# jeun-990806/pim-jpeg-decoder

Measured on AMD Instinct MI355X. Metric: MPixels/sec JPEG->RGB (bit-exact BMP), higher is better.
Workload: dtype int16/int32 (integer IDCT), u8 out

## Files before the change

### include/pjd.h

```cpp
#ifndef PJD_H
#define PJD_H

#include <stddef.h>
#include <stdint.h>

#ifdef __cplusplus
extern "C" {
#endif

#define PJD_VERSION 6

#define PJD_OK              0
#define PJD_E_NODEVICE     -1
#define PJD_E_HIP          -2
#define PJD_E_ARG          -3
#define PJD_E_NOMEM        -4
#define PJD_E_STATE        -5

#define PJD_ST_OK        0
#define PJD_ST_DC_SYM    1
#define PJD_ST_DC_LEN    2
#define PJD_ST_DC_BITS   3
#define PJD_ST_AC_SYM    4
#define PJD_ST_AC_RUN    5
// ... 64 lines not shown
    uint32_t qt_slot48[4];
    const pjd_scan_desc *scans;
    uint32_t n_scans;
    uint32_t reserved_;
} pjd_image_desc;

typedef struct pjd_ctx pjd_ctx;
typedef struct pjd_batch pjd_batch;

#define PJD_MAX_KERNELS 16
typedef struct pjd_timings {
    int32_t n;
    float   ms[PJD_MAX_KERNELS];
    char    name[PJD_MAX_KERNELS][32];
    float   total_ms;
} pjd_timings;

typedef struct pjd_batch_info {
    int32_t  n_images;
    uint64_t pixels;
    uint64_t ecs_bytes;
    uint64_t out_bytes;
    uint64_t coef_bytes;
    uint64_t n_data_units;
    uint64_t n_subsequences;
    uint64_t device_bytes;
    int32_t  n_sequential;
    int32_t  n_fallback;
    uint64_t n_huff_workgroups;
    uint64_t sync_rounds;
    uint64_t sync_lane_passes;
    uint64_t fix_rounds, fix_lane_passes;
    uint32_t sub_bytes;
    uint32_t n_table_sets;
    uint64_t n_huff_waves;
    uint64_t n_entries;
    float    exact_fallback_ms;
    uint32_t n_entropy_errors;
    uint64_t flag_waves[8];
    uint32_t huff_lds_bytes;
    uint32_t plan_mode;
    uint64_t walks, walk_lanes;
    uint64_t n_steps;
    uint32_t lane_fill_x1024;
    uint32_t dc_plan;
} pjd_batch_info;

int  pjd_version(void);
int  pjd_open(int device_ordinal, pjd_ctx **out);
void pjd_close(pjd_ctx *ctx);
#define PJD_PLAN_LATENCY     0
#define PJD_PLAN_THROUGHPUT  1
int  pjd_set_plan_mode(pjd_ctx *ctx, int mode);
const char *pjd_last_error(pjd_ctx *ctx);
const char *pjd_status_string(int status);
void *pjd_stream(pjd_ctx *ctx);

int  pjd_batch_create(pjd_ctx *ctx, const pjd_image_desc *images, int n_images,
                      int out_format, pjd_batch **out);
int  pjd_batch_upload(pjd_batch *b);
int  pjd_batch_decode(pjd_batch *b);
int  pjd_batch_decode_timed(pjd_batch *b, pjd_timings *t);
int  pjd_batch_capture(pjd_batch *b);
int  pjd_batch_sync(pjd_batch *b);
int  pjd_batch_decode_chains(pjd_batch *b);
int  pjd_batch_download(pjd_batch *b, uint8_t *const *out, int32_t *status);
int  pjd_batch_download_packed(pjd_batch *b, uint8_t *host, uint64_t capacity, int32_t *status);
uint64_t pjd_batch_packed_size(pjd_batch *b);
uint64_t pjd_batch_output_offset(pjd_batch *b, int image);
int  pjd_batch_bind_output(pjd_batch *b, void *device_base, uint64_t capacity, const uint64_t *offsets);
int  pjd_batch_set_resize(pjd_batch *b, const uint32_t *out_w, const uint32_t *out_h);
int  pjd_resize_tap(uint32_t src_n, uint32_t dst_n, uint32_t i, uint32_t *i0, uint32_t *i1, uint32_t *w);
#define PJD_RESIZE_BILINEAR  0
#define PJD_RESIZE_ANTIALIAS 1
#define PJD_AA_MAX_TAPS      32
int  pjd_batch_set_resize_filter(pjd_batch *b, int filter);
int  pjd_resize_aa_taps(uint32_t src_n, uint32_t dst_n, uint32_t i, uint32_t *first, uint32_t *count, uint32_t *q);
#define PJD_RESIZE_BICUBIC      3
#define PJD_BICUBIC_MAX_TAPS    64
#define PJD_BICUBIC_MAX_GAIN    92681
int  pjd_resize_bicubic_taps(uint32_t src_n, uint32_t dst_n, uint32_t i, uint32_t *first, uint32_t *count, int32_t *q);
#define PJD_RW_HFLIP 1u
typedef struct pjd_resize_window {
    uint32_t x, y, w, h;
    uint32_t vw, vh;
    uint32_t ox, oy;
    uint32_t flags;
    uint32_t reserved_;
} pjd_resize_window;
int  pjd_batch_set_resize_window(pjd_batch *b, const pjd_resize_window *win );
int  pjd_resize_window_check(uint32_t sw, uint32_t sh, uint32_t tw, uint32_t th,
                             const pjd_resize_window *win, int filter);
int  pjd_batch_set_orientation(pjd_batch *b, const uint8_t *orientation );
typedef struct pjd_resize_pad { uint32_t left, top, right, bottom; } pjd_resize_pad;
int  pjd_batch_set_resize_pad(pjd_batch *b, const pjd_resize_pad *pad , const uint8_t fill[3]);
int  pjd_batch_set_pad_value(pjd_batch *b, const float value[3]);
int  pjd_resize_pad_check(uint32_t out_w, uint32_t out_h, const pjd_resize_pad *pad);
int  pjd_batch_set_resize_affine(pjd_batch *b, const double (*m)[6] , const uint8_t fill[3]);
int  pjd_warp_tap(const double m[6], uint32_t i, uint32_t j, int64_t *x0, int64_t *y0, uint32_t *wx, uint32_t *wy);
int  pjd_resize_affine_check(uint32_t sw, uint32_t sh, uint32_t tw, uint32_t th, const double m[6]);
int  pjd_batch_set_colour(pjd_batch *b, const double (*m)[12] );
int  pjd_colour_value(const double m[12], const uint8_t rgb[3], uint8_t out[3]);
int  pjd_colour_check(const double m[12]);
#define PJD_BLUR_MAX_TAPS 63
typedef struct pjd_blur { double sigma; uint32_t ksize; uint32_t reserved_; } pjd_blur;
int  pjd_batch_set_blur(pjd_batch *b, const pjd_blur *blur );
int  pjd_blur_taps(uint32_t ksize, double sigma, uint32_t *q );
int  pjd_blur_index(uint32_t n, int64_t i, uint32_t *src);
int  pjd_blur_check(const pjd_blur *blur);
#define PJD_DT_F16   1
#define PJD_DT_BF16  2
#define PJD_DT_F32   3
int  pjd_batch_set_normalize(pjd_batch *b, int dtype, const float scale[3], const float bias[3]);
int  pjd_normalize_value(int dtype, uint32_t v, float scale, float bias, void *out);
#define PJD_MAX_VIEWS 65536u
int  pjd_batch_set_views(pjd_batch *b, const uint32_t *picture_of_view, uint32_t n_views);
uint32_t pjd_batch_n_outputs(pjd_batch *b);
int  pjd_batch_get_info(pjd_batch *b, pjd_batch_info *info);
uint64_t pjd_batch_output_size(pjd_batch *b, int image);
void *pjd_batch_device_output(pjd_batch *b, int image);
void *pjd_batch_device_status(pjd_batch *b);
void pjd_batch_destroy(pjd_batch *b);

uint64_t pjd_coefficients_size(uint32_t width, uint32_t height, uint8_t h_samp, uint8_t v_samp);
int  pjd_batch_download_coefficients(pjd_batch *b, int image, int16_t *out, uint64_t capacity_int16);

int  pjd_decode_batch(pjd_ctx *ctx, const pjd_image_desc *images, int n_images,
                      int out_format, uint8_t *const *out, int32_t *status);

#define PJD_SPLIT_MAX_DEVICES 16
typedef struct pjd_split_stats {
    double   wall_s, broadcast_s, upload_s, exec_s, download_s;
    uint64_t blob_bytes;
    uint64_t ecs_bytes[PJD_SPLIT_MAX_DEVICES];
    uint32_t n_segments, n_ranks;
    uint32_t n_exact;
    int32_t  rccl_used;
    int32_t  redone_whole;
} pjd_split_stats;
int  pjd_split_decode(const pjd_image_desc *desc, const int32_t *devices, int n_devices, int out_format,
                      uint8_t *out, uint64_t capacity, int32_t *status, pjd_split_stats *stats);
int  pjd_split_plan(const pjd_image_desc *desc, int world, int rank, pjd_image_desc *shard, uint64_t *seg_scratch,
                    uint64_t *byte_lo, uint64_t *byte_hi, uint32_t *first_mcu, uint32_t *last_mcu);
void pjd_split_release(void);
int  pjd_split_rccl_selftest(int device_ordinal, uint64_t bytes);

int  pjd_exec_dpu_payload(pjd_ctx *ctx, const uint32_t *metadata, int16_t *mcus, int n_dpus);

int  pjd_plan_info(const pjd_image_desc *images, int n_images, int out_format, pjd_batch_info *info);
int  pjd_plan_check(const pjd_image_desc *images, int n_images, int out_format, char *text, uint64_t cap);
int  pjd_plan_step_bits(const pjd_image_desc *image, uint32_t *step_bits_x256);
int  pjd_plan_luts(const pjd_image_desc *image, void *blob, uint64_t cap, uint32_t *real_bytes, uint32_t *nominal_bytes, uint8_t *slots);
int  pjd_batch_huff_occupancy(pjd_batch *batch, int32_t *workgroups_per_cu, uint32_t *lds_bytes);

void *pjd_host_alloc(uint64_t bytes);
void pjd_host_free(void *p);

uint64_t pjd_output_size(uint32_t width, uint32_t height, int out_format);
int  pjd_output_channels(int out_format);
int  pjd_scaled_dims(uint32_t width, uint32_t height, uint32_t flags, uint32_t *out_w, uint32_t *out_h);
uint64_t pjd_image_output_size(const pjd_image_desc *d, int out_format);

#ifdef __cplusplus
}
#endif
#endif
```

### pim-jpeg-decoder_amd/csrc/pjd_api.hip

```cpp
#include <hip/hip_runtime.h>

#include <algorithm>
#include <cstdio>
#include <cstdlib>
#include <cstring>
#include <atomic>
#include <mutex>
#include <string>
#include <type_traits>
#include <vector>

#include "../../include/pjd.h"
#include "pjd_kernels.h"
#include "pjd_libjpeg.h"
#include "pjd_lut_build.h"
#include "pjd_plan.h"
#include "pjd_resize_plan.h"

struct PoolBlock { void *p; size_t bytes; };
struct Pool {
    std::mutex m;
    std::vector<PoolBlock> free_blocks;
    size_t bytes = 0;
    void *take(size_t want, size_t &got)
    {
        std::lock_guard<std::mutex> l(m);
        int best = -1;
        for (size_t k = 0; k < free_blocks.size(); k++) {
            const size_t sz = free_blocks[k].bytes;
            if (sz >= want && sz <= 2 * want + (1u << 20) && (best < 0 || sz < free_blocks[best].bytes)) best = (int)k;
        }
        if (best < 0) return nullptr;
        void *p = free_blocks[best].p;
        got = free_blocks[best].bytes;
        bytes -= got;
        free_blocks.erase(free_blocks.begin() + best);
        return p;
    }
    bool give(void *p, size_t sz, size_t cap)
    {
        std::lock_guard<std::mutex> l(m);
        if (bytes + sz > cap) return false;
        free_blocks.push_back({p, sz}); bytes += sz;
        return true;
    }
    template <class F> void flush(F release)
    {
        std::lock_guard<std::mutex> l(m);
        for (PoolBlock &k : free_blocks) release(k.p);
        free_blocks.clear(); bytes = 0;
    }
};

struct pjd_ctx {
    int device = 0;
    hipStream_t stream = nullptr;
    Pool dev_pool, pin_pool;
    size_t pool_cap = (size_t)64 << 30;
    std::string err;
    bool force_sequential = false;
    uint32_t sub_bytes_override = 0;
    int plan_mode = PJD_PLAN_LATENCY;
    int poison = -1;
    std::vector<hipStream_t> group_streams;
    std::vector<hipEvent_t> join_ev;
    hipEvent_t fork_ev = nullptr, tables_ev = nullptr;
};

#define HIP_TRY(ctx, call)                                                                      \
    do {                                                                                        \
        hipError_t e_ = (call);                                                                 \
        if (e_ != hipSuccess) {                                                                 \
            (ctx)->err = std::string(#call) + ": " + hipGetErrorString(e_);                     \
            return PJD_E_HIP;                                                                   \
        }                                                                                       \
    } while (0)

namespace {

std::atomic<int> g_active[64];

std::mutex g_ctx_m;
std::vector<pjd_ctx *> g_ctxs;

hipError_t poison_dev(pjd_ctx *ctx, void *p, size_t bytes)
{
    if (ctx->poison < 0 || !p || bytes == 0) return hipSuccess;
    return hipMemsetAsync(p, ctx->poison, bytes, ctx->stream);
}

int pool_dev_alloc(pjd_ctx *ctx, void **out, size_t bytes, std::vector<PoolBlock> &owned)
{
    if (bytes == 0) bytes = 16;
    size_t got = 0;
    void *p = ctx->dev_pool.take(bytes, got);
    if (!p) {
        hipError_t e = hipMalloc(&p, bytes);
        if (e != hipSuccess) {
            (void)hipGetLastError();
            std::lock_guard<std::mutex> l(g_ctx_m);
            for (pjd_ctx *c : g_ctxs)
                if (c->device == ctx->device) c->dev_pool.flush([](void *q) { (void)hipFree(q); });
            e = hipMalloc(&p, bytes);
        }
        if (e != hipSuccess) { ctx->err = std::string("hipMalloc: ") + hipGetErrorString(e); return PJD_E_NOMEM; }
        got = bytes;
    }
    owned.push_back({p, got});
    *out = p;
    if (poison_dev(ctx, p, got) != hipSuccess) { (void)hipGetLastError(); ctx->err = "PJD_DEBUG_POISON: hipMemsetAsync failed"; return PJD_E_HIP; }
    return PJD_OK;
}

std::string fmt_name(const char *f, const std::string &name)
{
    char buf[240];
    std::snprintf(buf, sizeof buf, f, name.c_str());
    return buf;
}

int pool_pin_alloc(pjd_ctx *ctx, void **out, size_t bytes, std::vector<PoolBlock> &owned)
{
    if (bytes == 0) bytes = 16;
    size_t got = 0;
    void *p = ctx->pin_pool.take(bytes, got);
    if (!p) {
        if (hipHostMalloc(&p, bytes, hipHostMallocDefault) != hipSuccess) { ctx->err = "hipHostMalloc failed"; return PJD_E_NOMEM; }
        got = bytes;
    }
    owned.push_back({p, got});
    *out = p;
    if (ctx->poison >= 0) std::memset(p, ctx->poison, got);
    return PJD_OK;
}

}

struct pjd_batch {
    pjd_ctx *ctx = nullptr;
    PjdPlan plan;
    PjdBackForm back{};
    PjdDevBatch dev{};
    PjdDevIdctWg *d_iwgs_dense = nullptr;
    PjdDevIdctWg *d_iwgs_dense_std = nullptr, *d_cwgs_std = nullptr;
    uint8_t *d_planes = nullptr;
    uint32_t *d_seq_list = nullptr;
    uint64_t *d_seq_base = nullptr;
    int32_t *d_status_init = nullptr;
    uint64_t *d_opstate = nullptr;
    size_t opstate_bytes = 0;
    uint8_t *d_in = nullptr, *h_in = nullptr;
    size_t in_bytes = 0, images_off = 0;
    int32_t *h_status = nullptr;
    unsigned long long *h_stats = nullptr;
    std::vector<uint32_t> seq_list;
    std::vector<PoolBlock> dev_blocks, pin_blocks;
    uint64_t device_bytes = 0;
    bool uploaded = false, decoded = false, settled = false;
    int n_fallback = 0;
    float exact_fallback_ms = 0;
    uint32_t n_entropy_errors = 0;
    hipGraph_t graph = nullptr;
    hipGraphExec_t graph_exec = nullptr;
    hipGraph_t graph_groups = nullptr;
    hipGraphExec_t graph_exec_groups = nullptr;
    bool counted = false;
    int chains = 0;
    int graph_chains[2] = {0, 0};
    bool bound = false, bound_offsets = false;
    uint64_t bound_capacity = 0;
    std::vector<uint64_t> packed_off;
    uint8_t *res_out = nullptr;
    std::vector<uint64_t> res_off, res_bytes;
    uint64_t res_buf_bytes = 0, res_out_bytes = 0;
    bool resized = false;
    bool viewed = false;
    std::vector<uint32_t> view_pic;
    size_t n_out() const { return viewed ? view_pic.size() : plan.images.size(); }
    uint32_t pic_of(size_t v) const { return viewed ? view_pic[v] : (uint32_t)v; }
    std::string out_name(size_t v) const
    {
        char buf[64];
        if (viewed) std::snprintf(buf, sizeof buf, "view %zu (picture %u)", v, view_pic[v]);
        else std::snprintf(buf, sizeof buf, "picture %zu", v);
        return buf;
    }
    PjdResizeSpec spec;
    PjdResizeForm form;
    struct Pair { uint8_t *h = nullptr, *d = nullptr; size_t bytes = 0; };
    Pair rs;
    Pair win;
    Pair pad;
    Pair aa;
    Pair warp;
    Pair col;
    Pair blur;
    uint8_t *d_blur_buf = nullptr;
    uint8_t *resample_dst() const { return form.blurred ? d_blur_buf : res_out; }
    PjdNormalize resample_norm() const { return form.blurred ? PjdNormalize{} : norm; }
    PjdNormalize norm{};
    uint8_t pad_fill[3] = {0, 0, 0};
    bool pad_value_set = false;
    float pad_value[3] = {0, 0, 0};

    void launch_resize(hipStream_t s) const
    {
        const size_t n = n_out();
        const bool planar = back.planes();
        pjd_launch_resize(s, PjdResizeLaunch{dev.out, resample_dst(), (const PjdDevResize *)rs.d, (const uint32_t *)(rs.d + n * sizeof(PjdDevResize)), (uint32_t)n, form.tiles, planar, resample_norm(),
                                             form.windowed ? (const PjdDevResizeWin *)win.d : nullptr, form.oriented, spec.filter,
                                             (const PjdDevResizeAA *)aa.d, aa.d ? (const uint32_t *)(aa.d + n * sizeof(PjdDevResizeAA)) : nullptr, form.lds,
                                             form.padded ? (const PjdDevResizePad *)pad.d : nullptr, spec.channels,
                                             form.coloured ? (const PjdDevColour *)col.d : nullptr});
    }
    void launch_warp(hipStream_t s) const
    {
        const size_t n = n_out();
        const uint8_t *f = spec.affine_fill;
        pjd_launch_warp(s, PjdWarpLaunch{dev.out, resample_dst(), (const PjdDevResize *)rs.d, (const PjdDevWarp *)warp.d, (const uint32_t *)(rs.d + n * sizeof(PjdDevResize)), (uint32_t)n, form.tiles,
                                         back.planes(), resample_norm(), (uint32_t)f[0] | ((uint32_t)f[1] << 8) | ((uint32_t)f[2] << 16), spec.channels,
                                         form.coloured ? (const PjdDevColour *)col.d : nullptr});
    }
    void launch_blur(hipStream_t s) const
    {
        const size_t n = n_out();
        const uint8_t *prefix = blur.d + n * sizeof(PjdDevBlur);
        pjd_launch_blur(s, PjdBlurLaunch{d_blur_buf, res_out, (const PjdDevBlur *)blur.d, (const uint32_t *)prefix, (const uint32_t *)(prefix + (n + 1) * sizeof(uint32_t)), (uint32_t)n,
                                         form.blur_tiles, back.planes(), norm, spec.channels, form.blur_lds});
    }
    void launch_pad(hipStream_t s) const
    {
        const size_t n = n_out();
        const bool planar = back.planes();
        pjd_launch_resize_border(s, PjdBorderLaunch{res_out, (const PjdDevResize *)rs.d, (const PjdDevResizePad *)pad.d, (const uint32_t *)(pad.d + n * sizeof(PjdDevResizePad)), (uint32_t)n,
                                                    form.lines, planar, norm.dtype ? PJD_DT_SIZE(norm.dtype) : 1u, pjd_pad_fill(norm, planar, pad_fill, pad_value_set ? pad_value : nullptr), spec.channels});
    }
};

namespace {

int take_pair(pjd_batch *b, pjd_batch::Pair &p, size_t bytes)
{
    if (p.d) return PJD_OK;
    int rc = p.h ? PJD_OK : pool_pin_alloc(b->ctx, (void **)&p.h, bytes, b->pin_blocks);
    if (rc == PJD_OK) rc = pool_dev_alloc(b->ctx, (void **)&p.d, bytes, b->dev_blocks);
    if (rc != PJD_OK) return rc;
    p.bytes = bytes;
    b->device_bytes += bytes;
    return PJD_OK;
}

void give_back(pjd_batch *b, void *p, uint64_t counted)
{
    pjd_ctx *ctx = b->ctx;
    for (size_t k = 0; k < b->dev_blocks.size(); k++)
        if (b->dev_blocks[k].p == p) {
            if (!ctx->dev_pool.give(b->dev_blocks[k].p, b->dev_blocks[k].bytes, ctx->pool_cap)) hipFree(b->dev_blocks[k].p);
            b->dev_blocks.erase(b->dev_blocks.begin() + (long)k);
            b->device_bytes -= counted;
            break;
        }
}

template <class A, class B = uint32_t>
void put(const pjd_batch::Pair &p, const std::vector<A> &a, const std::vector<B> &behind = {})
{
    if (!a.empty()) std::memcpy(p.h, a.data(), a.size() * sizeof(A));
    if (!behind.empty()) std::memcpy(p.h + a.size() * sizeof(A), behind.data(), behind.size() * sizeof(B));
}

int commit_request(pjd_batch *b, PjdResizeSpec &spec, const PjdResizeWork &w)
{
    hipSetDevice(b->ctx->device);
    const size_t n = spec.pic.size();
    int rc = take_pair(b, b->rs, n * sizeof(PjdDevResize) + (n + 1) * sizeof(uint32_t));
    if (rc == PJD_OK && w.form.windowed) rc = take_pair(b, b->win, n * sizeof(PjdDevResizeWin));
    if (rc == PJD_OK && w.form.padded) rc = take_pair(b, b->pad, n * sizeof(PjdDevResizePad) + (n + 1) * sizeof(uint32_t));
    if (rc == PJD_OK && spec.filter != PJD_RESIZE_BILINEAR) rc = take_pair(b, b->aa, n * sizeof(PjdDevResizeAA) + w.tab.size() * sizeof(uint32_t));
    if (rc == PJD_OK && w.form.warp) rc = take_pair(b, b->warp, n * sizeof(PjdDevWarp));
    if (rc == PJD_OK && w.form.coloured) rc = take_pair(b, b->col, n * sizeof(PjdDevColour));
    if (rc == PJD_OK && w.form.blurred) rc = take_pair(b, b->blur, n * sizeof(PjdDevBlur) + (n + 1) * sizeof(uint32_t) + w.blur_taps.size() * sizeof(uint32_t));
    if (rc == PJD_OK && w.form.blurred && !b->d_blur_buf) {
        rc = pool_dev_alloc(b->ctx, (void **)&b->d_blur_buf, (size_t)w.form.blur_buf_bytes, b->dev_blocks);
        if (rc == PJD_OK) b->device_bytes += w.form.blur_buf_bytes;
    }
    if (rc != PJD_OK) return rc;
    put(b->rs, w.recs, w.tile_prefix);
    if (w.form.windowed) put(b->win, w.win);
    if (w.form.padded) put(b->pad, w.pad, w.line_prefix);
    if (spec.filter != PJD_RESIZE_BILINEAR) put(b->aa, w.aa, w.tab);
    if (w.form.warp) put(b->warp, w.warp);
    if (w.form.coloured) put(b->col, w.colour);
    if (w.form.blurred) {
        put(b->blur, w.blur, w.blur_prefix);
        std::memcpy(b->blur.h + n * sizeof(PjdDevBlur) + (n + 1) * sizeof(uint32_t), w.blur_taps.data(), w.blur_taps.size() * sizeof(uint32_t));
    }
    b->spec = std::move(spec);
    b->form = w.form;
    return PJD_OK;
}

int apply_request(pjd_batch *b, PjdResizeSpec &spec, const char *setter)
// ... 110 lines not shown
}

int pjd_set_plan_mode(pjd_ctx *ctx, int mode)
{
    if (!ctx) return PJD_E_ARG;
    if (mode != PJD_PLAN_LATENCY && mode != PJD_PLAN_THROUGHPUT) { ctx->err = "unknown plan mode"; return PJD_E_ARG; }
    ctx->plan_mode = mode;
    return PJD_OK;
}

void pjd_close(pjd_ctx *ctx)
{
    if (!ctx) return;
    {
        std::lock_guard<std::mutex> l(g_ctx_m);
        for (size_t k = 0; k < g_ctxs.size(); k++)
            if (g_ctxs[k] == ctx) { g_ctxs.erase(g_ctxs.begin() + k); break; }
    }
    hipSetDevice(ctx->device);
    if (ctx->stream) { hipStreamSynchronize(ctx->stream); hipStreamDestroy(ctx->stream); }
    for (hipStream_t st : ctx->group_streams) { hipStreamSynchronize(st); hipStreamDestroy(st); }
    for (hipEvent_t ev : ctx->join_ev) hipEventDestroy(ev);
    if (ctx->fork_ev) hipEventDestroy(ctx->fork_ev);
    if (ctx->tables_ev) hipEventDestroy(ctx->tables_ev);
    ctx->dev_pool.flush([](void *q) { (void)hipFree(q); });
    ctx->pin_pool.flush([](void *q) { (void)hipHostFree(q); });
    delete ctx;
}

const char *pjd_last_error(pjd_ctx *ctx) { return ctx ? ctx->err.c_str() : "no context"; }

const char *pjd_status_string(int status)
{
    switch (status & 0xFF) {
        case PJD_ST_OK: return "";
        case PJD_ST_DC_SYM: return "Error - Invalid DC value (255)";
        case PJD_ST_DC_LEN: return "Error - DC coefficient length greater than 11";
        case PJD_ST_DC_BITS: return "Error - Invalid DC value";
        case PJD_ST_AC_SYM: return "Error - Invalid AC value";
        case PJD_ST_AC_RUN: return "Error - Zero run-length exceeded block component";
        case PJD_ST_AC_LEN: return "Error - AC coefficient length greater than 10";
        case PJD_ST_AC_BITS: return "Error - Invalid AC value";
        default: return "Error - unknown";
    }
}

void *pjd_stream(pjd_ctx *ctx) { return ctx ? (void *)ctx->stream : nullptr; }

void pjd_batch_destroy(pjd_batch *b)
{
    if (!b) return;
    hipSetDevice(b->ctx->device);
    hipStreamSynchronize(b->ctx->stream);
    if (b->counted) { g_active[b->ctx->device].fetch_sub(1); b->counted = false; }
    if (b->graph_exec) hipGraphExecDestroy(b->graph_exec);
    if (b->graph) hipGraphDestroy(b->graph);
    if (b->graph_exec_groups) hipGraphExecDestroy(b->graph_exec_groups);
    if (b->graph_groups) hipGraphDestroy(b->graph_groups);
    pjd_ctx *ctx = b->ctx;
    for (PoolBlock &k : b->dev_blocks)
        if (!ctx->dev_pool.give(k.p, k.bytes, ctx->pool_cap)) hipFree(k.p);
    for (PoolBlock &k : b->pin_blocks)
        if (!ctx->pin_pool.give(k.p, k.bytes, ctx->pool_cap / 4)) hipHostFree(k.p);
    delete b;
}

int pjd_batch_create(pjd_ctx *ctx, const pjd_image_desc *images, int n_images, int out_format, pjd_batch **out)
{
    if (!ctx || !out) return PJD_E_ARG;
    *out = nullptr;
    pjd_batch *b = new pjd_batch;
    b->ctx = ctx;
    std::vector<pjd_image_desc> forced;
    if (ctx->force_sequential && images && n_images > 0) {
        forced.assign(images, images + n_images);
        for (pjd_image_desc &d : forced) if (d.shard_n_segs == 0) d.flags |= PJD_F_FORCE_SEQUENTIAL;
        images = forced.data();
    }
    int rc = pjd_make_plan(images, n_images, out_format, b->plan, ctx->err, ctx->sub_bytes_override, ctx->plan_mode);
    if (rc != PJD_OK) { delete b; return rc; }
    PjdPlan &P = b->plan;
    hipSetDevice(ctx->device);

    auto fail = [&](int code) { pjd_batch_destroy(b); return code; };
    b->seq_list = P.seq_images;
    b->back = PjdBackForm{P.gray ? PJD_BACK_GRAY : (P.planar ? PJD_BACK_PLANAR : PJD_BACK_INTERLEAVED), P.scaled};
    std::vector<uint64_t> seq_base;
    std::vector<int32_t> st0(P.images.size(), 0);
    for (uint32_t i : b->seq_list) { st0[i] = PJD_STW_NEEDS_EXACT; seq_base.push_back(P.images[i].dense_base); }
    struct Part { const void *src; size_t bytes, off; void *dev; };
    std::vector<Part> parts;
    size_t in_bytes = 0;
    auto part = [&](const auto &vec, size_t min_count, auto *&dev) {
        using T = std::remove_cv_t<std::remove_reference_t<decltype(vec[0])>>;
        static_assert(std::is_same<T, std::remove_cv_t<std::remove_reference_t<decltype(*dev)>>>::value, "the list and its device pointer differ in type");
        const size_t off = in_bytes;
        parts.push_back({vec.data(), vec.size() * sizeof(T), off, &dev});
        in_bytes = (off + std::max(vec.size(), std::max(min_count, (size_t)1)) * sizeof(T) + 255) & ~(size_t)255;
        return off;
    };
    b->images_off = part(P.images, 0, b->dev.images);
    part(P.tsets, 0, b->dev.tsets); part(P.tables, 0, b->dev.raw_tables); part(P.qtab, 0, b->dev.qtab); part(P.segs, 0, b->dev.segs); part(P.subs, 0, b->dev.lanes);
    part(P.hwaves, 0, b->dev.hwaves); part(P.hwgs, 0, b->dev.hwgs); part(P.iwgs, 0, b->dev.iwgs); part(P.iwgs_dense, 0, b->d_iwgs_dense); part(P.pscans, 0, b->dev.pscans);
    part(P.group_images, 0, b->dev.group_images); part(P.iwg_order, 0, b->dev.iwg_order);
    if (P.libjpeg) { part(P.iwgs_dense_std, 0, b->d_iwgs_dense_std); part(P.cwgs_std, 0, b->d_cwgs_std); }
    part(b->seq_list, (size_t)n_images, b->d_seq_list); part(seq_base, (size_t)n_images, b->d_seq_base); part(st0, (size_t)n_images, b->d_status_init);
    const size_t o_ecs = in_bytes;
    in_bytes += P.ecs_buf_bytes;
    b->in_bytes = in_bytes;
    if (pool_pin_alloc(ctx, (void **)&b->h_in, in_bytes, b->pin_blocks) != PJD_OK) return fail(PJD_E_NOMEM);
    for (const Part &q : parts) if (q.bytes) std::memcpy(b->h_in + q.off, q.src, q.bytes);
    {
        uint8_t *h_ecs = b->h_in + o_ecs;
        uint64_t pos = 0;
        for (int i = 0; i < n_images; i++) {
            const uint64_t off = P.images[i].ecs_off, len = P.host[i].ecs_copy_len;
            if (off > pos) std::memset(h_ecs + pos, 0, off - pos);
            if (len) std::memcpy(h_ecs + off, P.host[i].ecs_src, len);
            pos = off + len;
            if (P.images[i].flags & PJD_IF_PROGRESSIVE)
                for (uint32_t k = 0; k < P.images[i].n_pscan; k++) {
                    const PjdHostScan &hs = P.host_scans[P.images[i].pscan_base + k];
                    if (hs.off > pos) std::memset(h_ecs + pos, 0, hs.off - pos);
                    if (hs.len) std::memcpy(h_ecs + hs.off, hs.src, hs.len);
                    pos = hs.off + hs.len;
                }
        }
        std::memset(h_ecs + pos, 0, P.ecs_buf_bytes - pos);
    }
    if (pool_pin_alloc(ctx, (void **)&b->h_status, sizeof(int32_t) * (n_images + 1), b->pin_blocks) != PJD_OK) return fail(PJD_E_NOMEM);
    if (pool_pin_alloc(ctx, (void **)&b->h_stats, 16 * sizeof(unsigned long long), b->pin_blocks) != PJD_OK) return fail(PJD_E_NOMEM);

#define TRY_RC(x) do { int rc_ = (x); if (rc_ != PJD_OK) return fail(rc_); } while (0)
    auto dev_alloc = [&](auto *&dptr, size_t n) {
        using T = std::remove_reference_t<decltype(*dptr)>;
        if (n == 0) n = 1;
        void *p = nullptr;
        const int r = pool_dev_alloc(ctx, &p, n * sizeof(T), b->dev_blocks);
        dptr = (T *)p;
        b->device_bytes += n * sizeof(T);
        return r;
    };
    const size_t n_hwave = P.hwaves.size();
    TRY_RC(dev_alloc(b->d_in, in_bytes));
    for (const Part &q : parts) { const uint8_t *p = b->d_in + q.off; std::memcpy(q.dev, &p, sizeof p); }
    b->dev.ecs = b->d_in + o_ecs;
    if (P.libjpeg && !P.gray) TRY_RC(dev_alloc(b->d_planes, (size_t)P.plane_bytes));
    TRY_RC(dev_alloc(b->dev.luts, (size_t)P.lut_buf_bytes));
    TRY_RC(dev_alloc(b->dev.words, (size_t)P.n_words));
    TRY_RC(dev_alloc(b->dev.coef, P.dense_du * 64));
    TRY_RC(dev_alloc(b->dev.ent, (size_t)P.n_ent));
    TRY_RC(dev_alloc(b->dev.lane_info, P.subs.size()));
    TRY_RC(dev_alloc(b->dev.lane_dc, P.subs.size()));
    TRY_RC(dev_alloc(b->dev.dc_blk, (size_t)P.n_dcblk * 8));
    TRY_RC(dev_alloc(b->dev.marks, P.iwgs.size()));
    TRY_RC(dev_alloc(b->dev.out, P.out_buf_bytes));
    TRY_RC(dev_alloc(b->dev.status, (size_t)n_images));
    TRY_RC(dev_alloc(b->dev.imstate, (size_t)n_images));
    const size_t op_words = n_hwave * (PJD_GENS + 1) + 2 + PJD_MAX_GROUPS;
    TRY_RC(dev_alloc(b->d_opstate, op_words));
    b->opstate_bytes = op_words * sizeof(uint64_t);
    b->dev.wave_gen = b->d_opstate;
    b->dev.wave_desc = b->d_opstate + n_hwave * PJD_GENS;
    b->dev.ticket = reinterpret_cast<uint32_t *>(b->d_opstate + n_hwave * (PJD_GENS + 1));
    if (std::getenv("PJD_DEBUG_STATS")) TRY_RC(dev_alloc(b->dev.dbg, n_hwave * 32));
    TRY_RC(dev_alloc(b->dev.stats, 16));
#undef TRY_RC
    b->dev.n_images = (uint32_t)n_images; b->dev.n_tsets = (uint32_t)P.tsets.size(); b->dev.n_lanes = (uint32_t)P.subs.size();
    b->dev.n_hwave = (uint32_t)n_hwave; b->dev.n_hwg = (uint32_t)P.hwgs.size();
    b->dev.n_iwg = (uint32_t)P.iwgs.size(); b->dev.n_dcblk = (uint32_t)P.n_dcblk;
    b->dev.sub_bytes = P.sub_bytes;
    b->dev.word_rows = PJD_WORD_ROWS(P.sub_bytes);
    b->dev.lane_cap = P.lane_cap;
    b->dev.max_lut_bytes = P.max_lut_bytes;
    b->res_out = b->dev.out;
    for (int i = 0; i < n_images; i++) { b->res_off.push_back(P.images[i].out_off); b->res_bytes.push_back(P.host[i].out_bytes); }
    b->res_buf_bytes = P.out_buf_bytes; b->res_out_bytes = P.out_bytes;
    *out = b;
    return PJD_OK;
}

int pjd_batch_upload(pjd_batch *b)
{
    if (!b) return PJD_E_ARG;
    pjd_ctx *ctx = b->ctx;
    PjdPlan &P = b->plan;
    if (int rc = check_views_resolved(b, "upload")) return rc;
    hipSetDevice(ctx->device);
    hipStream_t s = ctx->stream;
    HIP_TRY(ctx, hipMemcpyAsync(b->d_in, b->h_in, b->in_bytes, hipMemcpyHostToDevice, s));
    if (!b->bound || b->resized) HIP_TRY(ctx, hipMemsetAsync(b->dev.out, 0, P.out_buf_bytes, s));
    if (b->resized) HIP_TRY(ctx, hipMemcpyAsync(b->rs.d, b->rs.h, b->rs.bytes, hipMemcpyHostToDevice, s));
    if (b->aa.d) HIP_TRY(ctx, hipMemcpyAsync(b->aa.d, b->aa.h, b->aa.bytes, hipMemcpyHostToDevice, s));
    if (b->form.windowed) HIP_TRY(ctx, hipMemcpyAsync(b->win.d, b->win.h, b->win.bytes, hipMemcpyHostToDevice, s));
    if (b->form.padded) HIP_TRY(ctx, hipMemcpyAsync(b->pad.d, b->pad.h, b->pad.bytes, hipMemcpyHostToDevice, s));
    if (b->form.warp) HIP_TRY(ctx, hipMemcpyAsync(b->warp.d, b->warp.h, b->warp.bytes, hipMemcpyHostToDevice, s));
    if (b->form.coloured) HIP_TRY(ctx, hipMemcpyAsync(b->col.d, b->col.h, b->col.bytes, hipMemcpyHostToDevice, s));
    if (b->form.blurred) HIP_TRY(ctx, hipMemcpyAsync(b->blur.d, b->blur.h, b->blur.bytes, hipMemcpyHostToDevice, s));
    const bool parallel = !P.hwgs.empty();
    if (parallel || !b->seq_list.empty()) pjd_launch_build_tables(s, b->dev);
    if (parallel) pjd_launch_lane_words(s, b->dev);
    HIP_TRY(ctx, hipGetLastError());
    b->uploaded = true;
    return PJD_OK;
}

}

namespace {

struct KernelTimer {
    pjd_timings *t;
    hipStream_t s;
    std::vector<hipEvent_t> ev;
    std::vector<std::string> names;
    bool debug_sync = std::getenv("PJD_DEBUG_SYNC") != nullptr;
    void mark(const char *name)
    {
        if (debug_sync) {
            const hipError_t e = hipStreamSynchronize(s);
            std::fprintf(stderr, "[pjd] %-14s %s\n", name, e == hipSuccess ? "ok" : hipGetErrorString(e));
        }
        if (!t) return;
        hipEvent_t e;
        hipEventCreate(&e);
        hipEventRecord(e, s);
        ev.push_back(e);
        names.push_back(name);
    }
    void finish()
    {
        if (!t) return;
        hipStreamSynchronize(s);
        t->n = 0;
        for (size_t k = 0; k + 1 < ev.size() && t->n < PJD_MAX_KERNELS; k++) {
            float ms = 0;
            hipEventElapsedTime(&ms, ev[k], ev[k + 1]);
            t->ms[t->n] = ms;
            std::snprintf(t->name[t->n], sizeof t->name[0], "%s", names[k + 1].c_str());
            t->n++;
        }
        t->total_ms = 0;
        if (ev.size() >= 2) hipEventElapsedTime(&t->total_ms, ev.front(), ev.back());
        for (hipEvent_t e : ev) hipEventDestroy(e);
    }
};

bool ctx_group_streams(pjd_ctx *ctx, size_t ng)
{
    if (!ctx->fork_ev && hipEventCreateWithFlags(&ctx->fork_ev, hipEventDisableTiming) != hipSuccess) { ctx->fork_ev = nullptr; return false; }
    if (!ctx->tables_ev && hipEventCreateWithFlags(&ctx->tables_ev, hipEventDisableTiming) != hipSuccess) { ctx->tables_ev = nullptr; return false; }
    while (ctx->group_streams.size() + 1 < ng) {
        hipStream_t st = nullptr;
        hipEvent_t ev = nullptr;
        if (hipStreamCreateWithFlags(&st, hipStreamNonBlocking) != hipSuccess) return false;
        if (hipEventCreateWithFlags(&ev, hipEventDisableTiming) != hipSuccess) { hipStreamDestroy(st); return false; }
        ctx->group_streams.push_back(st);
        ctx->join_ev.push_back(ev);
    }
    return true;
}

void launch_dense(hipStream_t s, const pjd_batch *b, const PjdDevBatch &dv, const PjdDevIdctWg *wgs, size_t n, const PjdDevIdctWg *wgs_std, size_t n_std, size_t n_red,
                  const uint64_t *dense_base)
{
    pjd_launch_idct_dense(s, dv, b->back, wgs, dense_base, (uint32_t)n);
    pjd_launch_idct_std_dense(s, dv, b->back, wgs_std, dense_base, (uint32_t)n_std, (uint32_t)n_red, b->d_planes);
}

void launch_resample(hipStream_t s, const pjd_batch *b, KernelTimer *kt)
{
    if (!b->resized) return;
    if (b->form.warp) {
        b->launch_warp(s);
        if (kt) kt->mark("warp");
    } else {
        b->launch_resize(s);
        if (kt) kt->mark("resize");
        if (b->form.padded) {
            b->launch_pad(s);
            if (kt) kt->mark("pad");
        }
    }
    if (!b->form.blurred) return;
    b->launch_blur(s);
    if (kt) kt->mark("blur");
}

int enqueue_decode(pjd_batch *b, pjd_timings *timings, bool use_groups)
{
    pjd_ctx *ctx = b->ctx;
    PjdPlan &P = b->plan;
    hipStream_t s = ctx->stream;
    KernelTimer kt{timings, s, {}, {}};
    const bool parallel = !P.hwgs.empty();
    kt.mark("start");
    pjd_launch_reset(s, b->dev, b->d_status_init, parallel ? b->d_opstate : nullptr, parallel ? b->opstate_bytes / 8 : 0,
                     b->dev.dbg ? (uint32_t)(P.hwaves.size() * 32) : 0u);
    kt.mark("reset");
    static const bool idle_groups = [] { const char *e = std::getenv("PJD_IDLE_FORM"); return !e || std::strcmp(e, "chain") != 0; }();
    const bool idle = !timings && use_groups && parallel && !P.groups.empty() && idle_groups;
    const PjdBackForm F = b->back;
    const size_t ng = idle ? P.groups.size() : 0;
    const bool grouped = ng > 1 && ctx_group_streams(ctx, ng);
    if (grouped) {
        HIP_TRY(ctx, hipEventRecord(ctx->fork_ev, s));
        for (size_t g = 0; g < ng; g++) {
            hipStream_t gs = g == 0 ? s : ctx->group_streams[g - 1];
            if (g) HIP_TRY(ctx, hipStreamWaitEvent(gs, ctx->fork_ev, 0));
            pjd_launch_huff_lanes_group(gs, b->dev, P.groups[g], (uint32_t)g);
            pjd_launch_group_dc(gs, b->dev, P.groups[g]);
            pjd_launch_idct_lanes(gs, b->dev, F, b->dev.iwg_order + P.groups[g].iwg_first, P.groups[g].iwg_count);
            if (g) { HIP_TRY(ctx, hipEventRecord(ctx->join_ev[g - 1], gs)); }
        }
        for (size_t g = 1; g < ng; g++) HIP_TRY(ctx, hipStreamWaitEvent(s, ctx->join_ev[g - 1], 0));
    } else {
        if (parallel) {
            pjd_launch_huff_lanes(s, b->dev);    kt.mark("huff_lanes");
            pjd_launch_lane_dc_scan(s, b->dev, P.dc_per_picture);  kt.mark("dc_scan");
            pjd_launch_idct_lanes(s, b->dev, F, P.libjpeg ? b->dev.iwg_order : nullptr, P.libjpeg ? P.n_iwg_def : b->dev.n_iwg);
            kt.mark(F.gray() ? "idct_gray" : "idct_colour");
            if (P.n_iwg_std + P.n_iwg_red) {
                pjd_launch_idct_std_lanes(s, b->dev, F, b->dev.iwg_order + P.n_iwg_def, P.n_iwg_std, P.n_iwg_red, b->d_planes);
                kt.mark(F.gray() ? "idct_gray_std" : "idct_std");
            }
        }
    }
    if (!b->seq_list.empty()) {
        pjd_launch_zero(s, b->dev.coef, P.dense_du * 64 * sizeof(int16_t));
        pjd_launch_huff_sequential(s, b->dev, b->d_seq_list, b->d_seq_base, (uint32_t)b->seq_list.size());
        if (!P.pscans.empty()) pjd_launch_progressive(s, b->dev, b->d_seq_list, b->d_seq_base, (uint32_t)b->seq_list.size());
        launch_dense(s, b, b->dev, b->d_iwgs_dense, P.iwgs_dense.size(), b->d_iwgs_dense_std, P.libjpeg ? P.n_dense_std : 0, P.libjpeg ? P.n_dense_red : 0, b->d_seq_base);
        kt.mark("exact_path");
    }
    if (P.libjpeg && !F.gray()) {
        pjd_launch_colour_std(s, b->dev, b->d_cwgs_std, P.n_cwg_std, P.n_cwg_red, b->d_planes);
        kt.mark("colour_std");
    }
    launch_resample(s, b, &kt);
    HIP_TRY(ctx, hipGetLastError());
    kt.finish();
    b->decoded = true;
    b->settled = false;
    b->chains = grouped ? (int)ng : 1;
    return PJD_OK;
}

struct Scratch {
    std::vector<void *> blocks;
    std::vector<hipEvent_t> events;
    bool out_of_memory = false;
    Scratch() = default;
    Scratch(const Scratch &) = delete;
    ~Scratch() { for (hipEvent_t e : events) (void)hipEventDestroy(e); for (void *p : blocks) (void)hipFree(p); }
    template <class T> hipError_t alloc(T *&p, size_t bytes)
    {
        const hipError_t e = hipMalloc((void **)&p, bytes);
        if (e == hipSuccess) blocks.push_back(p); else { p = nullptr; out_of_memory = true; }
        return e;
    }
    hipEvent_t event()
    {
        hipEvent_t e = nullptr;
        if (hipEventCreate(&e) == hipSuccess) events.push_back(e); else e = nullptr;
        return e;
    }
};

hipError_t redo_exact(const pjd_batch *b, Scratch &tmp, const uint32_t *list, const uint64_t *base, size_t n, uint64_t du, const void *extra, size_t extra_bytes,
                      hipEvent_t before, PjdDevBatch &dv, uint8_t *d[4])
{
    hipStream_t s = b->ctx->stream;
    const void *h[4] = {nullptr, list, base, extra};
    const size_t bytes[4] = {(size_t)du * 64 * sizeof(int16_t), n * sizeof(uint32_t), n * sizeof(uint64_t), extra_bytes};
    hipError_t e = hipSuccess;
    for (int k = 0; k < 4 && e == hipSuccess; k++) { d[k] = nullptr; if (k == 0 || h[k]) e = tmp.alloc(d[k], bytes[k]); }
    for (int k = 0; k < 4 && e == hipSuccess; k++) e = poison_dev(b->ctx, d[k], bytes[k]);
    if (e != hipSuccess) return e;
    pjd_launch_zero(s, d[0], bytes[0]);
    e = hipGetLastError();
    for (int k = 1; k < 4 && e == hipSuccess; k++) if (h[k]) e = hipMemcpyAsync(d[k], h[k], bytes[k], hipMemcpyHostToDevice, s);
    if (e != hipSuccess) return e;
    dv = b->dev;
    dv.coef = (int16_t *)d[0];
    if (before) (void)hipEventRecord(before, s);
    pjd_launch_huff_sequential(s, dv, (const uint32_t *)d[1], (const uint64_t *)d[2], (uint32_t)n);
    return hipSuccess;
}

int settle(pjd_batch *b)
{
    pjd_ctx *ctx = b->ctx;
    PjdPlan &P = b->plan;
    hipStream_t s = ctx->stream;
    if (b->settled || !b->decoded) return PJD_OK;
    const size_t n = P.images.size();
    HIP_TRY(ctx, hipMemcpyAsync(b->h_status, b->dev.status, sizeof(int32_t) * n, hipMemcpyDeviceToHost, s));
    HIP_TRY(ctx, hipStreamSynchronize(s));
    if (b->counted) { g_active[ctx->device].fetch_sub(1); b->counted = false; }
    std::vector<uint32_t> fb;
    std::vector<uint64_t> fb_base;
    std::vector<PjdDevIdctWg> fb_wgs, fb_wgs_std, fb_wgs_red;
    std::vector<char> was_seq(n, 0);
    for (uint32_t i : b->seq_list) was_seq[i] = 1;
    uint64_t du = 0;
    for (size_t i = 0; i < n; i++)
        if ((b->h_status[i] & PJD_STW_NEEDS_EXACT) && !was_seq[i]) {
            const PjdDevImage &g = P.images[i];
            for (uint32_t k = 0; k < g.n_iwg; k++) {
                PjdDevIdctWg w = P.iwgs[g.iwg_base + k];
                w.pad_ = (uint32_t)fb.size();
                ((g.flags & PJD_IF_LIBJPEG) ? ((g.flags & PJD_IF_LJSCALE_MASK) ? fb_wgs_red : fb_wgs_std) : fb_wgs).push_back(w);
            }
            fb.push_back((uint32_t)i);
            fb_base.push_back(du);
            du += (uint64_t)(g.last_mcu - g.first_mcu) * g.dus_per_mcu;
        }
    b->n_fallback = (int)fb.size();
    b->exact_fallback_ms = 0;
    b->n_entropy_errors = 0;
    for (size_t i = 0; i < n; i++)
        if (!(b->h_status[i] & PJD_STW_NEEDS_EXACT) && (b->h_status[i] & 0xFF) != 0) b->n_entropy_errors++;
    if (!fb.empty()) {
        const size_t n_def = fb_wgs.size(), n_std = fb_wgs_std.size(), n_red = fb_wgs_red.size();
        fb_wgs.insert(fb_wgs.end(), fb_wgs_std.begin(), fb_wgs_std.end());
        fb_wgs.insert(fb_wgs.end(), fb_wgs_red.begin(), fb_wgs_red.end());
        Scratch tmp;
        hipEvent_t ev0 = tmp.event(), ev1 = tmp.event();
        PjdDevBatch dv;
        uint8_t *d[4];
        hipError_t e = redo_exact(b, tmp, fb.data(), fb_base.data(), fb.size(), du, fb_wgs.data(), fb_wgs.size() * sizeof(PjdDevIdctWg), ev0, dv, d);
        if (tmp.out_of_memory) { ctx->err = "hipMalloc failed for the exact-kernel scratch"; return PJD_E_NOMEM; }
        if (e == hipSuccess) {
            const PjdDevIdctWg *d_wgs = (const PjdDevIdctWg *)d[3];
            launch_dense(s, b, dv, d_wgs, n_def, d_wgs + n_def, n_std, n_red, (const uint64_t *)d[2]);
            if (n_std + n_red && !b->back.gray()) pjd_launch_colour_std(s, dv, b->d_cwgs_std, P.n_cwg_std, P.n_cwg_red, b->d_planes);
            if (ev1) (void)hipEventRecord(ev1, s);
            launch_resample(s, b, nullptr);
            e = hipGetLastError();
        }
        if (e == hipSuccess) e = hipMemcpyAsync(b->h_status, b->dev.status, sizeof(int32_t) * n, hipMemcpyDeviceToHost, s);
        if (e == hipSuccess) e = hipStreamSynchronize(s);
        if (e == hipSuccess && ev0 && ev1) (void)hipEventElapsedTime(&b->exact_fallback_ms, ev0, ev1);
        if (e != hipSuccess) { ctx->err = std::string("exact-kernel fallback: ") + hipGetErrorString(e); return PJD_E_HIP; }
    }
    b->settled = true;
    return PJD_OK;
}

}

extern "C" {

static bool device_idle_then_count(pjd_batch *b)
{
    const int dev = b->ctx->device;
    if (dev < 0 || dev >= 64) return false;
    const int before = b->counted ? g_active[dev].load() - 1 : g_active[dev].fetch_add(1);
    b->counted = true;
    static const int force = [] { const char *e = std::getenv("PJD_GROUPS_ALWAYS"); return e ? std::atoi(e) : -1; }();
    if (force >= 0) return force != 0;
    return before <= 0;
}

int pjd_batch_decode(pjd_batch *b)
{
    if (!b) return PJD_E_ARG;
    if (int rc = check_views_resolved(b, "decode")) return rc;
    if (!b->uploaded) { b->ctx->err = "decode before upload"; return PJD_E_STATE; }
    hipSetDevice(b->ctx->device);
    const bool groups = !b->plan.groups.empty() && device_idle_then_count(b);
// ... 419 lines not shown
    PjdResizeSpec spec = b->spec;
    spec.colour_set = true;
    spec.colour.resize(spec.pic.size());
    for (size_t i = 0; i < spec.pic.size(); i++) std::memcpy(spec.colour[i].m, m[i], sizeof spec.colour[i].m);
    return apply_request(b, spec, "set_colour");
}

int pjd_blur_check(const pjd_blur *blur) { return pjd_blur_fault(blur) ? 0 : 1; }

int pjd_blur_taps(uint32_t ksize, double sigma, uint32_t *q)
{
    const pjd_blur e{sigma, ksize, 0u};
    if (!q || ksize == 0 || pjd_blur_fault(&e)) return PJD_E_ARG;
    pjd_blur_taps_calc(ksize, sigma, q);
    return PJD_OK;
}

int pjd_blur_index(uint32_t n, int64_t i, uint32_t *src)
{
    if (!src || n == 0 || n > 65535u) return PJD_E_ARG;
    const int64_t p = n > 1u ? 2 * ((int64_t)n - 1) : 1;
    *src = pjd_blur_index_calc(n, (int32_t)(i % p));
    return PJD_OK;
}

int pjd_batch_set_blur(pjd_batch *b, const pjd_blur *blur)
{
    if (!b) return PJD_E_ARG;
    pjd_ctx *ctx = b->ctx;
    if (int rc = check_order(b, ST_BLUR)) return rc;
    if (!blur) { ctx->err = "set_blur: null record array"; return PJD_E_ARG; }
    PjdResizeSpec spec = b->spec;
    spec.blur_set = true;
    spec.blur.assign(blur, blur + spec.pic.size());
    return apply_request(b, spec, "set_blur");
}

int pjd_resize_pad_check(uint32_t out_w, uint32_t out_h, const pjd_resize_pad *pad)
{
    return pjd_resize_pad_fault(out_w, out_h, pad) ? PJD_E_ARG : PJD_OK;
}

int pjd_batch_set_resize_pad(pjd_batch *b, const pjd_resize_pad *pad, const uint8_t fill[3])
{
    if (!b) return PJD_E_ARG;
    pjd_ctx *ctx = b->ctx;
    if (int rc = check_order(b, ST_PAD)) return rc;
    if (!pad) { ctx->err = "set_resize_pad: null record array"; return PJD_E_ARG; }
    if (!fill) { ctx->err = "set_resize_pad: null fill"; return PJD_E_ARG; }
    PjdResizeSpec spec = b->spec;
    spec.pad_set = true; spec.pad.assign(pad, pad + spec.pic.size());
    const int rc = apply_request(b, spec, "set_resize_pad");
    if (rc == PJD_OK) std::memcpy(b->pad_fill, fill, 3);
    return rc;
}

int pjd_batch_set_pad_value(pjd_batch *b, const float value[3])
{
    if (!b) return PJD_E_ARG;
    pjd_ctx *ctx = b->ctx;
    if (int rc = check_order(b, ST_PAD_VALUE)) return rc;
    if (!value) { ctx->err = "set_pad_value: null value array"; return PJD_E_ARG; }
    for (int c = 0; c < 3; c++)
        if (!finite_f32(value[c])) { ctx->err = "set_pad_value: the values must be finite"; return PJD_E_ARG; }
    for (int c = 0; c < 3; c++) b->pad_value[c] = value[c];
    b->pad_value_set = true;
    return PJD_OK;
}

int pjd_normalize_value(int dtype, uint32_t v, float scale, float bias, void *out)
{
    if (dtype != PJD_DT_F16 && dtype != PJD_DT_BF16 && dtype != PJD_DT_F32) return PJD_E_ARG;
    if (v > 255u || !finite_f32(scale) || !finite_f32(bias) || !out) return PJD_E_ARG;
    const uint32_t e = pjd_f32_to_dtype_bits(dtype, pjd_normalize_f32(v, scale, bias));
    if (dtype == PJD_DT_F32) { std::memcpy(out, &e, 4); return PJD_OK; }
    const uint16_t h = (uint16_t)e;
    std::memcpy(out, &h, 2);
    return PJD_OK;
}

int pjd_batch_set_normalize(pjd_batch *b, int dtype, const float scale[3], const float bias[3])
{
    if (!b) return PJD_E_ARG;
    pjd_ctx *ctx = b->ctx;
    PjdPlan &P = b->plan;
    if (int rc = check_order(b, ST_NORMALIZE)) return rc;
    if (!scale || !bias) { ctx->err = "set_normalize: null constant array"; return PJD_E_ARG; }
    if (dtype != PJD_DT_F16 && dtype != PJD_DT_BF16 && dtype != PJD_DT_F32) { ctx->err = "set_normalize: unknown dtype (PJD_DT_F16, PJD_DT_BF16 or PJD_DT_F32)"; return PJD_E_ARG; }
    for (int c = 0; c < 3; c++)
        if (!finite_f32(scale[c]) || !finite_f32(bias[c])) { ctx->err = "set_normalize: scale and bias must be finite"; return PJD_E_ARG; }
    if (P.out_format == PJD_OUT_BMP) { ctx->err = "set_normalize: a BMP batch cannot be normalised (PJD_OUT_RGB8 or PJD_OUT_RGB8_PLANAR)"; return PJD_E_ARG; }
    const size_t n = b->n_out();
    for (size_t i = 0; i < n; i++)
        if (P.host[b->pic_of(i)].shard) { ctx->err = fmt_name("set_normalize: %s is a shard (its picture is only partly written)", b->out_name(i)); return PJD_E_ARG; }
    hipSetDevice(ctx->device);
    std::vector<uint32_t> w = b->spec.out_w, h = b->spec.out_h;
    if (!b->resized) {
        w.resize(n); h.resize(n);
        for (size_t i = 0; i < n; i++) {
            const PjdDevImage &g = P.images[b->pic_of(i)];
            pjd_scaled_dims(g.width, g.height, PJD_IF_OUT_SCALE_LOG(g.flags) << 4, &w[i], &h[i]);
        }
    }
    const PjdPackedLayout lay = pjd_packed_layout(w.data(), h.data(), n, PJD_DT_SIZE(dtype), P.gray ? 1u : 3u);
    void *d_res = nullptr;
    int rc = pool_dev_alloc(ctx, &d_res, (size_t)lay.buf_bytes, b->dev_blocks);
    if (rc != PJD_OK) return rc;
    b->device_bytes += lay.buf_bytes;
    if (!b->resized) {
        rc = pjd_batch_set_resize(b, w.data(), h.data());
        if (rc != PJD_OK) { give_back(b, d_res, lay.buf_bytes); return rc; }
    }
    give_back(b, b->res_out, b->res_buf_bytes);
    set_result_offsets(b, lay.off);
    b->res_out = (uint8_t *)d_res;
    b->res_off = lay.off; b->res_bytes = lay.bytes;
    b->res_buf_bytes = lay.buf_bytes; b->res_out_bytes = lay.sum;
    b->norm.dtype = dtype;
    for (int c = 0; c < 3; c++) { b->norm.scale[c] = scale[c]; b->norm.bias[c] = bias[c]; }
    return PJD_OK;
}

void *pjd_host_alloc(uint64_t bytes)
{
    void *p = nullptr;
    if (hipHostMalloc(&p, bytes ? bytes : 16, hipHostMallocDefault) != hipSuccess) return nullptr;
    return p;
}

void pjd_host_free(void *p) { if (p) hipHostFree(p); }

static void plan_info(const PjdPlan &P, pjd_batch_info *info)
{
    std::memset(info, 0, sizeof *info);
    info->n_images = (int32_t)P.images.size();
    info->pixels = P.pixels; info->ecs_bytes = P.ecs_bytes; info->out_bytes = P.out_bytes;
    info->coef_bytes = P.n_ent * 2 + P.n_words * 4 + P.dense_du * 128;
    info->n_data_units = P.n_du;
    info->n_subsequences = P.subs.size();
    info->n_sequential = (int32_t)P.seq_images.size();
    info->sub_bytes = P.sub_bytes;
    info->plan_mode = (uint32_t)P.plan_mode;
    info->n_table_sets = (uint32_t)P.tsets.size();
    info->huff_lds_bytes = (uint32_t)(P.max_lut_bytes + PJD_HUFF_WAVES * (PJD_WAVE_LDS + PJD_PHASE_LDS) + 16);
    info->n_huff_waves = P.hwaves.size();
    info->n_huff_workgroups = P.hwgs.size();
    info->dc_plan = (P.dc_per_picture ? 1u : 0u) | ((uint32_t)P.groups.size() << 8);
}

static void print_wave_timeline(const pjd_batch *b)
{
    int wg = 0;
    size_t lds = 0;
    if (pjd_huff_lanes_occupancy(b->dev, &wg, &lds) == hipSuccess)
        std::fprintf(stderr, "[pjd waves] pjd_k_huff_lanes: %zu B of LDS per workgroup, %d workgroups per CU\n", lds, wg);
    if (b->decoded) {
        const size_t nw = b->plan.hwaves.size();
        std::vector<uint32_t> d(nw * 32);
        if (hipMemcpy(d.data(), b->dev.dbg, d.size() * 4, hipMemcpyDeviceToHost) == hipSuccess && nw) {
            if (const char *dump = std::getenv("PJD_DEBUG_DUMP")) {
                if (FILE *f = std::fopen(dump, "wb")) { std::fwrite(d.data(), 4, d.size(), f); std::fclose(f); }
            }
            uint32_t t0 = d[0];
            for (size_t k = 0; k < nw; k++) if ((int32_t)(d[k * 32] - t0) < 0) t0 = d[k * 32];
            double sum[6] = {0}; uint32_t mx[6] = {0}; size_t worst = 0; uint32_t worst_end = 0;
            for (size_t k = 0; k < nw; k++) {
                const uint32_t *e = &d[k * 32];
                uint32_t end = e[0] - t0;
                for (int q = 1; q <= 5; q++) { sum[q] += e[q]; if (e[q] > mx[q]) mx[q] = e[q]; end += e[q]; }
                sum[0] += e[0] - t0; if (e[0] - t0 > mx[0]) mx[0] = e[0] - t0;
                if (end > worst_end) { worst_end = end; worst = k; }
            }
            const double n = (double)nw;
            {
                std::vector<uint32_t> cl;
                for (size_t k = 0; k < nw; k++) { cl.push_back(d[k * 32 + 7] >> 8); d[k * 32 + 7] &= 0xffu; }
                std::sort(cl.begin(), cl.end());
                std::fprintf(stderr, "[pjd waves] shader clock while the waves ran: median %.2f GHz (min %.2f, max %.2f)\n", cl[nw / 2] / 160.0, cl.front() / 160.0, cl.back() / 160.0);
            }
            std::fprintf(stderr, "[pjd waves] n %zu | mean(us): start %.1f passA %.1f rounds %.1f stitch %.1f scan %.1f write+verify %.1f | max(us): %.1f %.1f %.1f %.1f %.1f %.1f\n",
                         nw, sum[0] / n / 100, sum[1] / n / 100, sum[2] / n / 100, sum[3] / n / 100, sum[4] / n / 100, sum[5] / n / 100,
                         mx[0] / 100.0, mx[1] / 100.0, mx[2] / 100.0, mx[3] / 100.0, mx[4] / 100.0, mx[5] / 100.0);
            const uint32_t *e = &d[worst * 32];
            std::fprintf(stderr, "[pjd waves] last to finish: wave %zu (image %u, %u lanes) start %.1f passA %.1f rounds %.1f stitch %.1f scan %.1f write %.1f -> end %.1f us\n",
                         worst, e[6], e[7], (e[0] - t0) / 100.0, e[1] / 100.0, e[2] / 100.0, e[3] / 100.0, e[4] / 100.0, e[5] / 100.0, worst_end / 100.0);
            for (size_t k = 0; k < nw; k++)
                if (d[k * 32 + 6] == e[6] && d[k * 32 + 7] != 0) {
                    std::fprintf(stderr, "[pjd waves]   wave %zu: start %.1f passA %.1f rounds %.1f stitch %.1f scan %.1f write %.1f\n", k,
                                 (d[k * 32] - t0) / 100.0, d[k * 32 + 1] / 100.0, d[k * 32 + 2] / 100.0, d[k * 32 + 3] / 100.0, d[k * 32 + 4] / 100.0, d[k * 32 + 5] / 100.0);
                    std::fprintf(stderr, "[pjd waves]     rounds (lanes:us):");
                    for (int r = 0; r < 24 && d[k * 32 + 8 + r]; r++) {
                        const uint32_t v = d[k * 32 + 8 + r];
                        std::fprintf(stderr, (v >> 31) ? " w%u:%.1f" : " %u:%.1f", (v >> 24) & 0x7fu, (v & 0xffffff) / 100.0);
                    }
                    std::fprintf(stderr, "\n");
                }
        }
    }
}

int pjd_batch_get_info(pjd_batch *b, pjd_batch_info *info)
{
    if (!b || !info) return PJD_E_ARG;
    hipSetDevice(b->ctx->device);
    plan_info(b->plan, info);
    info->out_bytes = b->res_out_bytes;
    info->device_bytes = b->device_bytes;
    info->n_fallback = b->n_fallback; info->exact_fallback_ms = b->exact_fallback_ms; info->n_entropy_errors = b->n_entropy_errors;
    unsigned long long *st = b->h_stats;
    if (b->decoded && hipMemcpyAsync(st, b->dev.stats, 16 * sizeof(unsigned long long), hipMemcpyDeviceToHost, b->ctx->stream) == hipSuccess &&
        hipStreamSynchronize(b->ctx->stream) == hipSuccess) {
        info->sync_rounds = st[0]; info->sync_lane_passes = st[1]; info->fix_rounds = st[2]; info->fix_lane_passes = st[3];
        info->walks = st[PJD_STAT_WALKS]; info->walk_lanes = st[PJD_STAT_WALKS + 1];
        for (int r = 0; r < PJD_FLAG_REASONS && r < 8; r++) info->flag_waves[r] = st[PJD_STAT_FLAG0 + r];
        info->n_entries = st[PJD_STAT_ENTRIES];
        info->n_steps = st[PJD_STAT_STEPS];
        info->lane_fill_x1024 = (uint32_t)st[PJD_STAT_FILL];
    }
    if (b->dev.dbg) print_wave_timeline(b);
    return PJD_OK;
}

int pjd_plan_info(const pjd_image_desc *images, int n_images, int out_format, pjd_batch_info *info)
{
    if (!info) return PJD_E_ARG;
    PjdPlan P;
    std::string err;
    int rc = pjd_make_plan(images, n_images, out_format, P, err, env_sub_bytes(), env_plan_mode());
    if (rc != PJD_OK) return rc;
    plan_info(P, info);
    return PJD_OK;
}

int pjd_plan_check(const pjd_image_desc *images, int n_images, int out_format, char *text, uint64_t cap)
{
    PjdPlan P;
    std::string err;
    const int rc = pjd_make_plan(images, n_images, out_format, P, err);
    if (text && cap) std::snprintf(text, (size_t)cap, "%s", rc == PJD_OK ? "" : err.c_str());
    return rc;
}

int pjd_plan_step_bits(const pjd_image_desc *image, uint32_t *step_bits_x256)
{
    if (!image || !step_bits_x256) return PJD_E_ARG;
    PjdPlan P;
    std::string err;
    int rc = pjd_make_plan(image, 1, PJD_OUT_RGB8, P, err);
    if (rc != PJD_OK) return rc;
    if (P.images.empty() || P.tset_step_bits.empty() || (P.images[0].flags & PJD_IF_SEQUENTIAL)) return PJD_E_ARG;
    *step_bits_x256 = P.tset_step_bits[P.images[0].tset];
    return PJD_OK;
}

int pjd_plan_luts(const pjd_image_desc *image, void *blob, uint64_t cap, uint32_t *real_bytes, uint32_t *nominal_bytes, uint8_t *slots)
{
    if (!image || !real_bytes || !nominal_bytes) return PJD_E_ARG;
    PjdPlan P;
    std::string err;
    int rc = pjd_make_plan(image, 1, PJD_OUT_RGB8, P, err);
    if (rc != PJD_OK) return rc;
    if (P.images.empty() || P.tsets.empty() || (P.images[0].flags & PJD_IF_PROGRESSIVE)) return PJD_E_ARG;
    const PjdDevImage &im = P.images[0];
    const PjdDevTset &T = P.tsets[im.tset];
    *real_bytes = T.lut_bytes;
    *nominal_bytes = P.tset_nominal_bytes[im.tset];
    if (slots) std::memcpy(slots, im.tbl_slot, 6);
    if (!blob || T.lut_bytes == 0) return PJD_OK;
    if (cap < T.lut_bytes) return PJD_E_ARG;
    std::memset(blob, 0, T.lut_bytes);
    uint16_t *b16 = static_cast<uint16_t *>(blob);
    for (uint32_t slot = 0; slot < T.n_tables; slot++) {
        const PjdDevHuffRaw &r = P.tables[(size_t)im.tset * PJD_MAX_TABLES + slot];
        const uint32_t partner = r.is_ac ? slot : (uint32_t)T.pair_ac[slot];
        const bool has_partner = partner < T.n_tables;
        const PjdDevHuffRaw &r2 = P.tables[(size_t)im.tset * PJD_MAX_TABLES + (has_partner ? partner : slot)];
        uint32_t first[17], first2[17];
        pjd_lut_first_codes(r, first);
        pjd_lut_first_codes(r2, first2);
        uint32_t *L1 = reinterpret_cast<uint32_t *>(b16 + slot * (PJD_L1_BYTES / 2));
        const uint16_t *cp = T.l2_cp[slot], *ce = T.l2_ce[slot];
        const uint32_t p1 = T.l2_p1[slot];
        for (uint32_t idx = 0; idx < (1u << PJD_LUT_BITS); idx++)
            L1[idx] = pjd_lut_l1_entry(r, first, has_partner ? &r2 : nullptr, first2, cp, ce, p1, idx);
        const uint32_t n2 = pjd_lut_l2_entries(cp, p1);
        for (uint32_t j = 0; j < n2; j++) b16[ce[0] + j] = (uint16_t)pjd_lut_l2_entry(r, first, cp, ce, j);
    }
    return PJD_OK;
}

int pjd_batch_huff_occupancy(pjd_batch *b, int32_t *workgroups_per_cu, uint32_t *lds_bytes)
{
    if (!b || !workgroups_per_cu) return PJD_E_ARG;
    hipSetDevice(b->ctx->device);
    int n = 0;
    size_t lds = 0;
    if (pjd_huff_lanes_occupancy(b->dev, &n, &lds) != hipSuccess) return PJD_E_HIP;
    *workgroups_per_cu = n;
    if (lds_bytes) *lds_bytes = (uint32_t)lds;
    return PJD_OK;
}

uint64_t pjd_batch_output_size(pjd_batch *b, int image)
{
    if (!b || image < 0 || (size_t)image >= b->n_out()) return 0;
    return b->res_bytes[image];
}

void *pjd_batch_device_output(pjd_batch *b, int image)
{
    if (!b || image < 0 || (size_t)image >= b->n_out()) return nullptr;
    return b->res_out + b->res_off[image];
}

void *pjd_batch_device_status(pjd_batch *b) { return b ? (void *)b->dev.status : nullptr; }

uint64_t pjd_coefficients_size(uint32_t width, uint32_t height, uint8_t h_samp, uint8_t v_samp)
{
    uint64_t w = (width + 7) / 8, h = (height + 7) / 8;
    if (h_samp == 2 && (w & 1)) w++;
    if (v_samp == 2 && (h & 1)) h++;
    const uint64_t pw = (w + 1) / 2 * 2, ph = (h + 1) / 2 * 2;
    return (pw * ph + 99) / 100 * 19200;
}

int pjd_batch_download_coefficients(pjd_batch *b, int image, int16_t *out, uint64_t capacity_int16)
{
    if (!b || !out || image < 0 || (size_t)image >= b->plan.images.size()) return PJD_E_ARG;
    if (!b->decoded) { b->ctx->err = "download_coefficients before decode"; return PJD_E_STATE; }
    pjd_ctx *ctx = b->ctx;
    PjdPlan &P = b->plan;
    hipSetDevice(ctx->device);
    int rc = settle(b);
    if (rc != PJD_OK) return rc;
    const PjdDevImage &g = P.images[image];
    const uint64_t n16 = pjd_coefficients_size(g.width, g.height, (uint8_t)g.hs, (uint8_t)g.vs);
    if (capacity_int16 < n16) { ctx->err = "download_coefficients: buffer smaller than pjd_coefficients_size"; return PJD_E_ARG; }
    hipStream_t s = ctx->stream;
    Scratch tmp;
    int16_t *d_out = nullptr;
    if (tmp.alloc(d_out, n16 * sizeof(int16_t)) != hipSuccess) { ctx->err = "hipMalloc failed (coefficients)"; return PJD_E_NOMEM; }
    hipError_t e = poison_dev(ctx, d_out, n16 * sizeof(int16_t));
    pjd_launch_zero(s, d_out, n16 * sizeof(int16_t));
    const uint32_t n_du = (g.last_mcu - g.first_mcu) * g.dus_per_mcu, first_du = g.first_mcu * g.dus_per_mcu;
    const bool routed = P.host[image].sequential;
    const bool fell_back = !routed && (b->h_status[image] & PJD_STW_NEEDS_EXACT);
    const uint32_t one = (uint32_t)image; const uint64_t zero = 0;
    if (routed) {
        pjd_launch_coefdump_dense(s, b->dev, (uint32_t)image, b->dev.coef + g.dense_base * 64, first_du, n_du, d_out);
    } else if (fell_back) {
        PjdDevBatch dv;
        uint8_t *d[4];
        if (e == hipSuccess) e = redo_exact(b, tmp, &one, &zero, 1, n_du, nullptr, 0, nullptr, dv, d);
        if (tmp.out_of_memory) { ctx->err = "hipMalloc failed (coefficients scratch)"; return PJD_E_NOMEM; }
        if (e == hipSuccess) pjd_launch_coefdump_dense(s, dv, (uint32_t)image, dv.coef, first_du, n_du, d_out);
    } else {
        pjd_launch_coefdump_lanes(s, b->dev, (uint32_t)image, g.n_iwg, d_out);
    }
    if (e == hipSuccess) e = hipGetLastError();
    if (e == hipSuccess) e = hipMemcpyAsync(out, d_out, n16 * sizeof(int16_t), hipMemcpyDeviceToHost, s);
    if (e == hipSuccess) e = hipStreamSynchronize(s);
    if (e != hipSuccess) { ctx->err = std::string("download_coefficients: ") + hipGetErrorString(e); return PJD_E_HIP; }
    return PJD_OK;
}

int pjd_debug_poison_fill(pjd_ctx *ctx, void *p, uint64_t bytes)
{
    if (!ctx) return PJD_E_ARG;
    return poison_dev(ctx, p, (size_t)bytes) == hipSuccess ? PJD_OK : PJD_E_HIP;
}

int pjd_decode_batch(pjd_ctx *ctx, const pjd_image_desc *images, int n_images, int out_format,
                     uint8_t *const *out, int32_t *status)
{
    pjd_batch *b = nullptr;
    int rc = pjd_batch_create(ctx, images, n_images, out_format, &b);
    if (rc != PJD_OK) return rc;
    rc = pjd_batch_upload(b);
    if (rc == PJD_OK) rc = pjd_batch_decode(b);
    if (rc == PJD_OK) rc = pjd_batch_download(b, out, status);
    pjd_batch_destroy(b);
    return rc;
}

int pjd_exec_dpu_payload(pjd_ctx *ctx, const uint32_t *metadata, int16_t *mcus, int n_dpus)
{
    if (!ctx || !metadata || !mcus || n_dpus < 0) return PJD_E_ARG;
    if (n_dpus == 0) return PJD_OK;
    for (int d = 0; d < n_dpus; d++) {
        const uint32_t *m = metadata + (size_t)d * 276;
        const uint32_t V = m[5] & 255, H = m[6] & 255;
        if (m[19] != 100 || m[4] > 3 || (V != 1 && V != 2) || (H != 1 && H != 2)) { ctx->err = "DPU metadata outside the supported envelope"; return PJD_E_ARG; }
        for (uint32_t c = 0; c < m[4]; c++) if ((m[7 + c] & 255) > 3) { ctx->err = "DPU metadata: quantisation table id > 3"; return PJD_E_ARG; }
    }
    hipSetDevice(ctx->device);
    Scratch tmp;
    uint32_t *dm = nullptr; int16_t *dc = nullptr;
    const size_t mb = (size_t)n_dpus * 276 * 4, cb = (size_t)n_dpus * 19200 * 2;
    if (const hipError_t e = tmp.alloc(dm, mb)) { ctx->err = std::string("hipMalloc((void **)&dm, mb): ") + hipGetErrorString(e); return PJD_E_HIP; }
    if (tmp.alloc(dc, cb) != hipSuccess) { ctx->err = "hipMalloc(mcus)"; return PJD_E_NOMEM; }
    int rc = PJD_OK;
    auto chk = [&](hipError_t e, const char *what) { if (e != hipSuccess && rc == PJD_OK) { ctx->err = std::string(what) + ": " + hipGetErrorString(e); rc = PJD_E_HIP; } };
    chk(poison_dev(ctx, dm, mb), "poison(metadata_buffer)");
    chk(poison_dev(ctx, dc, cb), "poison(mcus)");
    chk(hipMemcpyAsync(dm, metadata, mb, hipMemcpyHostToDevice, ctx->stream), "copy(metadata_buffer)");
    chk(hipMemcpyAsync(dc, mcus, cb, hipMemcpyHostToDevice, ctx->stream), "copy(mcus)");
    if (rc == PJD_OK) { pjd_launch_dpu_payload(ctx->stream, dm, dc, n_dpus); chk(hipGetLastError(), "exec"); }
    chk(hipMemcpyAsync(mcus, dc, cb, hipMemcpyDeviceToHost, ctx->stream), "copy back");
    chk(hipStreamSynchronize(ctx->stream), "sync");
    return rc;
}

}
```

### pim-jpeg-decoder_amd/csrc/pjd_internal.h

```cpp
#pragma once
#include <stdint.h>

#ifndef PJD_SUB_BYTES_MIN
#define PJD_SUB_BYTES_MIN  128
#endif
#define PJD_SUB_BYTES_MAX  1024
#define PJD_HUFF_LANES     64
#ifndef PJD_HUFF_WAVES
#define PJD_HUFF_WAVES     2
#endif
#define PJD_HUFF_THREADS   (PJD_HUFF_LANES * PJD_HUFF_WAVES)
#ifndef PJD_NCHK
#define PJD_NCHK           4
#endif
#define PJD_STAGE_ENTRIES  16
#define PJD_CHK_BYTES      (2 * PJD_NCHK * 64 * 4)
#define PJD_STAGE_BYTES    (PJD_STAGE_ENTRIES * 2 * 64)
#define PJD_WAVE_LDS       (PJD_CHK_BYTES > PJD_STAGE_BYTES ? PJD_CHK_BYTES : PJD_STAGE_BYTES)
#define PJD_PHASE_LDS      256
#ifndef PJD_TAIL_PRIO
#define PJD_TAIL_PRIO      1
#endif
#ifndef PJD_IDCT_PRIO
#define PJD_IDCT_PRIO      0
// ... 45 lines not shown
#define PJD_IF_LJSCALE_MASK     (3u << PJD_IF_LJSCALE_SHIFT)
#define PJD_IF_OUT_SCALE_LOG(flags) ((((flags) & PJD_IF_SCALE_MASK) >> PJD_IF_SCALE_SHIFT) + (((flags) & PJD_IF_LJSCALE_MASK) >> PJD_IF_LJSCALE_SHIFT))
static inline __host__ __device__ uint32_t pjd_lj_chroma_size(uint32_t n, uint32_t hs, uint32_t vs)
{
    uint32_t cn = n;
    while (cn < 8u && 2u * cn <= hs * n && 2u * cn <= vs * n) cn *= 2u;
    return cn;
}

#define PJD_STW_NEEDS_EXACT 0x100

struct PjdDevImState {
    unsigned long long err_key;
    uint32_t flag_pos;
    uint32_t end_pos;
};

enum {
    PJD_FLAG_SYMBOL = 0,
    PJD_FLAG_SEGMENT,
    PJD_FLAG_NOSYNC,
    PJD_FLAG_STITCH,
    PJD_FLAG_TIMEOUT,
    PJD_FLAG_OVERFLOW,
    PJD_FLAG_VERIFY,
    PJD_FLAG_REASONS
};
#define PJD_STAT_FLAG0 4
#define PJD_STAT_ENTRIES 11
#define PJD_STAT_STEPS   14
#define PJD_STAT_FILL    15
#define PJD_STAT_WALKS   12

struct PjdDevImage {
    uint32_t width, height;
    uint32_t mcux, mcuy, n_mcu;
    uint32_t ncomp, hs, vs;
    uint32_t n_luma;
    uint32_t dus_per_mcu;
    uint32_t restart_interval;
    uint32_t flags;
    uint32_t ref_mcu_w, ref_mcu_h, ref_mcu_w_real;
    uint32_t ecs_len;
    uint64_t ecs_off;
    uint64_t dense_base;
    uint32_t n_du;
    uint32_t image_index;
    uint32_t out_stride;
    uint64_t out_off;
    uint32_t seg_base, n_seg;
    uint32_t lane_base, n_lane;
    uint32_t hwave_base, n_hwave;
    uint32_t iwg_base, n_iwg;
    uint32_t idct_mcus;
    uint32_t first_mcu, last_mcu;
    uint32_t tset;
    uint32_t sub_bytes;
    uint8_t  tbl_slot[3][2];
    uint8_t  walk_max;
    uint8_t  pad_;
    uint32_t pscan_base, n_pscan;
    uint32_t lane_cap;
    uint32_t plane_off256;
    uint64_t ent_base;
};

struct PjdDevHuffRaw {
    uint8_t offsets[17];
    uint8_t symbols[162];
    uint8_t is_ac;
};

struct PjdDevScan {
    uint64_t ecs_off;
    uint32_t ecs_len;
    uint32_t restart_interval;
    uint8_t  n_comp, comp[3];
    uint8_t  ss, se, ah, al;
    PjdDevHuffRaw table[3];
};

struct PjdDevTset {
    uint32_t lut_off16;
    uint32_t lut_bytes;
    uint32_t n_tables;
    uint16_t l2_cp[PJD_MAX_TABLES][PJD_L2_BITS];
    uint16_t l2_ce[PJD_MAX_TABLES][PJD_L2_BITS];
    uint16_t l2_p1[PJD_MAX_TABLES];
    uint8_t  pair_ac[PJD_MAX_TABLES];
    uint8_t  pad_[2];
};
#define PJD_LUT_USED(e)  ((e) & 31u)
#define PJD_LUT_ADV(e)   (((e) >> 5) & 127u)
#define PJD_LUT_SIZE(e)  (((e) >> 12) & 15u)
#define PJD_LUT_PAIR_USED(e)  (((e) >> 16) & 31u)
#define PJD_LUT_PAIR_ADV(e)   (((e) >> 21) & 127u)
#define PJD_LUT_PAIR_SIZE2(e) ((e) >> 28)
#define PJD_LUT_PTR_SHIFT(e)  (((e) >> 5) & 31u)
#define PJD_LUT_PTR_BYTES(e)  ((e) >> 16)
#define PJD_LUT_EOB      0x0800u
#define PJD_LUT_BADSYM   14u
#define PJD_LUT_BADLEN   15u
#define PJD_LUT_ENTRY(used, adv, eob, size)  ((used) | ((adv) << 5) | ((eob) ? PJD_LUT_EOB : 0u) | ((size) << 12))

struct PjdDevSegment {
    uint32_t byte_start;
    uint32_t byte_end;
    uint32_t first_du;
    uint32_t n_du;
};

struct PjdDevSub {
    uint32_t byte_start;
    uint32_t seg;
};

struct PjdDevHuffWave {
    uint32_t image;
    uint32_t first_lane;
    uint32_t n_lanes;
    uint32_t pad_;
};

struct PjdDevHuffWg {
    uint32_t first_wave;
    uint32_t n_waves;
    uint32_t tset;
    uint32_t pad_;
};

struct PjdDevIdctWg {
    uint32_t image;
    uint32_t first_mcu;
    uint32_t n_mcu;
    uint32_t pad_;
};

#define PJD_MAX_GROUPS 8
struct PjdDevGroup {
    uint32_t hwg_first, hwg_count;
    uint32_t img_first, img_count;
    uint32_t iwg_first, iwg_count;
    uint32_t pad_[2];
};

struct PjdDevLaneInfo {
    uint32_t n_ent;
    uint32_t first_du;
    uint16_t dc_sum[3];
    uint16_t pad_;
};
#define PJD_LANE_SEG_FIRST 0x80000000u

struct PjdDevLaneDc {
    uint16_t dc_in[3];
    uint16_t abs;
};

struct PjdDevMark {
    uint32_t lane;
    uint32_t ent_off;
    uint16_t acc[3];
    uint16_t pad_;
};

static inline __host__ __device__ uint64_t pjd_pack_state(uint32_t p, uint32_t c, uint32_t z)
{
    return (uint64_t)p | ((uint64_t)c << 32) | ((uint64_t)z << 40);
}

static inline __host__ __device__ void pjd_resize_tap_calc(uint32_t sn, uint32_t dn, uint32_t i, uint32_t &i0, uint32_t &i1, uint32_t &w)
{
    const uint32_t d2 = 2u * dn;
    if ((uint64_t)sn * dn < (1ull << 31)) {
        const uint32_t a = (2u * i + 1u) * sn;
        uint32_t X = a > dn ? a - dn : 0u;
        const uint32_t hi = d2 * (sn - 1u);
        X = X < hi ? X : hi;
        i0 = X / d2;
        w = ((X - i0 * d2) * 256u + dn) / d2;
    } else {
        const uint64_t a = (uint64_t)(2u * i + 1u) * sn;
        uint64_t X = a > dn ? a - dn : 0u;
        const uint64_t hi = (uint64_t)d2 * (sn - 1u);
        X = X < hi ? X : hi;
        i0 = (uint32_t)(X / d2);
        w = (uint32_t)(((X - (uint64_t)i0 * d2) * 256u + dn) / d2);
    }
    i1 = i0 + 1u < sn ? i0 + 1u : sn - 1u;
}

#define PJD_RS_PX    4
#define PJD_RS_COLS  (64 * PJD_RS_PX)
#define PJD_RS_ROWS  8
#define PJD_RS_WAVES 4
struct PjdDevResize {
    uint64_t src_off;
    uint64_t dst_off;
    uint32_t sw, sh, src_stride;
    uint32_t tw, th;
    uint32_t col_tiles;
};

static inline __host__ __device__ uint32_t pjd_resize_aa_taps_calc(uint32_t sn, uint32_t dn, uint32_t i, uint32_t &first, uint32_t *q)
{
    const int64_t S2 = 2 * (int64_t)(sn > dn ? sn : dn), c = (int64_t)(2u * i + 1u) * sn, d2 = 2 * (int64_t)dn;
    const int64_t lo = c - S2;
    first = lo < (int64_t)dn ? 0u : (uint32_t)((lo - dn) / d2) + 1u;
    uint32_t n = 0, best = 0;
    uint64_t R = 0;
    for (int64_t p = (2 * (int64_t)first + 1) * dn; n < 32u && first + n < sn && p < c + S2; p += d2, n++) {
        const int64_t dist = p > c ? p - c : c - p;
        q[n] = (uint32_t)(S2 - dist);
        R += q[n];
        if (q[n] > q[best]) best = n;
    }
    int64_t rest = 65536;
    for (uint32_t k = 0; k < n; k++) {
        q[k] = (uint32_t)(((uint64_t)q[k] * 65536u + R / 2u) / R);
        rest -= q[k];
    }
    q[best] = (uint32_t)((int64_t)q[best] + rest);
    return n;
}

static inline uint32_t pjd_resize_bicubic_taps_calc(uint32_t sn, uint32_t dn, uint32_t i, uint32_t &first, int32_t *q)
{
    const int64_t T = 2 * (int64_t)(sn > dn ? sn : dn), c = (int64_t)(2u * i + 1u) * sn, d2 = 2 * (int64_t)dn;
    const int64_t lo = c - 2 * T;
    first = lo < (int64_t)dn ? 0u : (uint32_t)((lo - dn) / d2) + 1u;
    int64_t r[64], R = 0;
    uint32_t n = 0, best = 0;
    for (int64_t p = (2 * (int64_t)first + 1) * dn; n < 64u && first + n < sn && p < c + 2 * T; p += d2, n++) {
        const int64_t D = p > c ? p - c : c - p;
        r[n] = D < T ? 3 * D * D * D - 5 * T * D * D + 2 * T * T * T : -D * D * D + 5 * T * D * D - 8 * T * T * D + 4 * T * T * T;
        R += r[n];
        if (r[n] > r[best]) best = n;
    }
    int64_t rest = 65536;
    for (uint32_t k = 0; k < n; k++) {
        const __int128 num = (__int128)r[k] * 131072 + R, den = 2 * (__int128)R;
        __int128 v = num / den;
        if (num % den < 0) v--;
        q[k] = (int32_t)v;
        rest -= q[k];
    }
    q[best] = (int32_t)(q[best] + rest);
    return n;
}

struct PjdDevResizeAA {
    uint32_t x_tab, x_taps;
    uint32_t y_tab, y_taps;
};

static inline __host__ __device__ uint32_t pjd_resize_aa_lds(uint32_t span, bool planar, uint32_t nc = 3u) { return planar ? nc * ((span + 6u) & ~3u) : (3u * span + 6u) & ~3u; }

struct PjdDevResizeWin {
    uint32_t x, y, w, h;
    uint32_t vw, vh;
    uint32_t ox, oy;
    uint32_t flags;
    uint32_t pad_;
};

#define PJD_RWI_XMIRROR   1u
#define PJD_RWI_YMIRROR   2u
#define PJD_RWI_TRANSPOSE 4u
static inline uint32_t pjd_orient_tvh(uint32_t o)
{
    static const uint8_t tvh[8] = {0, 1, 3, 2, 4, 5, 7, 6};
    return tvh[(o - 1u) & 7u];
}
static inline uint32_t pjd_orient_flags(uint32_t o)
{
    const uint32_t b = pjd_orient_tvh(o), t = b >> 2, v = (b >> 1) & 1u, h = b & 1u;
    return t ? PJD_RWI_TRANSPOSE | (v ? PJD_RWI_XMIRROR : 0u) | (h ? PJD_RWI_YMIRROR : 0u) : (h ? PJD_RWI_XMIRROR : 0u) | (v ? PJD_RWI_YMIRROR : 0u);
}

static inline __host__ __device__ PjdDevResizeWin pjd_resize_win_identity(const PjdDevResize &r)
{
    return PjdDevResizeWin{0, 0, r.sw, r.sh, r.tw, r.th, 0, 0, 0, 0};
}

static inline __host__ __device__ void pjd_resize_win_ends(const PjdDevResizeWin &w, uint32_t tw, uint32_t c0, uint32_t c1, uint32_t &lo, uint32_t &hi)
{
    const bool flip = (w.flags & 1u) != 0;
    lo = w.ox + (flip ? tw - 1u - c1 : c0);
    hi = w.ox + (flip ? tw - 1u - c0 : c1);
}

struct PjdDevResizePad {
    uint32_t W, H;
    uint32_t left, top;
    uint32_t cw, ch;
    uint32_t pad_[2];
};
struct PjdPadFill { uint32_t d[3]; };
static inline __host__ __device__ uint32_t pjd_pad_fill_dword(uint32_t p0, uint32_t p1, uint32_t p2, uint32_t j)
{
    const uint32_t m = j % 12u, q = m >> 2, sh = 8u * (m & 3u);
    const uint32_t lo = q == 0u ? p0 : q == 1u ? p1 : p2, hi = q == 0u ? p1 : q == 1u ? p2 : p0;
    return (uint32_t)((((uint64_t)hi << 32) | lo) >> sh);
}

static inline __host__ __device__ float pjd_normalize_f32(uint32_t v, float scale, float bias) { return __builtin_fmaf((float)v, scale, bias); }
// ... 82 lines not shown
```

### pim-jpeg-decoder_amd/csrc/pjd_k_huffman.hip

```cpp

#include "pjd_device_common.h"
#include "pjd_kernels.h"
#include "pjd_lut_build.h"
#include "../../include/pjd.h"

static_assert(sizeof(PjdDevHuffRaw) == 180, "raw table layout");
static_assert(PJD_LUT_BITS + PJD_L2_BITS == 16 && PJD_L1_BYTES == (4 << PJD_LUT_BITS), "two-level table geometry");
static_assert(PJD_HUFF_LANES == 64, "one wave per 64 lanes");
static_assert(PJD_STAGE_ENTRIES == PJD_GROUP && PJD_GROUP == 16, "a group (a head word + 7 step words) is what one flush of the staging buffer writes");

__global__ __launch_bounds__(256) void pjd_k_build_tables(PjdDevBatch B)
{
    const uint32_t ts = blockIdx.x / PJD_MAX_TABLES, slot = blockIdx.x % PJD_MAX_TABLES;
    const PjdDevTset &T = B.tsets[ts];
    if (slot >= T.n_tables || T.lut_bytes == 0) return;
    const PjdDevHuffRaw &r = B.raw_tables[(size_t)ts * PJD_MAX_TABLES + slot];
    uint16_t *blob = reinterpret_cast<uint16_t *>(B.luts + (size_t)T.lut_off16 * 16);
    uint32_t *L1 = reinterpret_cast<uint32_t *>(blob + slot * (PJD_L1_BYTES / 2));
    const uint32_t partner = r.is_ac ? slot : (uint32_t)T.pair_ac[slot];
    const bool has_partner = partner < T.n_tables;
    const PjdDevHuffRaw &r2 = B.raw_tables[(size_t)ts * PJD_MAX_TABLES + (has_partner ? partner : slot)];
    __shared__ uint32_t first[17], first2[17];
    __shared__ uint16_t cp[PJD_L2_BITS], ce[PJD_L2_BITS];
    const uint32_t tid = threadIdx.x;
// ... 622 lines not shown
    uint32_t col;
};

extern __shared__ __attribute__((aligned(16))) uint8_t pjd_huff_lds[];

struct WaveState { uint32_t p_img, cz, cnt; };

__device__ __forceinline__ bool wave_rounds(const PhaseCtx &P, const LaneGeom &g, const ChkCtx &K, WalkBuf &wb, WaveState &S, BCache &Bc, uint32_t changed,
                                            uint32_t ext_p, uint32_t ext_cz, bool ext_new, uint32_t &err_acc,
                                            unsigned long long *stats, int stat_base, uint32_t *rdbg)
{
    const uint32_t l = threadIdx.x & 63;
    for (int iter = 0; iter < PJD_SYNC_MAX_ITERS; iter++) {
#if PJD_TAIL_PRIO
        if (iter == 1) __builtin_amdgcn_s_setprio(2);
        if (iter == 4) __builtin_amdgcn_s_setprio(3);
#endif
        uint32_t pp = __shfl_up(S.p_img, 1), pcz = __shfl_up(S.cz, 1), pch = __shfl_up(changed, 1);
        if (l == 0) { pp = ext_p; pcz = ext_cz; pch = (ext_new && iter == 0) ? 1u : 0u; }
        const bool act = g.valid && !g.seg_first && pch != 0;
        const uint64_t act_mask = __ballot(act);
        if (!act_mask) return true;
        const uint64_t tr0 = rdbg ? __builtin_amdgcn_s_memrealtime() : 0;
        if ((uint32_t)__popcll(act_mask) <= K.walk_max) {
            uint64_t mask = act_mask;
            uint32_t walked = 0;
            const uint32_t chk_bits = rfl(K.chk_bits);
            const uint64_t can = __ballot(g.valid && !g.seg_first);
            while (mask) {
                uint32_t a = (uint32_t)__builtin_ctzll(mask);
                mask &= mask - 1;
                uint32_t ep = rfl(ext_p), ecz = rfl(ext_cz);
                if (a) { ep = (uint32_t)__builtin_amdgcn_readlane((int)S.p_img, (int)(a - 1)); ecz = (uint32_t)__builtin_amdgcn_readlane((int)S.cz, (int)(a - 1)); }
                for (;;) {
                    const uint32_t base = (uint32_t)__builtin_amdgcn_readlane((int)g.base_bit, (int)a);
                    const uint32_t endb = (uint32_t)__builtin_amdgcn_readlane((int)g.end_bit, (int)a);
                    uint32_t p = ep - base, c = ecz >> 8, z = ecz & 255u, ndu = 0, j;
                    uint32_t *st_col = K.state - l + a, *rem_col = K.rem - l + a;
                    const uint32_t Bst_a = (uint32_t)__builtin_amdgcn_readlane((int)Bc.st, (int)a);
                    uint32_t oa_st, oa_rem;
                    const int res = walk_lane(P, wb, l, base, p, c, z, endb, ndu, st_col, rem_col, chk_bits, j, Bst_a, oa_st, oa_rem);
                    walked++;
                    const uint32_t op = (uint32_t)__builtin_amdgcn_readlane((int)S.p_img, (int)a), ocz = (uint32_t)__builtin_amdgcn_readlane((int)S.cz, (int)a);
                    uint32_t np = p + base, ncz = (c << 8) | z;
                    if (res == SPAN_MERGED_B) {
                        const uint32_t Brem_a = (uint32_t)__builtin_amdgcn_readlane((int)Bc.rem, (int)a);
                        np = (uint32_t)__builtin_amdgcn_readlane((int)Bc.p, (int)a); ncz = (uint32_t)__builtin_amdgcn_readlane((int)Bc.cz, (int)a);
                        ndu += Brem_a;
                        if (l == 0) { st_col[64] = Bst_a; rem_col[64] = Brem_a; st_col[128] = 0xffffffffu; st_col[192] = 0xffffffffu; }
                    } else if (l == 0) for (uint32_t i = 1; i < j; i++) rem_col[i * 64] = ndu - rem_col[i * 64];
                    if (l == a) {
                        S.cnt = ndu;
                        if (oa_st != 0xffffffffu || res == SPAN_MERGED_B) { Bc.st = oa_st; Bc.rem = oa_rem; Bc.p = op; Bc.cz = ocz; }
                    }
                    if (res == SPAN_MERGED || (np == op && ncz == ocz)) break;
                    if (l == a) { S.p_img = np; S.cz = ncz; }
                    if (a == 63) break;
                    if (!((can >> (a + 1)) & 1ull)) break;
                    a++; mask &= ~(1ull << a);
                    ep = np; ecz = ncz;
                }
            }
            if (stats && l == 0) { atomicAdd(stats + stat_base, 1ull); atomicAdd(stats + stat_base + 1, (unsigned long long)walked); atomicAdd(stats + PJD_STAT_WALKS, 1ull); atomicAdd(stats + PJD_STAT_WALKS + 1, (unsigned long long)walked); }
            if (rdbg && l == 0 && iter < 24) rdbg[iter] = ((0x80u | (walked & 0x7fu)) << 24) | ((uint32_t)(__builtin_amdgcn_s_memrealtime() - tr0) & 0xffffffu);
            return true;
        }
        if (stats && l == 0) { atomicAdd(stats + stat_base, 1ull); atomicAdd(stats + stat_base + 1, (unsigned long long)__popcll(act_mask)); }
        changed = 0;
        if (act) {
            uint32_t p = pp - g.base_bit, c = pcz >> 8, z = pcz & 255, ndu = 0, j, oa_st, oa_rem;
            const int res = sync_span<true>(P, g.words, g.col, p, c, z, g.end_bit, ndu, K, j, Bc.st, oa_st, oa_rem);
            const uint32_t op = S.p_img, ocz = S.cz;
            if (res == SPAN_MERGED_B) {
                ndu += Bc.rem;
                K.state[64] = Bc.st; K.rem[64] = Bc.rem; K.state[128] = 0xffffffffu; K.state[192] = 0xffffffffu;
                if (Bc.p != S.p_img || Bc.cz != S.cz) { S.p_img = Bc.p; S.cz = Bc.cz; changed = 1; }
            } else {
                chk_finish(K, j, ndu);
                if (res != SPAN_MERGED) {
                    const uint32_t np = p + g.base_bit, ncz = (c << 8) | z;
                    if (np != S.p_img || ncz != S.cz) { S.p_img = np; S.cz = ncz; changed = 1; }
                }
            }
            S.cnt = ndu;
            if (oa_st != 0xffffffffu || res == SPAN_MERGED_B) { Bc.st = oa_st; Bc.rem = oa_rem; Bc.p = op; Bc.cz = ocz; }
        }
        if (rdbg && l == 0 && iter < 24) rdbg[iter] = ((uint32_t)__popcll(act_mask) << 24) | ((uint32_t)(__builtin_amdgcn_s_memrealtime() - tr0) & 0xffffffu);
    }
    return !__any(changed != 0);
}

__device__ __forceinline__ void seg_combine(uint32_t av, uint32_t af, uint32_t &bv, uint32_t &bf, uint32_t cap)
{
    if (!bf) { const uint32_t t = bv + av; bv = t < cap ? t : cap; }
    bf |= af;
}

__device__ __forceinline__ void wave_seg_scan(uint32_t &v, uint32_t &f, uint32_t cap)
{
    const uint32_t lane = threadIdx.x & 63;
    for (int off = 1; off < 64; off <<= 1) {
        const uint32_t ov = __shfl_up(v, off), of = __shfl_up(f, off);
        if ((int)lane >= off) seg_combine(ov, of, v, f, cap);
    }
}

#define OP_FLAG        (1ull << 63)
#define OP_ST_AGG      (1ull << 62)
#define OP_ST_PFX      (2ull << 62)
#define OP_ST_MASK     (3ull << 62)
#define OP_POISON      (1ull << 61)
#define OP_HEAD        (1ull << 60)
#define OP_SPIN_LIMIT  (1u << 22)

__device__ __forceinline__ uint64_t op_load(const uint64_t *p) { return __hip_atomic_load(p, __ATOMIC_RELAXED, __HIP_MEMORY_SCOPE_AGENT); }
__device__ __forceinline__ void op_store(uint64_t *p, uint64_t v) { __hip_atomic_store(p, v, __ATOMIC_RELAXED, __HIP_MEMORY_SCOPE_AGENT); }

__device__ __forceinline__ uint64_t op_desc(uint64_t status, uint32_t v, uint32_t f, bool poison)
{
    return status | (poison ? OP_POISON : 0ull) | (f ? OP_HEAD : 0ull) | (uint64_t)(v & 0x0fffffffu);
}

__device__ __forceinline__ uint64_t readfirstlane_u64(uint64_t v)
{
    const uint32_t lo = (uint32_t)__builtin_amdgcn_readfirstlane((int)(uint32_t)v);
    const uint32_t hi = (uint32_t)__builtin_amdgcn_readfirstlane((int)(uint32_t)(v >> 32));
    return ((uint64_t)hi << 32) | lo;
}

__device__ __forceinline__ uint64_t op_wait_flag(const uint64_t *p, bool &timeout)
{
    uint64_t v = 0;
    if ((threadIdx.x & 63) == 0)
        for (uint32_t it = 0; it < OP_SPIN_LIMIT; it++) {
            v = op_load(p);
            if (v & OP_FLAG) break;
            __builtin_amdgcn_s_sleep(8);
        }
    v = readfirstlane_u64(v);
    timeout = timeout || !(v & OP_FLAG);
    return v & ~OP_FLAG;
}

#ifndef PJD_HUFF_OCC
#define PJD_HUFF_OCC 0
#endif
#if PJD_HUFF_OCC
#define PJD_HUFF_OCC_ATTR __attribute__((amdgpu_waves_per_eu(PJD_HUFF_OCC, PJD_HUFF_OCC)))
#else
#define PJD_HUFF_OCC_ATTR
#endif
__global__ __launch_bounds__(PJD_HUFF_THREADS) PJD_HUFF_OCC_ATTR void pjd_k_huff_lanes(PjdDevBatch B, uint32_t hwg_base, uint32_t *__restrict__ ticket)
{
    const uint32_t t = threadIdx.x, l = t & 63, wi = t >> 6;
    uint8_t *lds = pjd_huff_lds;
    uint8_t *areas = lds + B.max_lut_bytes;
    uint8_t *phase_tabs = areas + PJD_HUFF_WAVES * PJD_WAVE_LDS;
    uint32_t *tick = reinterpret_cast<uint32_t *>(phase_tabs + PJD_HUFF_WAVES * PJD_PHASE_LDS);
    if (t == 0) *tick = hwg_base + atomicAdd(ticket, 1u);
    __syncthreads();
    const uint32_t gidx = rfl(*tick);
    const PjdDevHuffWg wg = B.hwgs[gidx];
    {
        const PjdDevTset &T = B.tsets[wg.tset];
        const uint32_t n16 = T.lut_bytes / 16;
        const uint4 *tsrc = reinterpret_cast<const uint4 *>(B.luts) + T.lut_off16;
        uint4 *tdst = reinterpret_cast<uint4 *>(lds);
        for (uint32_t i0 = t; i0 < n16; i0 += 4 * PJD_HUFF_THREADS) {
            const uint32_t i1 = i0 + PJD_HUFF_THREADS, i2 = i1 + PJD_HUFF_THREADS, i3 = i2 + PJD_HUFF_THREADS;
            uint4 v0 = tsrc[i0], v1, v2, v3;
            if (i1 < n16) v1 = tsrc[i1];
            if (i2 < n16) v2 = tsrc[i2];
            if (i3 < n16) v3 = tsrc[i3];
            tdst[i0] = v0;
            if (i1 < n16) tdst[i1] = v1;
            if (i2 < n16) tdst[i2] = v2;
            if (i3 < n16) tdst[i3] = v3;
        }
    }
    const bool wave_on = wi < wg.n_waves;
    const uint32_t w = wg.first_wave + (wave_on ? wi : 0u);
    const PjdDevHuffWave hw = B.hwaves[w];
    const PjdDevImage &im = B.images[hw.image];
    PhaseCtx P;
    {
        const uint32_t nl = rfl(im.n_luma), dus = rfl(im.dus_per_mcu), nc = dus - nl;
        const uint32_t c1 = nc >= 1 ? 1u : 0u, c2 = nc >= 2 ? 2u : c1;
        const uint32_t lb = lds_abs(lds);
        P.lbase = lb;
        P.tY  = rfl((lb + (uint32_t)im.tbl_slot[0][0] * PJD_L1_BYTES) | (lb + (uint32_t)im.tbl_slot[0][1] * PJD_L1_BYTES) << 16);
        P.tC1 = rfl((lb + (uint32_t)im.tbl_slot[c1][0] * PJD_L1_BYTES) | (lb + (uint32_t)im.tbl_slot[c1][1] * PJD_L1_BYTES) << 16);
        P.tC2 = rfl((lb + (uint32_t)im.tbl_slot[c2][0] * PJD_L1_BYTES) | (lb + (uint32_t)im.tbl_slot[c2][1] * PJD_L1_BYTES) << 16);
        P.nc = nc; P.dus1 = dus - 1;
        P.xbase = lds_abs(phase_tabs) + wi * PJD_PHASE_LDS;
    }
    const uint32_t dus = P.dus1 + 1;
    P.build(l);
    __syncthreads();
    if (!wave_on) return;

    const uint64_t ts0 = B.dbg ? __builtin_amdgcn_s_memrealtime() : 0;
    const uint64_t tc0 = B.dbg ? __builtin_amdgcn_s_memtime() : 0;
    uint64_t *genA = B.wave_gen, *genB = B.wave_gen + B.n_hwave;
    LaneGeom g;
    g.valid = l < hw.n_lanes;
    g.q = hw.first_lane + l;
    g.seg_first = g.seg_last = false;
    g.seg = 0; g.end_bit = g.seg_end_bit = g.base_bit = 0;
    g.words = (pjd_gptr)readfirstlane_u64((uint64_t)(B.words + (size_t)w * B.word_rows * 64));
    g.col = l * 4;
    uint32_t seg_first_du = 0, seg_n_du = 0;
    const uint32_t sub_bytes = rfl(im.sub_bytes);
    if (g.valid) {
        const PjdDevSub sb = B.lanes[g.q];
        g.seg = sb.seg & 0x7fffffffu;
        g.seg_first = (sb.seg >> 31) != 0;
        const PjdDevSegment sg = B.segs[g.seg];
        const uint32_t end_byte = sb.byte_start + sub_bytes < sg.byte_end ? sb.byte_start + sub_bytes : sg.byte_end;
        g.seg_last = end_byte == sg.byte_end;
        g.base_bit = sb.byte_start * 8;
        g.end_bit = (end_byte - sb.byte_start) * 8;
        g.seg_end_bit = (sg.byte_end - sb.byte_start) * 8;
        seg_first_du = sg.first_du; seg_n_du = sg.n_du;
    }
    uint32_t *area = reinterpret_cast<uint32_t *>(areas + wi * PJD_WAVE_LDS);
    ChkCtx K;
    K.state = area + l;
    K.rem = area + PJD_NCHK * 64 + l;
    K.chk_bits = sub_bytes * 8 / PJD_NCHK;
    K.walk_max = rfl(im.walk_max);
    for (int j = 0; j < PJD_NCHK; j++) { K.state[j * 64] = 0xffffffffu; K.rem[j * 64] = 0; }
    const bool first_is_head = __shfl((uint32_t)g.seg_first, 0) != 0;
    const uint32_t last_lane = hw.n_lanes - 1;
    bool dead = false;
    uint32_t flag = 0;

    WaveState S;
    {
        uint32_t p = 0, c = 0, z = 0, ndu = 0, j = 1;
        if (g.valid) {
            uint32_t oa, orem;
            sync_span<false>(P, g.words, g.col, p, c, z, g.end_bit, ndu, K, j, 0xffffffffu, oa, orem);
            chk_finish(K, j, ndu);
        }
        S.p_img = p + g.base_bit; S.cz = (c << 8) | z; S.cnt = ndu;
    }
    if (l == last_lane) op_store(genA + w, pjd_pack_state(S.p_img, S.cz >> 8, S.cz & 255) | OP_FLAG);
    const uint64_t ts1 = B.dbg ? __builtin_amdgcn_s_memrealtime() : 0;

    uint64_t entry_used = 0;
    uint32_t err_acc = 0;
    bool ok = true;
    WalkBuf wb;
    wb.ecs = (pjd_gptr)readfirstlane_u64((uint64_t)(B.ecs + im.ecs_off));
    wb.clamp = rfl(im.ecs_len) + 40u;
    wb.cb = 0; wb.cw = 0; wb.cn = 0; wb.have = 0;
    if (!first_is_head) entry_used = op_wait_flag(genA + w - 1, dead);
    BCache Bc;
    Bc.st = 0xffffffffu; Bc.rem = 0; Bc.p = 0; Bc.cz = 0;
    ok = wave_rounds(P, g, K, wb, S, Bc, g.valid ? 1u : 0u, (uint32_t)entry_used,
                     (((uint32_t)(entry_used >> 32) & 255) << 8) | ((uint32_t)(entry_used >> 40) & 255), !first_is_head && !dead,
                     err_acc, B.stats, 0, B.dbg ? B.dbg + (size_t)w * 32 + 8 : nullptr);
    if (l == last_lane) op_store(genB + w, pjd_pack_state(S.p_img, S.cz >> 8, S.cz & 255) | OP_FLAG);
    const uint64_t ts2 = B.dbg ? __builtin_amdgcn_s_memrealtime() : 0;

    for (uint32_t gen = 1; gen + 1 < PJD_GENS; gen++) {
        if (!first_is_head && !dead) {
            const uint64_t truth = op_wait_flag(B.wave_gen + (size_t)gen * B.n_hwave + w - 1, dead);
            if (!dead && truth != entry_used) {
                entry_used = truth;
                ok = wave_rounds(P, g, K, wb, S, Bc, 0u, (uint32_t)truth,
                                 (((uint32_t)(truth >> 32) & 255) << 8) | ((uint32_t)(truth >> 40) & 255), true,
                                 err_acc, B.stats, 2, nullptr) && ok;
            }
        }
        if (l == last_lane) op_store(B.wave_gen + (size_t)(gen + 1) * B.n_hwave + w, pjd_pack_state(S.p_img, S.cz >> 8, S.cz & 255) | OP_FLAG);
    }
    if (!ok) flag |= 1u << PJD_FLAG_NOSYNC;
    const uint64_t ts3 = B.dbg ? __builtin_amdgcn_s_memrealtime() : 0;

    const uint32_t du_cap = rfl(im.n_du) + 1;
    uint32_t cnt = 0, v = 0, f = 0;
    if (g.valid) {
        cnt = S.cnt;
        v = cnt < du_cap ? cnt : du_cap;
        if (g.seg_first) { f = 1; v = seg_first_du + v < du_cap ? seg_first_du + v : du_cap; }
    }
    wave_seg_scan(v, f, du_cap);
    const uint32_t agg_v = __shfl(v, 63), agg_f = __shfl(f, 63);
    uint32_t du_in = 0;
    if (w == im.hwave_base) {
        if (l == 0) op_store(B.wave_desc + w, op_desc(OP_ST_PFX, agg_v, agg_f, dead));
    } else {
        if (l == 0) op_store(B.wave_desc + w, op_desc(OP_ST_AGG, agg_v, agg_f, dead));
        uint32_t rv = 0, rf = 0;
        bool poison = false;
        int hi = (int)w - 1;
        for (;;) {
            const int j = hi - (int)l;
            const bool inside = j >= (int)im.hwave_base;
            uint64_t d = OP_ST_PFX;
            if (inside) {
                uint32_t it = 0;
                do { d = op_load(B.wave_desc + j); if (d & OP_ST_MASK) break; __builtin_amdgcn_s_sleep(8); } while (++it < OP_SPIN_LIMIT);
            }
            const bool ready = (d & OP_ST_MASK) != 0;
            if (__any(!ready)) { dead = true; break; }
            const uint64_t pfx_mask = __ballot((d & OP_ST_MASK) == OP_ST_PFX);
            const int k = pfx_mask ? __builtin_ctzll(pfx_mask) : 64;
            const bool use = (int)l <= k;
            uint32_t xv = use ? (uint32_t)d & 0x0fffffffu : 0u, xf = use ? (uint32_t)((d >> 60) & 1u) : 0u;
            poison = poison || __any(use && (d & OP_POISON));
            for (int off = 1; off < 64; off <<= 1) {
                const uint32_t ov = __shfl_down(xv, off), of = __shfl_down(xf, off);
                if ((int)l + off < 64) seg_combine(ov, of, xv, xf, du_cap);
            }
            const uint32_t wvv = __shfl(xv, 0), wf = __shfl(xf, 0);
            { uint32_t nv = rv, nf = rf; seg_combine(wvv, wf, nv, nf, du_cap); rv = nv; rf = nf; }
            if (k < 64) break;
            hi -= 64;
        }
        if (poison) dead = true;
        du_in = rv;
        uint32_t iv = agg_v, ifl = agg_f;
        seg_combine(rv, rf, iv, ifl, du_cap);
        if (l == 0) op_store(B.wave_desc + w, op_desc(OP_ST_PFX, iv, ifl, dead));
    }
    const uint64_t ts4 = B.dbg ? __builtin_amdgcn_s_memrealtime() : 0;

    const uint32_t prev_p = __shfl_up(S.p_img, 1), prev_cz = __shfl_up(S.cz, 1);
    const uint32_t prev_v = __shfl_up(v, 1), prev_f = __shfl_up(f, 1);
    uint32_t npair = 0;
    PjdDevLaneInfo li;
    li.n_ent = 0; li.first_du = g.seg_first ? PJD_LANE_SEG_FIRST : 0u; li.dc_sum[0] = li.dc_sum[1] = li.dc_sum[2] = 0; li.pad_ = 0;
    if (g.valid && !dead) {
        uint32_t D;
        if (g.seg_first) D = seg_first_du;
        else if (l == 0) D = du_in;
        else if (prev_f) D = prev_v;
        else D = du_in + prev_v < du_cap ? du_in + prev_v : du_cap;
        const uint32_t D_in = D, D_end = seg_first_du + seg_n_du;
        uint32_t p, c, z;
        if (g.seg_first) { p = 0; c = 0; z = 0; }
        else {
            if (l == 0) { p = (uint32_t)entry_used - g.base_bit; c = (uint32_t)(entry_used >> 32) & 255; z = (uint32_t)(entry_used >> 40) & 255; }
            else { p = prev_p - g.base_bit; c = prev_cz >> 8; z = prev_cz & 255; }
            if (D_in < D_end && (D_in % dus) != c) flag |= 1u << PJD_FLAG_SEGMENT;
        }
        if (D_in < D_end && !flag) {
            OutCtx O;
            O.region = B.ent + im.ent_base + (size_t)(g.q - im.lane_base) * im.lane_cap;
            O.stage = area + l;
            O.cap = im.lane_cap;
            O.n = 0; O.npair = 0; O.dcA = 0; O.dcB = 0; O.overflow = 0;
            O.ru = im.idct_mcus * dus;
            O.marks = B.marks + im.iwg_base;
            O.lane_q = g.q;
            O.D_in = D_in;
            li.first_du |= D_in;
            {
                const uint32_t first_du = im.first_mcu * dus;
                const uint32_t d_next = (z == 0) ? D_in : D_in + 1;
                const uint32_t k = (d_next - first_du + O.ru - 1) / O.ru;
                O.mark_next = k;
                O.mark_D = first_du + k * O.ru;
            }
            uint32_t err = 0;
            const uint32_t p0 = p, c0 = c, z0 = z, mark_next0 = O.mark_next, mark_D0 = O.mark_D;
            write_span(P, g.words, g.col, p, c, z, g.end_bit, err, D, D_end, O);
            li.n_ent = O.n;
            npair = O.npair;
            li.dc_sum[0] = (uint16_t)O.dcA; li.dc_sum[1] = (uint16_t)(O.dcA >> 16); li.dc_sum[2] = (uint16_t)O.dcB;
            const bool has_next = g.seg + 1 < im.seg_base + im.n_seg;
            const bool last_seg = !has_next && (im.flags & PJD_IF_ENDS_STREAM) != 0;
            const bool eof_lane = g.seg_last && last_seg;
            const bool eof_crossed = last_seg && !g.seg_last && p > g.seg_end_bit;
            bool settled = false;
            if (err || (eof_lane && (D < D_end || p > g.seg_end_bit)) || eof_crossed) {
                Careful R;
                R.marks = O.marks; R.mark_next = mark_next0; R.mark_D = mark_D0; R.ru = O.ru; R.lane_q = g.q;
                careful_span(P, g.words, g.col, p0, c0, z0, g.end_bit, (eof_lane || eof_crossed) ? g.seg_end_bit : 0xffffffffu, eof_lane,
                             D_in, D_end, O.region, O.cap, R);
                li.n_ent = R.n;
                npair = 0;
                li.dc_sum[0] = (uint16_t)R.dcA; li.dc_sum[1] = (uint16_t)(R.dcA >> 16); li.dc_sum[2] = (uint16_t)R.dcB;
                if (R.ovf) flag |= 1u << PJD_FLAG_OVERFLOW;
                else if (R.cls) {
                    const unsigned long long key = ((unsigned long long)(g.base_bit + R.p_err) << 32) | ((unsigned long long)R.D_err << 4) | (R.cls << 1) | R.in_dc;
                    atomicMin(&B.imstate[hw.image].err_key, key);
                    settled = true;
                }
            }
            if (!settled) {
                if (err) flag |= 1u << PJD_FLAG_SYMBOL;
                if (O.overflow) flag |= 1u << PJD_FLAG_OVERFLOW;
                if (D == D_end) {
                    if (p > g.seg_end_bit) flag |= 1u << PJD_FLAG_SEGMENT;
                    if (has_next && ((p + 7) & ~7u) != g.seg_end_bit) flag |= 1u << PJD_FLAG_SEGMENT;
                    if (last_seg && !flag) atomicMin(&B.imstate[hw.image].end_pos, g.base_bit + p);
                } else {
                    if (S.p_img - g.base_bit != p || (S.cz >> 8) != c || (S.cz & 255) != z) flag |= 1u << PJD_FLAG_VERIFY;
                    if (D - D_in != S.cnt) flag |= 1u << PJD_FLAG_VERIFY;
                    if (g.seg_last) flag |= 1u << PJD_FLAG_SEGMENT;
                }
            }
        }
    }
    if (g.valid) B.lane_info[g.q] = li;
    if (!first_is_head && !dead) {
        const uint64_t fin = op_wait_flag(B.wave_gen + (size_t)(PJD_GENS - 1) * B.n_hwave + w - 1, dead);
        if (fin != entry_used) flag |= 1u << PJD_FLAG_STITCH;
    }
    if (B.dbg && l == 0) {
        const uint64_t ts5 = __builtin_amdgcn_s_memrealtime();
        uint32_t *d = B.dbg + (size_t)w * 32;
        d[0] = (uint32_t)ts0; d[1] = (uint32_t)(ts1 - ts0); d[2] = (uint32_t)(ts2 - ts1); d[3] = (uint32_t)(ts3 - ts2);
        d[4] = (uint32_t)(ts4 - ts3); d[5] = (uint32_t)(ts5 - ts4); d[6] = hw.image; d[7] = hw.n_lanes;
        d[7] |= ((uint32_t)(((__builtin_amdgcn_s_memtime() - tc0) * 16) / ((ts5 - ts0) ? (ts5 - ts0) : 1)) & 0xffffffu) << 8;
    }
    if (dead) flag |= 1u << PJD_FLAG_TIMEOUT;
    uint32_t wflag = flag, went = npair, wsteps = g.valid ? li.n_ent / 2 - (li.n_ent + PJD_GROUP - 1) / PJD_GROUP : 0, wpos = (flag && g.valid) ? g.base_bit : 0xffffffffu;
    uint32_t wfill = g.valid ? (uint32_t)(((uint64_t)li.n_ent << 10) / im.lane_cap) : 0u;
    for (int off = 1; off < 64; off <<= 1) {
        wflag |= __shfl_xor(wflag, off); went += __shfl_xor(went, off); wsteps += __shfl_xor(wsteps, off);
        { const uint32_t o = __shfl_xor(wfill, off); wfill = o > wfill ? o : wfill; }
        const uint32_t o = __shfl_xor(wpos, off);
        wpos = o < wpos ? o : wpos;
    }
    if (l == 0) { atomicAdd(B.stats + PJD_STAT_ENTRIES, (unsigned long long)(went + wsteps)); atomicAdd(B.stats + PJD_STAT_STEPS, (unsigned long long)wsteps); atomicMax(B.stats + PJD_STAT_FILL, (unsigned long long)wfill); }
    if (wflag && l == 0) {
        atomicMin(&B.imstate[hw.image].flag_pos, wpos);
        for (int r = 0; r < PJD_FLAG_REASONS; r++)
            if (wflag & (1u << r)) atomicAdd(B.stats + PJD_STAT_FLAG0 + r, 1ull);
    }
}

struct SeqWin {
    pjd_gptr base;
    uint32_t hi, lo, nxt, off;
    int s;
    __device__ __forceinline__ uint32_t word(uint32_t byte_off) const
    {
        return __builtin_bswap32(reinterpret_cast<const __attribute__((address_space(1))) UnalignedU32 *>(base + byte_off)->v);
    }
    __device__ __forceinline__ void init(pjd_gptr b)
    {
        base = b; hi = 0; lo = word(0); nxt = word(4); off = 8; s = 0;
    }
    __device__ __forceinline__ uint32_t peek() const { return __builtin_amdgcn_alignbit(hi, lo, (uint32_t)s); }
    __device__ __forceinline__ void drop(uint32_t n)
    {
        s -= (int)n;
        if (s < 0) { s += 32; hi = lo; lo = nxt; nxt = word(off); off += 4; }
    }
};

__global__ __launch_bounds__(64) void pjd_k_huff_exact_lut(PjdDevBatch B, const uint32_t *__restrict__ image_list, const uint64_t *__restrict__ dense_base)
{
    const uint32_t ii = image_list[blockIdx.x];
    const PjdDevImage &im = B.images[ii];
    if (im.flags & PJD_IF_PROGRESSIVE) return;
    const PjdDevTset &T = B.tsets[im.tset];
    if (T.lut_bytes == 0) return;
    const uint32_t l = threadIdx.x;
    uint8_t *lds = pjd_huff_lds;
    {
        const uint4 *tsrc = reinterpret_cast<const uint4 *>(B.luts) + T.lut_off16;
        uint4 *tdst = reinterpret_cast<uint4 *>(lds);
        for (uint32_t i = l; i < T.lut_bytes / 16; i += 64) tdst[i] = tsrc[i];
    }
    PhaseCtx P;
    {
        const uint32_t dus = im.dus_per_mcu, nc = dus - im.n_luma;
        const uint32_t c1 = nc >= 1 ? 1u : 0u, c2 = nc >= 2 ? 2u : c1;
        const uint32_t lb = lds_abs(lds);
        P.lbase = lb;
        P.tY  = (lb + (uint32_t)im.tbl_slot[0][0] * PJD_L1_BYTES) | (lb + (uint32_t)im.tbl_slot[0][1] * PJD_L1_BYTES) << 16;
        P.tC1 = (lb + (uint32_t)im.tbl_slot[c1][0] * PJD_L1_BYTES) | (lb + (uint32_t)im.tbl_slot[c1][1] * PJD_L1_BYTES) << 16;
        P.tC2 = (lb + (uint32_t)im.tbl_slot[c2][0] * PJD_L1_BYTES) | (lb + (uint32_t)im.tbl_slot[c2][1] * PJD_L1_BYTES) << 16;
        P.nc = nc; P.dus1 = dus - 1;
        P.xbase = 0;
    }
    __syncthreads();
    if (l != 0) return;

    int16_t *coef = B.coef + dense_base[blockIdx.x] * 64;
    const uint32_t RI = im.restart_interval, Wr = im.ref_mcu_w_real;
    const bool std_rule = (im.flags & PJD_IF_STANDARD_RESTART) != 0;
    const uint32_t nbits = im.ecs_len * 8u;
    SeqWin w;
    w.init((pjd_gptr)(B.ecs + im.ecs_off));
    uint32_t p = 0, D = 0;
    int pred[3] = {0, 0, 0};
    int status = PJD_ST_OK;
    for (uint32_t m = im.first_mcu; m < im.last_mcu && !status; m++) {
        const uint32_t y = (m / im.mcux) * im.vs, x = (m % im.mcux) * im.hs;
        if (RI != 0 && (std_rule ? (m % RI == 0) : ((y * Wr + x) % RI == 0))) {
            pred[0] = pred[1] = pred[2] = 0;
            if ((p >> 3) < im.ecs_len && (p & 7)) { const uint32_t a = 8u - (p & 7); w.drop(a); p += a; }
        }
        for (uint32_t k = 0; k < im.dus_per_mcu && !status; k++, D++) {
            const uint32_t r = P.dus1 - k, comp = P.comp(r), tabs = P.tabs(r);
            int16_t *unit = coef + (size_t)D * 64;
            {
                const uint32_t pk = w.peek();
                const uint32_t e = lut_lookup(P.lbase, tabs & 0xffffu, pk);
                const uint32_t used = PJD_LUT_USED(e), size = PJD_LUT_SIZE(e);
                const uint32_t vbits = size >= PJD_LUT_BADSYM ? 0u : size, codelen = used - vbits, left = nbits > p ? nbits - p : 0u;
                if (size == PJD_LUT_BADSYM || codelen > left) { status = PJD_ST_DC_SYM; break; }
                if (size == PJD_LUT_BADLEN) { status = PJD_ST_DC_LEN; break; }
                if (vbits > left - codelen) { status = PJD_ST_DC_BITS; break; }
                const uint32_t bits = __builtin_amdgcn_ubfe(pk, 32u - used, size), m1 = 1u << size;
                const int val = (int)bits + ((((int)bits - (int)(m1 >> 1)) >> 31) & (int)(1u - m1));
                w.drop(used); p += used;
                unit[0] = (int16_t)(val + pred[comp]);
                pred[comp] = unit[0];
            }
            for (uint32_t z = 1; z < 64; z++) {
                const uint32_t pk = w.peek();
                const uint32_t e = lut_lookup(P.lbase, tabs >> 16, pk);
                const uint32_t used = PJD_LUT_USED(e), size = PJD_LUT_SIZE(e), adv = PJD_LUT_ADV(e);
                const uint32_t vbits = size >= PJD_LUT_BADSYM ? 0u : size, codelen = used - vbits, left = nbits > p ? nbits - p : 0u;
                if (size == PJD_LUT_BADSYM || codelen > left) { status = PJD_ST_AC_SYM; break; }
                if (e & PJD_LUT_EOB) { w.drop(used); p += used; break; }
                const uint32_t run = (adv - 1u) & 15u;
                if (z + run >= 64) { status = PJD_ST_AC_RUN; break; }
                z += run;
                if (size == PJD_LUT_BADLEN) { status = PJD_ST_AC_LEN; break; }
                if (vbits > left - codelen) { status = PJD_ST_AC_BITS; break; }
                const uint32_t bits = __builtin_amdgcn_ubfe(pk, 32u - used, size), m1 = 1u << size;
                const int val = (int)bits + ((((int)bits - (int)(m1 >> 1)) >> 31) & (int)(1u - m1));
                w.drop(used); p += used;
                unit[z] = (size == 0 && z == 52) ? (int16_t)PJD_COEF_SENTINEL : (int16_t)val;
            }
        }
    }
    B.status[ii] = (B.status[ii] & PJD_STW_NEEDS_EXACT) | status;
}

void pjd_launch_huff_exact_lut(hipStream_t s, const PjdDevBatch &b, const uint32_t *image_list, const uint64_t *dense_base, uint32_t n)
{
    if (n == 0 || b.max_lut_bytes == 0) return;
    hipLaunchKernelGGL(pjd_k_huff_exact_lut, dim3(n), dim3(64), (size_t)b.max_lut_bytes + 64, s, b, image_list, dense_base);
}

static size_t huff_lds_bytes(const PjdDevBatch &b)
{
    return (size_t)b.max_lut_bytes + PJD_HUFF_WAVES * (PJD_WAVE_LDS + PJD_PHASE_LDS) + 16;
}

void pjd_launch_build_tables(hipStream_t s, const PjdDevBatch &b)
{
    if (b.n_tsets == 0) return;
    hipLaunchKernelGGL(pjd_k_build_tables, dim3(b.n_tsets * PJD_MAX_TABLES), dim3(256), 0, s, b);
}
void pjd_launch_lane_words(hipStream_t s, const PjdDevBatch &b)
{
    if (b.n_hwave) hipLaunchKernelGGL(pjd_k_lane_words, dim3(b.n_hwave), dim3(256), 0, s, b);
}
void pjd_launch_huff_lanes(hipStream_t s, const PjdDevBatch &b)
{
    if (b.n_hwg) hipLaunchKernelGGL(pjd_k_huff_lanes, dim3(b.n_hwg), dim3(PJD_HUFF_THREADS), huff_lds_bytes(b), s, b, 0u, b.ticket);
}
hipError_t pjd_huff_lanes_occupancy(const PjdDevBatch &b, int *workgroups_per_cu, size_t *lds_bytes)
{
    *lds_bytes = huff_lds_bytes(b);
    return hipOccupancyMaxActiveBlocksPerMultiprocessor(workgroups_per_cu, pjd_k_huff_lanes, PJD_HUFF_THREADS, *lds_bytes);
}
void pjd_launch_huff_lanes_group(hipStream_t s, const PjdDevBatch &b, const PjdDevGroup &g, uint32_t group_index)
{
    if (g.hwg_count) hipLaunchKernelGGL(pjd_k_huff_lanes, dim3(g.hwg_count), dim3(PJD_HUFF_THREADS), huff_lds_bytes(b), s, b, g.hwg_first, b.ticket + 2 + 2 * group_index);
}
```

### pim-jpeg-decoder_amd/csrc/pjd_kernels.h

```cpp
#pragma once
#include <hip/hip_runtime.h>
#include <stdint.h>

#include "pjd_internal.h"

struct PjdDevBatch {
    const PjdDevImage *images;
    const PjdDevTset *tsets;
    const PjdDevHuffRaw *raw_tables;
    uint8_t *luts;
    const uint16_t *qtab;
    const PjdDevSegment *segs;
    const PjdDevSub *lanes;
    const PjdDevHuffWave *hwaves;
    const PjdDevHuffWg *hwgs;
    const PjdDevIdctWg *iwgs;
    const PjdDevScan *pscans;
    const uint32_t *group_images;
    const uint32_t *iwg_order;
    const uint8_t *ecs;
    uint32_t *words;
    int16_t *coef;
    uint16_t *ent;
    PjdDevLaneInfo *lane_info;
    PjdDevLaneDc *lane_dc;
    uint16_t *dc_blk;
    PjdDevMark *marks;
    uint8_t *out;
    int32_t *status;
    PjdDevImState *imstate;
    uint64_t *wave_gen;
    uint64_t *wave_desc;
    uint32_t *ticket;
    uint32_t *dbg;
    unsigned long long *stats;
    uint32_t n_images, n_tsets, n_lanes, n_hwave, n_hwg, n_iwg, n_dcblk;
    uint32_t sub_bytes;
    uint32_t word_rows;
    uint32_t lane_cap;
    uint32_t max_lut_bytes;
};

void pjd_launch_dpu_payload(hipStream_t s, const uint32_t *metadata, int16_t *mcus, int n_dpus);
void pjd_launch_zero(hipStream_t s, void *p, size_t bytes);
void pjd_launch_reset(hipStream_t s, const PjdDevBatch &b, const int32_t *status_init, uint64_t *opstate, size_t opstate_words, uint32_t dbg_words);
enum PjdBackLayout : uint8_t { PJD_BACK_INTERLEAVED = 0, PJD_BACK_PLANAR = 1, PJD_BACK_GRAY = 2 };
struct PjdBackForm {
    PjdBackLayout layout;
    bool scaled;
    bool planes() const { return layout != PJD_BACK_INTERLEAVED; }
    bool gray() const { return layout == PJD_BACK_GRAY; }
};
void pjd_launch_idct_lanes(hipStream_t s, const PjdDevBatch &b, PjdBackForm f, const uint32_t *order, uint32_t n_wg);
void pjd_launch_idct_dense(hipStream_t s, const PjdDevBatch &b, PjdBackForm f, const PjdDevIdctWg *wgs, const uint64_t *dense_base, uint32_t n_wg);
void pjd_launch_lane_dc_scan(hipStream_t s, const PjdDevBatch &b, bool per_picture);
void pjd_launch_group_dc(hipStream_t s, const PjdDevBatch &b, const PjdDevGroup &g);
void pjd_launch_idct_std_lanes(hipStream_t s, const PjdDevBatch &b, PjdBackForm f, const uint32_t *order, uint32_t n_wg, uint32_t n_red, uint8_t *planes);
void pjd_launch_idct_std_dense(hipStream_t s, const PjdDevBatch &b, PjdBackForm f, const PjdDevIdctWg *wgs, const uint64_t *dense_base, uint32_t n_wg, uint32_t n_red,
                               uint8_t *planes);
void pjd_launch_colour_std(hipStream_t s, const PjdDevBatch &b, const PjdDevIdctWg *cwgs, uint32_t n_wg, uint32_t n_red, uint8_t *planes);
struct PjdResizeLaunch {
    const uint8_t *src;
    uint8_t *dst;
    const PjdDevResize *recs;
    const uint32_t *tile_prefix;
    uint32_t n_images, n_tiles;
    bool planar;
    PjdNormalize norm;
    const PjdDevResizeWin *win;
    bool oriented;
    int filter;
    const PjdDevResizeAA *aa;
    const uint32_t *tab;
    uint32_t lds_bytes;
    const PjdDevResizePad *pad;
    uint32_t channels = 3;
    const PjdDevColour *colour = nullptr;
};
void pjd_launch_resize(hipStream_t s, const PjdResizeLaunch &a);
struct PjdBorderLaunch {
    uint8_t *dst;
    const PjdDevResize *recs;
    const PjdDevResizePad *pad;
    const uint32_t *line_prefix;
    uint32_t n_images, n_lines;
    bool planar;
    uint32_t elem_bytes;
    PjdPadFill fill;
    uint32_t channels = 3;
};
void pjd_launch_resize_border(hipStream_t s, const PjdBorderLaunch &a);
struct PjdWarpLaunch {
    const uint8_t *src;
    uint8_t *dst;
    const PjdDevResize *recs;
    const PjdDevWarp *warp;
    const uint32_t *tile_prefix;
    uint32_t n_images, n_tiles;
    bool planar;
    PjdNormalize norm;
    uint32_t fill;
    uint32_t channels = 3;
    const PjdDevColour *colour = nullptr;
};
void pjd_launch_warp(hipStream_t s, const PjdWarpLaunch &a);
struct PjdBlurLaunch {
    const uint8_t *src;
    uint8_t *dst;
    const PjdDevBlur *recs;
    const uint32_t *tile_prefix;
    const uint32_t *taps;
    uint32_t n_images, n_tiles;
    bool planar;
    PjdNormalize norm;
    uint32_t channels = 3;
    uint32_t lds_bytes = 0;
};
void pjd_launch_blur(hipStream_t s, const PjdBlurLaunch &a);
void pjd_launch_coefdump_lanes(hipStream_t s, const PjdDevBatch &b, uint32_t image, uint32_t n_iwg, int16_t *out);
void pjd_launch_coefdump_dense(hipStream_t s, const PjdDevBatch &b, uint32_t image, const int16_t *scratch, uint32_t first_du, uint32_t n_du, int16_t *out);
void pjd_launch_huff_sequential(hipStream_t s, const PjdDevBatch &b, const uint32_t *image_list, const uint64_t *dense_base, uint32_t n);
void pjd_launch_huff_exact_lut(hipStream_t s, const PjdDevBatch &b, const uint32_t *image_list, const uint64_t *dense_base, uint32_t n);
void pjd_launch_progressive(hipStream_t s, const PjdDevBatch &b, const uint32_t *image_list, const uint64_t *dense_base, uint32_t n);
void pjd_launch_build_tables(hipStream_t s, const PjdDevBatch &b);
void pjd_launch_lane_words(hipStream_t s, const PjdDevBatch &b);
void pjd_launch_huff_lanes(hipStream_t s, const PjdDevBatch &b);
hipError_t pjd_huff_lanes_occupancy(const PjdDevBatch &b, int *workgroups_per_cu, size_t *lds_bytes);
void pjd_launch_huff_lanes_group(hipStream_t s, const PjdDevBatch &b, const PjdDevGroup &g, uint32_t group_index);
```

### pim-jpeg-decoder_amd/csrc/pjd_plan.cpp

```cpp
#include "pjd_plan.h"
#include "pjd_lut_build.h"

#include <cstdio>
#include <cstring>
#include <algorithm>
#include <cstdlib>
#include <map>

namespace {

uint64_t align_up(uint64_t v, uint64_t a) { return (v + a - 1) / a * a; }

bool same_table(const pjd_huff_table &a, const pjd_huff_table &b)
{
    return std::memcmp(a.offsets, b.offsets, 17) == 0 && std::memcmp(a.symbols, b.symbols, 162) == 0;
}

std::string fmt(const char *f, int i, long a = 0, long b = 0)
{
    char buf[256];
    std::snprintf(buf, sizeof buf, f, i, a, b);
    return buf;
}

// ... 490 lines not shown
                P.hwgs.back().n_waves++;
                P.hwaves.push_back(w);
            }
            g.n_hwave = (uint32_t)P.hwaves.size() - g.hwave_base;
            P.fast_images.push_back((uint32_t)i);
        } else {
            P.seq_images.push_back((uint32_t)i);
        }

        g.image_index = (uint32_t)i;
        du_total += g.n_du;
        if (sequential) { g.dense_base = dense_seq; dense_seq += g.n_du; }
        g.idct_mcus = PJD_IDCT_MAX_DU / g.dus_per_mcu;
        const uint32_t lj_sl = (g.flags & PJD_IF_LJSCALE_MASK) >> PJD_IF_LJSCALE_SHIFT;
        std::vector<PjdDevIdctWg> &iwg_list = sequential ? (lj ? (lj_sl ? P.iwgs_dense_red : P.iwgs_dense_std) : P.iwgs_dense) : P.iwgs;
        g.iwg_base = (uint32_t)iwg_list.size();
        for (uint32_t m = g.first_mcu; m < g.last_mcu; m += g.idct_mcus) {
            PjdDevIdctWg w;
            w.image = (uint32_t)i;
            w.first_mcu = m;
            w.n_mcu = (g.last_mcu - m < g.idct_mcus) ? g.last_mcu - m : g.idct_mcus;
            w.pad_ = sequential ? (uint32_t)(P.seq_images.size() - 1) : 0;
            iwg_list.push_back(w);
        }
        g.n_iwg = (uint32_t)iwg_list.size() - g.iwg_base;
        if (lj && out_format != PJD_OUT_GRAY8) {
            g.plane_off256 = (uint32_t)(P.plane_bytes / 256);
            const uint32_t n = 8u >> lj_sl, cn = pjd_lj_chroma_size(n, g.hs, g.vs);
            const uint64_t ypl = (uint64_t)g.mcux * g.hs * n * g.mcuy * g.vs * n, cpl = (uint64_t)g.mcux * cn * g.mcuy * cn;
            P.plane_bytes = align_up(P.plane_bytes + ypl + (g.ncomp == 3 ? 2 * cpl : 0) + (lj_sl ? 8 : 0), 256);
            uint32_t ow = 0, oh = 0;
            pjd_scaled_dims(d.width, d.height, d.flags, &ow, &oh);
            const uint32_t items = ((ow + 3) / 4) * oh;
            std::vector<PjdDevIdctWg> &cl = lj_sl ? P.cwgs_red : P.cwgs_std;
            for (uint32_t it = 0; it < items; it += PJD_IDCT_THREADS) cl.push_back(PjdDevIdctWg{(uint32_t)i, it, 0, 0});
        }
        h.out_bytes = pjd_image_output_size(&d, out_format);
        g.out_off = out_off;
        out_off = align_up(out_off + h.out_bytes, 256);

        P.pixels += (uint64_t)d.width * d.height;
        P.ecs_bytes += d.ecs_len;
        P.out_bytes += h.out_bytes;
    }
    if (P.hwgs.size() > 1 && !std::getenv("PJD_KEEP_WG_ORDER")) {
        struct Unit { size_t first, count; double key; };
        std::vector<Unit> units;
        auto density = [&](uint32_t img) { const PjdDevImage &g = P.images[img]; return g.n_mcu ? (double)g.ecs_len / (double)(g.last_mcu - g.first_mcu ? g.last_mcu - g.first_mcu : 1) : 0.0; };
        for (size_t k = 0; k < P.hwgs.size(); k++) {
            const PjdDevHuffWg &w = P.hwgs[k];
            const uint32_t img_first = P.hwaves[w.first_wave].image, img_last = P.hwaves[w.first_wave + w.n_waves - 1].image;
            double key = 0;
            for (uint32_t im = img_first; im <= img_last; im++) key = std::max(key, density(im));
            const bool joins = !units.empty() && P.hwaves[P.hwgs[k - 1].first_wave + P.hwgs[k - 1].n_waves - 1].image == img_first;
            if (joins) { units.back().count++; units.back().key = std::max(units.back().key, key); }
            else units.push_back({k, 1, key});
        }
        std::stable_sort(units.begin(), units.end(), [](const Unit &a, const Unit &b) { return a.key > b.key; });
        std::vector<PjdDevHuffWg> ordered;
        ordered.reserve(P.hwgs.size());
        std::vector<size_t> unit_end;
        for (const Unit &u : units) {
            ordered.insert(ordered.end(), P.hwgs.begin() + (long)u.first, P.hwgs.begin() + (long)(u.first + u.count));
            unit_end.push_back(ordered.size());
        }
        P.hwgs.swap(ordered);
        uint32_t want = 3;
        std::vector<uint32_t> cuts_pct = {30, 65};
        if (const char *e = std::getenv("PJD_GROUPS")) { const int v = std::atoi(e); want = (uint32_t)(v < 1 ? 1 : (v > PJD_MAX_GROUPS ? PJD_MAX_GROUPS : v)); cuts_pct.clear(); }
        if (const char *e = std::getenv("PJD_GROUP_CUTS")) {
            cuts_pct.clear();
            bool ok = true;
            for (const char *q = e; ok;) {
                char *end = nullptr;
                const unsigned long v = std::strtoul(q, &end, 10);
                ok = end != q && v >= 1 && v <= 99 && (cuts_pct.empty() || v > cuts_pct.back());
                if (!ok) break;
                cuts_pct.push_back((uint32_t)v);
                for (q = end; *q == ' '; q++) {}
                if (!*q) break;
                ok = *q == ',';
                q++;
            }
            if (!ok) cuts_pct = {30, 65};
            want = (uint32_t)cuts_pct.size() + 1;
            if (want > PJD_MAX_GROUPS) { want = PJD_MAX_GROUPS; cuts_pct.resize(PJD_MAX_GROUPS - 1); }
        }
        if (cuts_pct.empty()) for (uint32_t k = 1; k < want; k++) cuts_pct.push_back(100u * k / want);
        bool small = P.fast_images.size() >= 64;
        for (uint32_t i : P.fast_images) if (P.images[i].n_lane > 8192) small = false;
        if (small && want > 1) {
            const size_t total_waves = P.hwaves.size();
            size_t h0 = 0, waves = 0;
            std::vector<char> seen(P.images.size(), 0);
            auto close_group = [&](size_t h1) {
                PjdDevGroup g;
                std::memset(&g, 0, sizeof g);
                g.hwg_first = (uint32_t)h0; g.hwg_count = (uint32_t)(h1 - h0);
                g.img_first = (uint32_t)P.group_images.size();
                g.iwg_first = (uint32_t)P.iwg_order.size();
                for (size_t k = h0; k < h1; k++)
                    for (uint32_t w = P.hwgs[k].first_wave; w < P.hwgs[k].first_wave + P.hwgs[k].n_waves; w++) {
                        const uint32_t im = P.hwaves[w].image;
                        if (seen[im]) continue;
                        seen[im] = 1;
                        P.group_images.push_back(im);
                        for (uint32_t q = 0; q < P.images[im].n_iwg; q++) P.iwg_order.push_back(P.images[im].iwg_base + q);
                    }
                g.img_count = (uint32_t)P.group_images.size() - g.img_first;
                g.iwg_count = (uint32_t)P.iwg_order.size() - g.iwg_first;
                P.groups.push_back(g);
                h0 = h1;
            };
            size_t pos = 0;
            for (size_t u = 0; u < unit_end.size(); u++) {
                for (; pos < unit_end[u]; pos++) waves += P.hwgs[pos].n_waves;
                const size_t k = P.groups.size();
                if (k + 1 < want && waves * 100 >= (size_t)cuts_pct[k] * total_waves && u + 1 < unit_end.size()) close_group(pos);
            }
            close_group(P.hwgs.size());
            if (P.groups.size() < 2) { P.groups.clear(); P.group_images.clear(); P.iwg_order.clear(); }
        }
    }
    if (P.libjpeg) {
        P.groups.clear(); P.group_images.clear(); P.iwg_order.clear();
        auto cls = [&](uint32_t image) { const uint32_t f = P.images[image].flags; return !(f & PJD_IF_LIBJPEG) ? 0 : ((f & PJD_IF_LJSCALE_MASK) ? 2 : 1); };
        for (int pass = 0; pass < 3; pass++)
            for (uint32_t k = 0; k < P.iwgs.size(); k++)
                if (cls(P.iwgs[k].image) == pass) P.iwg_order.push_back(k);
        for (const PjdDevIdctWg &w : P.iwgs) { const int c = cls(w.image); (c == 0 ? P.n_iwg_def : (c == 1 ? P.n_iwg_std : P.n_iwg_red))++; }
        P.n_dense_std = (uint32_t)P.iwgs_dense_std.size(); P.n_dense_red = (uint32_t)P.iwgs_dense_red.size();
        P.iwgs_dense_std.insert(P.iwgs_dense_std.end(), P.iwgs_dense_red.begin(), P.iwgs_dense_red.end());
        P.n_cwg_std = (uint32_t)P.cwgs_std.size(); P.n_cwg_red = (uint32_t)P.cwgs_red.size();
        P.cwgs_std.insert(P.cwgs_std.end(), P.cwgs_red.begin(), P.cwgs_red.end());
        if (P.plane_bytes >= (1ull << 40)) { err = "batch needs too large a plane buffer"; return PJD_E_ARG; }
    }
    P.ecs_buf_bytes = align_up(ecs_off + PJD_SUB_BYTES_MAX + 64, 256);
    P.n_du = du_total;
    P.sub_bytes = sb_max;
    if (P.min_sym_bits < 1 || P.tsets.empty()) P.min_sym_bits = 1;
    P.n_ent = ent_off + 16;
    P.n_words = (uint64_t)P.hwaves.size() * PJD_WORD_ROWS(sb_max) * 64;
    P.dense_du = dense_seq;
    P.out_buf_bytes = align_up(out_off, 256);
    P.n_dcblk = (P.subs.size() + PJD_DC_BLOCK - 1) / PJD_DC_BLOCK;
    {
        uint32_t max_lanes = 0;
        for (uint32_t i : P.fast_images) max_lanes = std::max(max_lanes, P.images[i].n_lane);
        P.dc_per_picture = max_lanes <= PJD_DC_PICTURE_MAX_LANES;
        if (const char *e = std::getenv("PJD_DC_FORM")) {
            if (!std::strcmp(e, "picture")) P.dc_per_picture = true;
            else if (!std::strcmp(e, "scan")) P.dc_per_picture = false;
        }
    }
    P.lut_buf_bytes = align_up(lut_off + 16, 256);
    if (P.ecs_buf_bytes >= (1ull << 40)) { err = "batch bitstream too large"; return PJD_E_ARG; }
    {
        const uint64_t reach = (uint64_t)PJD_WORD_ROWS(sb_max) * 4;
        for (const PjdDevImage &g : P.images)
            for (uint32_t q = g.lane_base; q < g.lane_base + g.n_lane; q++)
                if (g.ecs_off + P.subs[q].byte_start + reach > P.ecs_buf_bytes) { err = "internal: a Huffman lane would read past the bitstream buffer"; return PJD_E_ARG; }
    }
    if (P.subs.size() >= (1ull << 31) || P.n_ent >= (1ull << 40)) { err = "batch has too many Huffman lanes"; return PJD_E_ARG; }
    return PJD_OK;
}
```

### pim-jpeg-decoder_amd/csrc/pjd_plan.h

```cpp
#pragma once
#include <string>
#include <vector>

#include "../../include/pjd.h"
#include "pjd_internal.h"

struct PjdHostImage {
    const uint8_t *ecs_src;
    uint64_t ecs_copy_len;
    uint64_t out_bytes;
    bool shard;
    bool sequential;
};

struct PjdHostScan {
    const uint8_t *src;
    uint64_t len, off;
};

struct PjdPlan {
    int out_format = 0;
    uint32_t sub_bytes = 512;
    uint32_t min_sym_bits = 16;
    uint32_t lane_cap = 0;
    std::vector<PjdDevImage> images;
    std::vector<PjdHostImage> host;
    std::vector<PjdDevTset> tsets;
    std::vector<PjdDevHuffRaw> tables;
    std::vector<uint16_t> qtab;
    std::vector<PjdDevSegment> segs;
    std::vector<PjdDevSub> subs;
    std::vector<PjdDevHuffWave> hwaves;
    std::vector<PjdDevHuffWg> hwgs;
    std::vector<PjdDevIdctWg> iwgs;
    std::vector<PjdDevIdctWg> iwgs_dense;
    std::vector<PjdDevScan> pscans;
    std::vector<PjdHostScan> host_scans;
    std::vector<PjdDevGroup> groups;
    std::vector<uint32_t> group_images;
    std::vector<uint32_t> iwg_order;
    std::vector<uint32_t> seq_images;
    std::vector<uint32_t> fast_images;
    uint64_t ecs_buf_bytes = 0;
    uint64_t n_du = 0;
    uint64_t n_ent = 0;
    uint64_t n_words = 0;
    uint64_t dense_du = 0;
    uint64_t out_buf_bytes = 0;
    uint64_t n_dcblk = 0;
    uint64_t lut_buf_bytes = 0;
    uint32_t max_lut_bytes = 0;
    uint64_t pixels = 0, ecs_bytes = 0, out_bytes = 0;
    bool scaled = false;
    bool planar = false;
    bool gray = false;
    bool libjpeg = false;
    uint32_t n_iwg_def = 0, n_iwg_std = 0;
    std::vector<PjdDevIdctWg> iwgs_dense_std;
    std::vector<PjdDevIdctWg> cwgs_std;
    uint32_t n_iwg_red = 0, n_dense_std = 0, n_dense_red = 0, n_cwg_std = 0, n_cwg_red = 0;
    std::vector<PjdDevIdctWg> iwgs_dense_red, cwgs_red;
    uint64_t plane_bytes = 0;
    bool dc_per_picture = false;
    int plan_mode = 0;
    std::vector<uint32_t> tset_step_bits;
    std::vector<uint32_t> tset_nominal_bytes;
};

int pjd_make_plan(const pjd_image_desc *images, int n, int out_format, PjdPlan &plan, std::string &err,
                  uint32_t sub_bytes_override = 0, int plan_mode = 0);
```

### pim-jpeg-decoder_amd/python/pjd_amd/__init__.py

```python
import ctypes as C
import os

import numpy as np

_PKG = os.path.dirname(os.path.dirname(os.path.dirname(os.path.abspath(__file__))))
LIB_DIR = os.path.join(_PKG, "lib")
LIBPJD = os.path.join(LIB_DIR, "libpjd.so")
LIBHOST = os.path.join(LIB_DIR, "libpjdhost.so")
LIBPIPE = os.path.join(LIB_DIR, "libpjdpipe.so")

OUT_RGB8, OUT_BMP = 0, 1
OUT_RGB8_PLANAR = 2
OUT_GRAY8 = 4
PLAN_LATENCY, PLAN_THROUGHPUT = 0, 1
F_STANDARD_RESTART, F_FORCE_SEQUENTIAL, F_STANDARD_ZIGZAG, F_PROGRESSIVE = 1, 2, 4, 8
F_SCALE_1_2, F_SCALE_1_4, F_SCALE_1_8, F_SCALE_MASK = 16, 32, 48, 48
F_LIBJPEG_SCALE_1_2, F_LIBJPEG_SCALE_1_4, F_LIBJPEG_SCALE_1_8, F_LIBJPEG_SCALE_MASK = 128, 256, 384, 384
F_LIBJPEG = 64
RESIZE_BILINEAR, RESIZE_ANTIALIAS = 0, 1
RW_HFLIP = 1
AA_MAX_TAPS = 32
RESIZE_BICUBIC = 3
BICUBIC_MAX_TAPS = 64
BICUBIC_MAX_GAIN = 92681
# ... 286 lines not shown
        n = int(self.desc.ecs_len)
        if n == 0:
            return np.zeros(0, np.uint8)
        return np.ctypeslib.as_array(C.cast(self.desc.ecs, C.POINTER(C.c_uint8)), (n,)).copy()

    def seg_offsets(self):
        n = int(self.desc.n_segments)
        return np.ctypeslib.as_array(C.cast(self.desc.seg_offsets, C.POINTER(C.c_uint64)), (n,)).copy()

    def __del__(self):
        try:
            if getattr(self, "_h", None):
                host_lib().pjd_scanned_free(self._h)
                self._h = None
        except Exception:
            pass


def rgb_to_bmp(rgb: np.ndarray) -> bytes:
    h, w, _ = rgb.shape
    rgb = np.ascontiguousarray(rgb, np.uint8)
    out = np.zeros(26 + h * (3 * w + w % 4), np.uint8)
    host_lib().pjd_rgb_to_bmp(rgb.ctypes.data, w, h, out.ctypes.data)
    return out.tobytes()


class Context:

    def __init__(self, device: int = 0, plan_mode: int = None):
        L = dev_lib()
        h = C.c_void_p()
        rc = L.pjd_open(device, C.byref(h))
        if rc != 0:
            raise PjdError(f"pjd_open({device}) failed with {rc}: no usable gfx950 device")
        self._h = h
        self.L = L
        self.device = int(device)
        if plan_mode is not None:
            self.set_plan_mode(plan_mode)

    def set_plan_mode(self, mode: int):
        self._check(self.L.pjd_set_plan_mode(self._h, int(mode)), "pjd_set_plan_mode")

    def close(self):
        if self._h:
            self.L.pjd_close(self._h)
            self._h = None

    def _check(self, rc, what):
        if rc != 0:
            raise PjdError(f"{what} failed ({rc}): {self.L.pjd_last_error(self._h).decode()}")

    @property
    def stream(self):
        return self.L.pjd_stream(self._h)

    def batch(self, descs, out_format=OUT_RGB8):
        return Batch(self, descs, out_format)

    def decode(self, descs, out_format=OUT_RGB8):
        with self.batch(descs, out_format) as b:
            b.upload()
            b.decode()
            return b.download()

    def exec_dpu_payload(self, metadata: np.ndarray, mcus: np.ndarray):
        metadata = np.ascontiguousarray(metadata, np.uint32).reshape(-1, 276)
        assert mcus.dtype == np.int16 and mcus.flags.c_contiguous
        n = metadata.shape[0]
        assert mcus.size == n * 19200
        self._check(self.L.pjd_exec_dpu_payload(self._h, metadata.ctypes.data, mcus.ctypes.data, n), "pjd_exec_dpu_payload")
        return mcus


class Batch:
    def __init__(self, ctx: Context, descs, out_format):
        self.ctx, self.L = ctx, ctx.L
        self.n = len(descs)
        self.out_format = out_format
        arr = (ImageDesc * max(self.n, 1))()
        for i, d in enumerate(descs):
            C.memmove(C.byref(arr[i]), C.byref(d), C.sizeof(ImageDesc))
        self._descs = arr
        self._keep = descs
        h = C.c_void_p()
        ctx._check(self.L.pjd_batch_create(ctx._h, arr, self.n, out_format, C.byref(h)), "pjd_batch_create")
        self._h = h
        self._resize = None
        self.views = None
        self._dtype = None

    def __enter__(self):
        return self

    def __exit__(self, *a):
        self.destroy()

    def destroy(self):
        if self._h:
            self.L.pjd_batch_destroy(self._h)
            self._h = None

    @property
    def n_out(self):
        return self.n if self.views is None else len(self.views)

    def set_views(self, picture_of_view):
        views = [int(p) for p in picture_of_view]
        if any(not 0 <= p < 2 ** 32 for p in views):
            raise ValueError("set_views: picture indices must fit 32 bits")
        if len(views) >= 2 ** 32:
            raise ValueError("set_views: too many views")
        arr = (C.c_uint32 * max(len(views), 1))(*views)
        self.ctx._check(self.L.pjd_batch_set_views(self._h, arr, len(views)), "pjd_batch_set_views")
        self.views = views

    def upload(self):
        self.ctx._check(self.L.pjd_batch_upload(self._h), "pjd_batch_upload")

    def decode(self):
        self.ctx._check(self.L.pjd_batch_decode(self._h), "pjd_batch_decode")

    def decode_timed(self):
        t = Timings()
        self.ctx._check(self.L.pjd_batch_decode_timed(self._h, C.byref(t)), "pjd_batch_decode_timed")
        return t.as_dict(), float(t.total_ms)

    def capture(self):
        self.ctx._check(self.L.pjd_batch_capture(self._h), "pjd_batch_capture")

    def sync(self):
        self.ctx._check(self.L.pjd_batch_sync(self._h), "pjd_batch_sync")

    def decode_chains(self):
        self.L.pjd_batch_decode_chains.restype = C.c_int32
        self.L.pjd_batch_decode_chains.argtypes = [C.c_void_p]
        n = int(self.L.pjd_batch_decode_chains(self._h))
        if n < 0:
            self.ctx._check(n, "pjd_batch_decode_chains")
        return n

    def info(self):
        bi = BatchInfo()
        self.ctx._check(self.L.pjd_batch_get_info(self._h, C.byref(bi)), "pjd_batch_get_info")
        return {k: (list(getattr(bi, k)) if k == "flag_waves" else (float(getattr(bi, k)) if k == "exact_fallback_ms" else int(getattr(bi, k)))) for k, _ in bi._fields_}

    def huff_occupancy(self):
        self.L.pjd_batch_huff_occupancy.restype = C.c_int32
        self.L.pjd_batch_huff_occupancy.argtypes = [C.c_void_p, C.POINTER(C.c_int32), C.POINTER(C.c_uint32)]
        n, lds = C.c_int32(), C.c_uint32()
        self.ctx._check(self.L.pjd_batch_huff_occupancy(self._h, C.byref(n), C.byref(lds)), "pjd_batch_huff_occupancy")
        return int(n.value), int(lds.value)

    def output_size(self, i):
        return int(self.L.pjd_batch_output_size(self._h, i))

    def device_output(self, i):
        return self.L.pjd_batch_device_output(self._h, i)

    def output_offset(self, i):
        return int(self.L.pjd_batch_output_offset(self._h, i))

    def packed_size(self):
        return int(self.L.pjd_batch_packed_size(self._h))

    def output_shape(self, i):
        d = self._descs[i if self.views is None else self.views[i]]
        if self._resize is not None:
            h, w = self._resize[i]
        else:
            w, h = scaled_dims(d.width, d.height, d.flags)
        if self.out_format == OUT_RGB8:
            return (h, w, 3)
        if self.out_format == OUT_RGB8_PLANAR:
            return (3, h, w)
        if self.out_format == OUT_GRAY8:
            return (h, w)
        return (self.output_size(i),)

    def set_resize(self, sizes):
        if len(sizes) != self.n_out:
            raise ValueError("set_resize: one (h, w) per picture (per view after set_views)")
        sizes = [(int(h), int(w)) for h, w in sizes]
        for h, w in sizes:
            if not (0 <= h < 2 ** 32 and 0 <= w < 2 ** 32):
                raise ValueError("set_resize: sizes must fit 32 bits")
        ws = (C.c_uint32 * max(self.n_out, 1))(*[w for _, w in sizes])
        hs = (C.c_uint32 * max(self.n_out, 1))(*[h for h, _ in sizes])
        self.ctx._check(self.L.pjd_batch_set_resize(self._h, ws, hs), "pjd_batch_set_resize")
        self._resize = sizes

    def set_resize_pad(self, pads, fill=(0, 0, 0)):
        if len(pads) != self.n_out:
            raise ValueError("set_resize_pad: one pad (or None) per picture (per view after set_views)")
        if len(fill) != 3 or any(not 0 <= int(v) <= 255 or int(v) != v for v in fill):
            raise ValueError("set_resize_pad: the fill is three bytes (R, G, B)")
        arr = (ResizePad * max(self.n_out, 1))()
        for i, p in enumerate(pads):
            if p is not None:
                arr[i] = resize_pad(p)
        fl = (C.c_uint8 * 3)(*[int(v) for v in fill])
        self.ctx._check(self.L.pjd_batch_set_resize_pad(self._h, arr, fl), "pjd_batch_set_resize_pad")

    def set_pad_value(self, values):
        if len(values) != 3:
            raise ValueError("set_pad_value: three values (R, G, B)")
        va = (C.c_float * 3)(*[float(v) for v in values])
        self.ctx._check(self.L.pjd_batch_set_pad_value(self._h, va), "pjd_batch_set_pad_value")

    def set_orientation(self, orientations):
        if len(orientations) != self.n_out:
            raise ValueError("set_orientation: one orientation per picture (per view after set_views)")
        vals = [int(o) for o in orientations]
        if any(not 0 <= o <= 255 for o in vals):
            raise ValueError("set_orientation: orientations are 1..8")
        arr = (C.c_uint8 * max(self.n_out, 1))(*vals)
        self.ctx._check(self.L.pjd_batch_set_orientation(self._h, arr), "pjd_batch_set_orientation")

    def set_resize_window(self, windows):
        if len(windows) != self.n_out:
            raise ValueError("set_resize_window: one window (or None) per picture (per view after set_views)")
        arr = (ResizeWindow * max(self.n_out, 1))()
        for i, w in enumerate(windows):
            if w is not None:
                arr[i] = resize_window(w)
        self.ctx._check(self.L.pjd_batch_set_resize_window(self._h, arr), "pjd_batch_set_resize_window")

    def set_resize_affine(self, matrices, fill=(0, 0, 0)):
        if len(matrices) != self.n_out:
            raise ValueError("set_resize_affine: one matrix of six values per picture (per view after set_views)")
        if len(fill) != 3 or any(not 0 <= int(v) <= 255 or int(v) != v for v in fill):
            raise ValueError("set_resize_affine: the fill is three bytes (R, G, B)")
        arr = ((C.c_double * 6) * max(self.n_out, 1))()
        for i, m in enumerate(matrices):
            arr[i] = _affine6(m, "set_resize_affine")
        fl = (C.c_uint8 * 3)(*[int(v) for v in fill])
        self.ctx._check(self.L.pjd_batch_set_resize_affine(self._h, arr, fl), "pjd_batch_set_resize_affine")

    def set_colour(self, matrices):
        if len(matrices) != self.n_out:
            raise ValueError("set_colour: one matrix of twelve values (or None) per picture (per view after set_views)")
        arr = ((C.c_double * 12) * max(self.n_out, 1))()
        for i, m in enumerate(matrices):
            arr[i] = _colour12(COLOUR_IDENTITY if m is None else m, "set_colour")
        self.ctx._check(self.L.pjd_batch_set_colour(self._h, arr), "pjd_batch_set_colour")

    def set_blur(self, blurs):
        if len(blurs) != self.n_out:
            raise ValueError("set_blur: one (ksize, sigma) (or None) per picture (per view after set_views)")
        arr = (Blur * max(self.n_out, 1))()
        for i, e in enumerate(blurs):
            arr[i] = Blur(0.0, 0, 0) if e is None else Blur(float(e[1]), int(e[0]), 0)
        self.ctx._check(self.L.pjd_batch_set_blur(self._h, arr), "pjd_batch_set_blur")

    def set_resize_filter(self, filter):
        self.ctx._check(self.L.pjd_batch_set_resize_filter(self._h, int(filter)), "pjd_batch_set_resize_filter")

    def set_normalize(self, dtype, scale, bias):
        if len(scale) != 3 or len(bias) != 3:
            raise ValueError("set_normalize: three scales and three biases (R, G, B)")
        sc = (C.c_float * 3)(*[float(v) for v in scale])
        bi = (C.c_float * 3)(*[float(v) for v in bias])
        self.ctx._check(self.L.pjd_batch_set_normalize(self._h, int(dtype), sc, bi), "pjd_batch_set_normalize")
        self._dtype = int(dtype)

    def bind_output(self, device_ptr, capacity, offsets=None):
        arr = None
        if offsets is not None:
            if len(offsets) != self.n_out:
                raise ValueError("bind_output: one offset per picture (per view after set_views)")
            arr = (C.c_uint64 * max(self.n_out, 1))(*[int(o) for o in offsets])
        self.ctx._check(self.L.pjd_batch_bind_output(self._h, C.c_void_p(int(device_ptr)), int(capacity), arr), "pjd_batch_bind_output")

    def statuses(self):
        st = (C.c_int32 * max(self.n, 1))()
        self.ctx._check(self.L.pjd_batch_download(self._h, None, st), "pjd_batch_download")
        return [int(st[i]) for i in range(self.n)]

    def download(self):
        outs = [np.zeros(self.output_size(i), np.uint8) for i in range(self.n_out)]
        ptrs = (C.c_void_p * max(self.n_out, 1))(*[o.ctypes.data for o in outs])
        st = (C.c_int32 * max(self.n, 1))()
        self.ctx._check(self.L.pjd_batch_download(self._h, ptrs, st), "pjd_batch_download")
        if self._dtype is not None:
            outs = [o.view({DT_F16: np.float16, DT_BF16: np.uint16, DT_F32: np.float32}[self._dtype]) for o in outs]
        outs = [o.reshape(self.output_shape(i)) for i, o in enumerate(outs)]
        return outs, [int(st[i]) for i in range(self.n)]


    def coefficients(self, i):
        d = self._descs[i]
        n = int(self.L.pjd_coefficients_size(d.width, d.height, d.h_samp, d.v_samp))
        out = np.zeros(n, np.int16)
        self.ctx._check(self.L.pjd_batch_download_coefficients(self._h, i, out.ctypes.data, n), "pjd_batch_download_coefficients")
        return out.reshape(-1, 19200)

    def download_packed(self):
        size = int(self.L.pjd_batch_packed_size(self._h))
        host = self.L.pjd_host_alloc(size)
        if not host:
            raise PjdError("pjd_host_alloc failed")
        try:
            st = (C.c_int32 * max(self.n, 1))()
            self.ctx._check(self.L.pjd_batch_download_packed(self._h, host, size, st), "pjd_batch_download_packed")
            whole = np.ctypeslib.as_array(C.cast(host, C.POINTER(C.c_uint8)), shape=(size,))
            outs = []
# ... 378 lines not shown
```

Before: 145,600.

## Split fused Huffman lanes kernel into sync and write kernels

The single Huffman decode kernel becomes two kernels from a shared body header. One performs the speculative sync rounds and prefix scan and records per-lane entry state in a new lane-record buffer. The other reads those records and writes the entropy output. The sync kernel is pinned to a fixed waves-per-EU target so that its register pressure and occupancy no longer depend on the heavier write path. The split is on by default for the non-grouped chain path, at the cost of an extra launch and a round trip of lane state through global memory.

```diff
diff --git a/include/pjd.h b/include/pjd.h
--- a/include/pjd.h
+++ b/include/pjd.h
@@ -240,6 +240,8 @@
 int  pjd_plan_step_bits(const pjd_image_desc *image, uint32_t *step_bits_x256);
 int  pjd_plan_luts(const pjd_image_desc *image, void *blob, uint64_t cap, uint32_t *real_bytes, uint32_t *nominal_bytes, uint8_t *slots);
 int  pjd_batch_huff_occupancy(pjd_batch *batch, int32_t *workgroups_per_cu, uint32_t *lds_bytes);
+int  pjd_batch_huff_split_occupancy(pjd_batch *batch, int32_t *sync_workgroups_per_cu, int32_t *write_workgroups_per_cu);
+int  pjd_batch_huff_form(pjd_batch *batch);
 
 void *pjd_host_alloc(uint64_t bytes);
 void pjd_host_free(void *p);
diff --git a/pim-jpeg-decoder_amd/csrc/pjd_api.hip b/pim-jpeg-decoder_amd/csrc/pjd_api.hip
--- a/pim-jpeg-decoder_amd/csrc/pjd_api.hip
+++ b/pim-jpeg-decoder_amd/csrc/pjd_api.hip
@@ -148,6 +148,7 @@
     uint64_t *d_seq_base = nullptr;
     int32_t *d_status_init = nullptr;
     uint64_t *d_opstate = nullptr;
+    PjdDevLaneRec *d_lane_rec = nullptr;
     size_t opstate_bytes = 0;
     uint8_t *d_in = nullptr, *h_in = nullptr;
     size_t in_bytes = 0, images_off = 0;
@@ -564,6 +565,7 @@
     TRY_RC(dev_alloc(b->dev.ent, (size_t)P.n_ent));
     TRY_RC(dev_alloc(b->dev.lane_info, P.subs.size()));
     TRY_RC(dev_alloc(b->dev.lane_dc, P.subs.size()));
+    TRY_RC(dev_alloc(b->d_lane_rec, P.subs.size()));
     TRY_RC(dev_alloc(b->dev.dc_blk, (size_t)P.n_dcblk * 8));
     TRY_RC(dev_alloc(b->dev.marks, P.iwgs.size()));
     TRY_RC(dev_alloc(b->dev.out, P.out_buf_bytes));
@@ -720,7 +722,7 @@
         for (size_t g = 0; g < ng; g++) {
             hipStream_t gs = g == 0 ? s : ctx->group_streams[g - 1];
             if (g) HIP_TRY(ctx, hipStreamWaitEvent(gs, ctx->fork_ev, 0));
-            pjd_launch_huff_lanes_group(gs, b->dev, P.groups[g], (uint32_t)g);
+            pjd_launch_huff_lanes_group(gs, b->dev, P.groups[g], (uint32_t)g, P.huff_split_groups ? b->d_lane_rec : nullptr);
             pjd_launch_group_dc(gs, b->dev, P.groups[g]);
             pjd_launch_idct_lanes(gs, b->dev, F, b->dev.iwg_order + P.groups[g].iwg_first, P.groups[g].iwg_count);
             if (g) { HIP_TRY(ctx, hipEventRecord(ctx->join_ev[g - 1], gs)); }
@@ -728,7 +730,7 @@
         for (size_t g = 1; g < ng; g++) HIP_TRY(ctx, hipStreamWaitEvent(s, ctx->join_ev[g - 1], 0));
     } else {
         if (parallel) {
-            pjd_launch_huff_lanes(s, b->dev);    kt.mark("huff_lanes");
+            pjd_launch_huff_lanes(s, b->dev, P.huff_split_chain ? b->d_lane_rec : nullptr);    kt.mark("huff_lanes");
             pjd_launch_lane_dc_scan(s, b->dev, P.dc_per_picture);  kt.mark("dc_scan");
             pjd_launch_idct_lanes(s, b->dev, F, P.libjpeg ? b->dev.iwg_order : nullptr, P.libjpeg ? P.n_iwg_def : b->dev.n_iwg);
             kt.mark(F.gray() ? "idct_gray" : "idct_colour");
@@ -1454,8 +1456,9 @@
 {
     int wg = 0;
     size_t lds = 0;
-    if (pjd_huff_lanes_occupancy(b->dev, &wg, &lds) == hipSuccess)
-        std::fprintf(stderr, "[pjd waves] pjd_k_huff_lanes: %zu B of LDS per workgroup, %d workgroups per CU\n", lds, wg);
+    int wg_sync = 0, wg_write = 0;
+    if (pjd_huff_lanes_occupancy(b->dev, &wg, &lds, &wg_sync, &wg_write) == hipSuccess)
+        std::fprintf(stderr, "[pjd waves] pjd_k_huff_lanes: %zu B of LDS per workgroup, %d workgroups per CU (pjd_k_huff_sync %d, pjd_k_huff_write %d)\n", lds, wg, wg_sync, wg_write);
     if (b->decoded) {
         const size_t nw = b->plan.hwaves.size();
         std::vector<uint32_t> d(nw * 32);
@@ -1603,6 +1606,24 @@
     return PJD_OK;
 }
 
+int pjd_batch_huff_split_occupancy(pjd_batch *b, int32_t *sync_workgroups_per_cu, int32_t *write_workgroups_per_cu)
+{
+    if (!b || !sync_workgroups_per_cu || !write_workgroups_per_cu) return PJD_E_ARG;
+    hipSetDevice(b->ctx->device);
+    int n = 0, ns = 0, nw = 0;
+    size_t lds = 0;
+    if (pjd_huff_lanes_occupancy(b->dev, &n, &lds, &ns, &nw) != hipSuccess) return PJD_E_HIP;
+    *sync_workgroups_per_cu = ns;
+    *write_workgroups_per_cu = nw;
+    return PJD_OK;
+}
+
+int pjd_batch_huff_form(pjd_batch *b)
+{
+    if (!b) return PJD_E_ARG;
+    return (b->plan.huff_split_chain ? 1 : 0) | (b->plan.huff_split_groups ? 2 : 0);
+}
+
 uint64_t pjd_batch_output_size(pjd_batch *b, int image)
 {
     if (!b || image < 0 || (size_t)image >= b->n_out()) return 0;
diff --git a/pim-jpeg-decoder_amd/csrc/pjd_internal.h b/pim-jpeg-decoder_amd/csrc/pjd_internal.h
--- a/pim-jpeg-decoder_amd/csrc/pjd_internal.h
+++ b/pim-jpeg-decoder_amd/csrc/pjd_internal.h
@@ -221,6 +221,15 @@
 };
 #define PJD_LANE_SEG_FIRST 0x80000000u
 
+struct alignas(8) PjdDevLaneRec {
+    uint32_t p;
+    uint32_t czf;
+    uint32_t d_in;
+    uint32_t exit_p, exit_cz, cnt;
+};
+#define PJD_REC_SKIP       0x80000000u
+#define PJD_REC_FLAG_SHIFT 16
+
 struct PjdDevLaneDc {
     uint16_t dc_in[3];
     uint16_t abs;
diff --git a/pim-jpeg-decoder_amd/csrc/pjd_k_huff_body.h b/pim-jpeg-decoder_amd/csrc/pjd_k_huff_body.h
--- /dev/null
+++ b/pim-jpeg-decoder_amd/csrc/pjd_k_huff_body.h
@@ -0,0 +1,340 @@
+    const uint32_t t = threadIdx.x, l = t & 63, wi = t >> 6;
+    uint8_t *lds = pjd_huff_lds;
+    uint8_t *areas = lds + B.max_lut_bytes;
+    uint8_t *phase_tabs = areas + PJD_HUFF_WAVES * PJD_WAVE_LDS;
+#if PJD_HB_SYNC
+    uint32_t *tick = reinterpret_cast<uint32_t *>(phase_tabs + PJD_HUFF_WAVES * PJD_PHASE_LDS);
+    if (t == 0) *tick = hwg_base + atomicAdd(ticket, 1u);
+    __syncthreads();
+    const uint32_t gidx = rfl(*tick);
+#else
+    const uint32_t gidx = hwg_base + blockIdx.x;
+#endif
+    const PjdDevHuffWg wg = B.hwgs[gidx];
+    {
+        const PjdDevTset &T = B.tsets[wg.tset];
+        const uint32_t n16 = T.lut_bytes / 16;
+        const uint4 *tsrc = reinterpret_cast<const uint4 *>(B.luts) + T.lut_off16;
+        uint4 *tdst = reinterpret_cast<uint4 *>(lds);
+        for (uint32_t i0 = t; i0 < n16; i0 += 4 * PJD_HUFF_THREADS) {
+            const uint32_t i1 = i0 + PJD_HUFF_THREADS, i2 = i1 + PJD_HUFF_THREADS, i3 = i2 + PJD_HUFF_THREADS;
+            uint4 v0 = tsrc[i0], v1, v2, v3;
+            if (i1 < n16) v1 = tsrc[i1];
+            if (i2 < n16) v2 = tsrc[i2];
+            if (i3 < n16) v3 = tsrc[i3];
+            tdst[i0] = v0;
+            if (i1 < n16) tdst[i1] = v1;
+            if (i2 < n16) tdst[i2] = v2;
+            if (i3 < n16) tdst[i3] = v3;
+        }
+    }
+    const bool wave_on = wi < wg.n_waves;
+    const uint32_t w = wg.first_wave + (wave_on ? wi : 0u);
+    const PjdDevHuffWave hw = B.hwaves[w];
+    const PjdDevImage &im = B.images[hw.image];
+    PhaseCtx P;
+    {
+        const uint32_t nl = rfl(im.n_luma), dus = rfl(im.dus_per_mcu), nc = dus - nl;
+        const uint32_t c1 = nc >= 1 ? 1u : 0u, c2 = nc >= 2 ? 2u : c1;
+        const uint32_t lb = lds_abs(lds);
+        P.lbase = lb;
+        P.tY  = rfl((lb + (uint32_t)im.tbl_slot[0][0] * PJD_L1_BYTES) | (lb + (uint32_t)im.tbl_slot[0][1] * PJD_L1_BYTES) << 16);
+        P.tC1 = rfl((lb + (uint32_t)im.tbl_slot[c1][0] * PJD_L1_BYTES) | (lb + (uint32_t)im.tbl_slot[c1][1] * PJD_L1_BYTES) << 16);
+        P.tC2 = rfl((lb + (uint32_t)im.tbl_slot[c2][0] * PJD_L1_BYTES) | (lb + (uint32_t)im.tbl_slot[c2][1] * PJD_L1_BYTES) << 16);
+        P.nc = nc; P.dus1 = dus - 1;
+        P.xbase = lds_abs(phase_tabs) + wi * PJD_PHASE_LDS;
+    }
+    const uint32_t dus = P.dus1 + 1;
+    P.build(l);
+    __syncthreads();
+    if (!wave_on) return;
+
+#if PJD_HB_SYNC
+    const uint64_t ts0 = B.dbg ? __builtin_amdgcn_s_memrealtime() : 0;
+    const uint64_t tc0 = B.dbg ? __builtin_amdgcn_s_memtime() : 0;
+    uint64_t *genA = B.wave_gen, *genB = B.wave_gen + B.n_hwave;
+#endif
+    LaneGeom g;
+    g.valid = l < hw.n_lanes;
+    g.q = hw.first_lane + l;
+    g.seg_first = g.seg_last = false;
+    g.seg = 0; g.end_bit = g.seg_end_bit = g.base_bit = 0;
+    g.words = (pjd_gptr)readfirstlane_u64((uint64_t)(B.words + (size_t)w * B.word_rows * 64));
+    g.col = l * 4;
+    uint32_t seg_first_du = 0, seg_n_du = 0;
+    const uint32_t sub_bytes = rfl(im.sub_bytes);
+    if (g.valid) {
+        const PjdDevSub sb = B.lanes[g.q];
+        g.seg = sb.seg & 0x7fffffffu;
+        g.seg_first = (sb.seg >> 31) != 0;
+        const PjdDevSegment sg = B.segs[g.seg];
+        const uint32_t end_byte = sb.byte_start + sub_bytes < sg.byte_end ? sb.byte_start + sub_bytes : sg.byte_end;
+        g.seg_last = end_byte == sg.byte_end;
+        g.base_bit = sb.byte_start * 8;
+        g.end_bit = (end_byte - sb.byte_start) * 8;
+        g.seg_end_bit = (sg.byte_end - sb.byte_start) * 8;
+        seg_first_du = sg.first_du; seg_n_du = sg.n_du;
+    }
+    uint32_t *area = reinterpret_cast<uint32_t *>(areas + wi * PJD_WAVE_LDS);
+#if !PJD_HB_SYNC
+    uint32_t flag = 0;
+#else
+    ChkCtx K;
+    K.state = area + l;
+    K.rem = area + PJD_NCHK * 64 + l;
+    K.chk_bits = sub_bytes * 8 / PJD_NCHK;
+    K.walk_max = rfl(im.walk_max);
+    for (int j = 0; j < PJD_NCHK; j++) { K.state[j * 64] = 0xffffffffu; K.rem[j * 64] = 0; }
+    const bool first_is_head = __shfl((uint32_t)g.seg_first, 0) != 0;
+    const uint32_t last_lane = hw.n_lanes - 1;
+    bool dead = false;
+    uint32_t flag = 0;
+
+    WaveState S;
+    {
+        uint32_t p = 0, c = 0, z = 0, ndu = 0, j = 1;
+        if (g.valid) {
+            uint32_t oa, orem;
+            sync_span<false>(P, g.words, g.col, p, c, z, g.end_bit, ndu, K, j, 0xffffffffu, oa, orem);
+            chk_finish(K, j, ndu);
+        }
+        S.p_img = p + g.base_bit; S.cz = (c << 8) | z; S.cnt = ndu;
+    }
+    if (l == last_lane) op_store(genA + w, pjd_pack_state(S.p_img, S.cz >> 8, S.cz & 255) | OP_FLAG);
+    const uint64_t ts1 = B.dbg ? __builtin_amdgcn_s_memrealtime() : 0;
+
+    uint64_t entry_used = 0;
+    uint32_t err_acc = 0;
+    bool ok = true;
+    WalkBuf wb;
+    wb.ecs = (pjd_gptr)readfirstlane_u64((uint64_t)(B.ecs + im.ecs_off));
+    wb.clamp = rfl(im.ecs_len) + 40u;
+    wb.cb = 0; wb.cw = 0; wb.cn = 0; wb.have = 0;
+    if (!first_is_head) entry_used = op_wait_flag(genA + w - 1, dead);
+    BCache Bc;
+    Bc.st = 0xffffffffu; Bc.rem = 0; Bc.p = 0; Bc.cz = 0;
+    ok = wave_rounds(P, g, K, wb, S, Bc, g.valid ? 1u : 0u, (uint32_t)entry_used,
+                     (((uint32_t)(entry_used >> 32) & 255) << 8) | ((uint32_t)(entry_used >> 40) & 255), !first_is_head && !dead,
+                     err_acc, B.stats, 0, B.dbg ? B.dbg + (size_t)w * 32 + 8 : nullptr);
+    if (l == last_lane) op_store(genB + w, pjd_pack_state(S.p_img, S.cz >> 8, S.cz & 255) | OP_FLAG);
+    const uint64_t ts2 = B.dbg ? __builtin_amdgcn_s_memrealtime() : 0;
+
+    for (uint32_t gen = 1; gen + 1 < PJD_GENS; gen++) {
+        if (!first_is_head && !dead) {
+            const uint64_t truth = op_wait_flag(B.wave_gen + (size_t)gen * B.n_hwave + w - 1, dead);
+            if (!dead && truth != entry_used) {
+                entry_used = truth;
+                ok = wave_rounds(P, g, K, wb, S, Bc, 0u, (uint32_t)truth,
+                                 (((uint32_t)(truth >> 32) & 255) << 8) | ((uint32_t)(truth >> 40) & 255), true,
+                                 err_acc, B.stats, 2, nullptr) && ok;
+            }
+        }
+        if (l == last_lane) op_store(B.wave_gen + (size_t)(gen + 1) * B.n_hwave + w, pjd_pack_state(S.p_img, S.cz >> 8, S.cz & 255) | OP_FLAG);
+    }
+    if (!ok) flag |= 1u << PJD_FLAG_NOSYNC;
+    const uint64_t ts3 = B.dbg ? __builtin_amdgcn_s_memrealtime() : 0;
+
+    const uint32_t du_cap = rfl(im.n_du) + 1;
+    uint32_t cnt = 0, v = 0, f = 0;
+    if (g.valid) {
+        cnt = S.cnt;
+        v = cnt < du_cap ? cnt : du_cap;
+        if (g.seg_first) { f = 1; v = seg_first_du + v < du_cap ? seg_first_du + v : du_cap; }
+    }
+    wave_seg_scan(v, f, du_cap);
+    const uint32_t agg_v = __shfl(v, 63), agg_f = __shfl(f, 63);
+    uint32_t du_in = 0;
+    if (w == im.hwave_base) {
+        if (l == 0) op_store(B.wave_desc + w, op_desc(OP_ST_PFX, agg_v, agg_f, dead));
+    } else {
+        if (l == 0) op_store(B.wave_desc + w, op_desc(OP_ST_AGG, agg_v, agg_f, dead));
+        uint32_t rv = 0, rf = 0;
+        bool poison = false;
+        int hi = (int)w - 1;
+        for (;;) {
+            const int j = hi - (int)l;
+            const bool inside = j >= (int)im.hwave_base;
+            uint64_t d = OP_ST_PFX;
+            if (inside) {
+                uint32_t it = 0;
+                do { d = op_load(B.wave_desc + j); if (d & OP_ST_MASK) break; __builtin_amdgcn_s_sleep(8); } while (++it < OP_SPIN_LIMIT);
+            }
+            const bool ready = (d & OP_ST_MASK) != 0;
+            if (__any(!ready)) { dead = true; break; }
+            const uint64_t pfx_mask = __ballot((d & OP_ST_MASK) == OP_ST_PFX);
+            const int k = pfx_mask ? __builtin_ctzll(pfx_mask) : 64;
+            const bool use = (int)l <= k;
+            uint32_t xv = use ? (uint32_t)d & 0x0fffffffu : 0u, xf = use ? (uint32_t)((d >> 60) & 1u) : 0u;
+            poison = poison || __any(use && (d & OP_POISON));
+            for (int off = 1; off < 64; off <<= 1) {
+                const uint32_t ov = __shfl_down(xv, off), of = __shfl_down(xf, off);
+                if ((int)l + off < 64) seg_combine(ov, of, xv, xf, du_cap);
+            }
+            const uint32_t wvv = __shfl(xv, 0), wf = __shfl(xf, 0);
+            { uint32_t nv = rv, nf = rf; seg_combine(wvv, wf, nv, nf, du_cap); rv = nv; rf = nf; }
+            if (k < 64) break;
+            hi -= 64;
+        }
+        if (poison) dead = true;
+        du_in = rv;
+        uint32_t iv = agg_v, ifl = agg_f;
+        seg_combine(rv, rf, iv, ifl, du_cap);
+        if (l == 0) op_store(B.wave_desc + w, op_desc(OP_ST_PFX, iv, ifl, dead));
+    }
+    const uint64_t ts4 = B.dbg ? __builtin_amdgcn_s_memrealtime() : 0;
+#endif
+
+#if PJD_HB_SYNC
+    const uint32_t prev_p = __shfl_up(S.p_img, 1), prev_cz = __shfl_up(S.cz, 1);
+    const uint32_t prev_v = __shfl_up(v, 1), prev_f = __shfl_up(f, 1);
+#endif
+#if PJD_HB_WRITE
+    uint32_t npair = 0;
+    PjdDevLaneInfo li;
+    li.n_ent = 0; li.first_du = g.seg_first ? PJD_LANE_SEG_FIRST : 0u; li.dc_sum[0] = li.dc_sum[1] = li.dc_sum[2] = 0; li.pad_ = 0;
+#endif
+#if !PJD_HB_WRITE
+    PjdDevLaneRec rec;
+    rec.p = 0; rec.czf = PJD_REC_SKIP; rec.d_in = 0; rec.exit_p = S.p_img; rec.exit_cz = S.cz; rec.cnt = S.cnt;
+#endif
+#if !PJD_HB_SYNC
+    PjdDevLaneRec rec;
+    rec.p = 0; rec.czf = PJD_REC_SKIP; rec.d_in = 0; rec.exit_p = 0; rec.exit_cz = 0; rec.cnt = 0;
+    if (g.valid) rec = lane_rec[g.q];
+    struct { uint32_t p_img, cz, cnt; } S = {rec.exit_p, rec.exit_cz, rec.cnt};
+    if (g.valid && !(rec.czf & PJD_REC_SKIP)) {
+        uint32_t D = rec.d_in;
+        const uint32_t D_in = D, D_end = seg_first_du + seg_n_du;
+        uint32_t p = rec.p, c = rec.czf & 255u, z = (rec.czf >> 8) & 255u;
+#else
+    if (g.valid && !dead) {
+        uint32_t D;
+        if (g.seg_first) D = seg_first_du;
+        else if (l == 0) D = du_in;
+        else if (prev_f) D = prev_v;
+        else D = du_in + prev_v < du_cap ? du_in + prev_v : du_cap;
+        const uint32_t D_in = D, D_end = seg_first_du + seg_n_du;
+        uint32_t p, c, z;
+        if (g.seg_first) { p = 0; c = 0; z = 0; }
+        else {
+            if (l == 0) { p = (uint32_t)entry_used - g.base_bit; c = (uint32_t)(entry_used >> 32) & 255; z = (uint32_t)(entry_used >> 40) & 255; }
+            else { p = prev_p - g.base_bit; c = prev_cz >> 8; z = prev_cz & 255; }
+            if (D_in < D_end && (D_in % dus) != c) flag |= 1u << PJD_FLAG_SEGMENT;
+        }
+#endif
+#if !PJD_HB_WRITE
+        rec.p = p; rec.d_in = D_in;
+        rec.czf = c | (z << 8) | ((D_in < D_end && !flag) ? 0u : PJD_REC_SKIP);
+#else
+        if (D_in < D_end && !flag) {
+            OutCtx O;
+            O.region = B.ent + im.ent_base + (size_t)(g.q - im.lane_base) * im.lane_cap;
+            O.stage = area + l;
+            O.cap = im.lane_cap;
+            O.n = 0; O.npair = 0; O.dcA = 0; O.dcB = 0; O.overflow = 0;
+            O.ru = im.idct_mcus * dus;
+            O.marks = B.marks + im.iwg_base;
+            O.lane_q = g.q;
+            O.D_in = D_in;
+            li.first_du |= D_in;
+            {
+                const uint32_t first_du = im.first_mcu * dus;
+                const uint32_t d_next = (z == 0) ? D_in : D_in + 1;
+                const uint32_t k = (d_next - first_du + O.ru - 1) / O.ru;
+                O.mark_next = k;
+                O.mark_D = first_du + k * O.ru;
+            }
+            uint32_t err = 0;
+            const uint32_t p0 = p, c0 = c, z0 = z, mark_next0 = O.mark_next, mark_D0 = O.mark_D;
+            write_span(P, g.words, g.col, p, c, z, g.end_bit, err, D, D_end, O);
+            li.n_ent = O.n;
+            npair = O.npair;
+            li.dc_sum[0] = (uint16_t)O.dcA; li.dc_sum[1] = (uint16_t)(O.dcA >> 16); li.dc_sum[2] = (uint16_t)O.dcB;
+            const bool has_next = g.seg + 1 < im.seg_base + im.n_seg;
+            const bool last_seg = !has_next && (im.flags & PJD_IF_ENDS_STREAM) != 0;
+            const bool eof_lane = g.seg_last && last_seg;
+            const bool eof_crossed = last_seg && !g.seg_last && p > g.seg_end_bit;
+            bool settled = false;
+            if (err || (eof_lane && (D < D_end || p > g.seg_end_bit)) || eof_crossed) {
+                Careful R;
+                R.marks = O.marks; R.mark_next = mark_next0; R.mark_D = mark_D0; R.ru = O.ru; R.lane_q = g.q;
+                careful_span(P, g.words, g.col, p0, c0, z0, g.end_bit, (eof_lane || eof_crossed) ? g.seg_end_bit : 0xffffffffu, eof_lane,
+                             D_in, D_end, O.region, O.cap, R);
+                li.n_ent = R.n;
+                npair = 0;
+                li.dc_sum[0] = (uint16_t)R.dcA; li.dc_sum[1] = (uint16_t)(R.dcA >> 16); li.dc_sum[2] = (uint16_t)R.dcB;
+                if (R.ovf) flag |= 1u << PJD_FLAG_OVERFLOW;
+                else if (R.cls) {
+                    const unsigned long long key = ((unsigned long long)(g.base_bit + R.p_err) << 32) | ((unsigned long long)R.D_err << 4) | (R.cls << 1) | R.in_dc;
+                    atomicMin(&B.imstate[hw.image].err_key, key);
+                    settled = true;
+                }
+            }
+            if (!settled) {
+                if (err) flag |= 1u << PJD_FLAG_SYMBOL;
+                if (O.overflow) flag |= 1u << PJD_FLAG_OVERFLOW;
+                if (D == D_end) {
+                    if (p > g.seg_end_bit) flag |= 1u << PJD_FLAG_SEGMENT;
+                    if (has_next && ((p + 7) & ~7u) != g.seg_end_bit) flag |= 1u << PJD_FLAG_SEGMENT;
+                    if (last_seg && !flag) atomicMin(&B.imstate[hw.image].end_pos, g.base_bit + p);
+                } else {
+                    if (S.p_img - g.base_bit != p || (S.cz >> 8) != c || (S.cz & 255) != z) flag |= 1u << PJD_FLAG_VERIFY;
+                    if (D - D_in != S.cnt) flag |= 1u << PJD_FLAG_VERIFY;
+                    if (g.seg_last) flag |= 1u << PJD_FLAG_SEGMENT;
+                }
+            }
+        }
+#endif
+    }
+#if PJD_HB_WRITE
+    if (g.valid) B.lane_info[g.q] = li;
+#else
+    if (g.valid) { rec.czf |= flag << PJD_REC_FLAG_SHIFT; lane_rec[g.q] = rec; }
+#endif
+#if PJD_HB_SYNC
+    if (!first_is_head && !dead) {
+        const uint64_t fin = op_wait_flag(B.wave_gen + (size_t)(PJD_GENS - 1) * B.n_hwave + w - 1, dead);
+        if (fin != entry_used) flag |= 1u << PJD_FLAG_STITCH;
+    }
+    if (B.dbg && l == 0) {
+        const uint64_t ts5 = __builtin_amdgcn_s_memrealtime();
+        uint32_t *d = B.dbg + (size_t)w * 32;
+        d[0] = (uint32_t)ts0; d[1] = (uint32_t)(ts1 - ts0); d[2] = (uint32_t)(ts2 - ts1); d[3] = (uint32_t)(ts3 - ts2);
+        d[4] = (uint32_t)(ts4 - ts3); d[5] = (uint32_t)(ts5 - ts4); d[6] = hw.image; d[7] = hw.n_lanes;
+        d[7] |= ((uint32_t)(((__builtin_amdgcn_s_memtime() - tc0) * 16) / ((ts5 - ts0) ? (ts5 - ts0) : 1)) & 0xffffffu) << 8;
+    }
+    if (dead) flag |= 1u << PJD_FLAG_TIMEOUT;
+#endif
+#if PJD_HB_WRITE
+    uint32_t wflag = flag, went = npair, wsteps = g.valid ? li.n_ent / 2 - (li.n_ent + PJD_GROUP - 1) / PJD_GROUP : 0, wpos = (flag && g.valid) ? g.base_bit : 0xffffffffu;
+    uint32_t wfill = g.valid ? (uint32_t)(((uint64_t)li.n_ent << 10) / im.lane_cap) : 0u;
+#if !PJD_HB_SYNC
+    uint32_t wpre = g.valid ? (rec.czf >> PJD_REC_FLAG_SHIFT) & ((1u << PJD_FLAG_REASONS) - 1u) : 0u;
+#endif
+    for (int off = 1; off < 64; off <<= 1) {
+        wflag |= __shfl_xor(wflag, off); went += __shfl_xor(went, off); wsteps += __shfl_xor(wsteps, off);
+        { const uint32_t o = __shfl_xor(wfill, off); wfill = o > wfill ? o : wfill; }
+        const uint32_t o = __shfl_xor(wpos, off);
+        wpos = o < wpos ? o : wpos;
+#if !PJD_HB_SYNC
+        wpre |= __shfl_xor(wpre, off);
+#endif
+    }
+    if (l == 0) { atomicAdd(B.stats + PJD_STAT_ENTRIES, (unsigned long long)(went + wsteps)); atomicAdd(B.stats + PJD_STAT_STEPS, (unsigned long long)wsteps); atomicMax(B.stats + PJD_STAT_FILL, (unsigned long long)wfill); }
+#if !PJD_HB_SYNC
+    if (wflag && l == 0) atomicMin(&B.imstate[hw.image].flag_pos, wpos);
+    wflag &= ~wpre;
+#endif
+#else
+    uint32_t wflag = flag, wpos = (flag && g.valid) ? g.base_bit : 0xffffffffu;
+    for (int off = 1; off < 64; off <<= 1) {
+        wflag |= __shfl_xor(wflag, off);
+        const uint32_t o = __shfl_xor(wpos, off);
+        wpos = o < wpos ? o : wpos;
+    }
+#endif
+    if (wflag && l == 0) {
+        atomicMin(&B.imstate[hw.image].flag_pos, wpos);
+        for (int r = 0; r < PJD_FLAG_REASONS; r++)
+            if (wflag & (1u << r)) atomicAdd(B.stats + PJD_STAT_FLAG0 + r, 1ull);
+    }
diff --git a/pim-jpeg-decoder_amd/csrc/pjd_k_huffman.hip b/pim-jpeg-decoder_amd/csrc/pjd_k_huffman.hip
--- a/pim-jpeg-decoder_amd/csrc/pjd_k_huffman.hip
+++ b/pim-jpeg-decoder_amd/csrc/pjd_k_huffman.hip
@@ -798,287 +798,11 @@
 #endif
 __global__ __launch_bounds__(PJD_HUFF_THREADS) PJD_HUFF_OCC_ATTR void pjd_k_huff_lanes(PjdDevBatch B, uint32_t hwg_base, uint32_t *__restrict__ ticket)
 {
-    const uint32_t t = threadIdx.x, l = t & 63, wi = t >> 6;
-    uint8_t *lds = pjd_huff_lds;
-    uint8_t *areas = lds + B.max_lut_bytes;
-    uint8_t *phase_tabs = areas + PJD_HUFF_WAVES * PJD_WAVE_LDS;
-    uint32_t *tick = reinterpret_cast<uint32_t *>(phase_tabs + PJD_HUFF_WAVES * PJD_PHASE_LDS);
-    if (t == 0) *tick = hwg_base + atomicAdd(ticket, 1u);
-    __syncthreads();
-    const uint32_t gidx = rfl(*tick);
-    const PjdDevHuffWg wg = B.hwgs[gidx];
-    {
-        const PjdDevTset &T = B.tsets[wg.tset];
-        const uint32_t n16 = T.lut_bytes / 16;
-        const uint4 *tsrc = reinterpret_cast<const uint4 *>(B.luts) + T.lut_off16;
-        uint4 *tdst = reinterpret_cast<uint4 *>(lds);
-        for (uint32_t i0 = t; i0 < n16; i0 += 4 * PJD_HUFF_THREADS) {
-            const uint32_t i1 = i0 + PJD_HUFF_THREADS, i2 = i1 + PJD_HUFF_THREADS, i3 = i2 + PJD_HUFF_THREADS;
-            uint4 v0 = tsrc[i0], v1, v2, v3;
-            if (i1 < n16) v1 = tsrc[i1];
-            if (i2 < n16) v2 = tsrc[i2];
-            if (i3 < n16) v3 = tsrc[i3];
-            tdst[i0] = v0;
-            if (i1 < n16) tdst[i1] = v1;
-            if (i2 < n16) tdst[i2] = v2;
-            if (i3 < n16) tdst[i3] = v3;
-        }
-    }
-    const bool wave_on = wi < wg.n_waves;
-    const uint32_t w = wg.first_wave + (wave_on ? wi : 0u);
-    const PjdDevHuffWave hw = B.hwaves[w];
-    const PjdDevImage &im = B.images[hw.image];
-    PhaseCtx P;
-    {
-        const uint32_t nl = rfl(im.n_luma), dus = rfl(im.dus_per_mcu), nc = dus - nl;
-        const uint32_t c1 = nc >= 1 ? 1u : 0u, c2 = nc >= 2 ? 2u : c1;
-        const uint32_t lb = lds_abs(lds);
-        P.lbase = lb;
-        P.tY  = rfl((lb + (uint32_t)im.tbl_slot[0][0] * PJD_L1_BYTES) | (lb + (uint32_t)im.tbl_slot[0][1] * PJD_L1_BYTES) << 16);
-        P.tC1 = rfl((lb + (uint32_t)im.tbl_slot[c1][0] * PJD_L1_BYTES) | (lb + (uint32_t)im.tbl_slot[c1][1] * PJD_L1_BYTES) << 16);
-        P.tC2 = rfl((lb + (uint32_t)im.tbl_slot[c2][0] * PJD_L1_BYTES) | (lb + (uint32_t)im.tbl_slot[c2][1] * PJD_L1_BYTES) << 16);
-        P.nc = nc; P.dus1 = dus - 1;
-        P.xbase = lds_abs(phase_tabs) + wi * PJD_PHASE_LDS;
-    }
-    const uint32_t dus = P.dus1 + 1;
-    P.build(l);
-    __syncthreads();
-    if (!wave_on) return;
-
-    const uint64_t ts0 = B.dbg ? __builtin_amdgcn_s_memrealtime() : 0;
-    const uint64_t tc0 = B.dbg ? __builtin_amdgcn_s_memtime() : 0;
-    uint64_t *genA = B.wave_gen, *genB = B.wave_gen + B.n_hwave;
-    LaneGeom g;
-    g.valid = l < hw.n_lanes;
-    g.q = hw.first_lane + l;
-    g.seg_first = g.seg_last = false;
-    g.seg = 0; g.end_bit = g.seg_end_bit = g.base_bit = 0;
-    g.words = (pjd_gptr)readfirstlane_u64((uint64_t)(B.words + (size_t)w * B.word_rows * 64));
-    g.col = l * 4;
-    uint32_t seg_first_du = 0, seg_n_du = 0;
-    const uint32_t sub_bytes = rfl(im.sub_bytes);
-    if (g.valid) {
-        const PjdDevSub sb = B.lanes[g.q];
-        g.seg = sb.seg & 0x7fffffffu;
-        g.seg_first = (sb.seg >> 31) != 0;
-        const PjdDevSegment sg = B.segs[g.seg];
-        const uint32_t end_byte = sb.byte_start + sub_bytes < sg.byte_end ? sb.byte_start + sub_bytes : sg.byte_end;
-        g.seg_last = end_byte == sg.byte_end;
-        g.base_bit = sb.byte_start * 8;
-        g.end_bit = (end_byte - sb.byte_start) * 8;
-        g.seg_end_bit = (sg.byte_end - sb.byte_start) * 8;
-        seg_first_du = sg.first_du; seg_n_du = sg.n_du;
-    }
-    uint32_t *area = reinterpret_cast<uint32_t *>(areas + wi * PJD_WAVE_LDS);
-    ChkCtx K;
-    K.state = area + l;
-    K.rem = area + PJD_NCHK * 64 + l;
-    K.chk_bits = sub_bytes * 8 / PJD_NCHK;
-    K.walk_max = rfl(im.walk_max);
-    for (int j = 0; j < PJD_NCHK; j++) { K.state[j * 64] = 0xffffffffu; K.rem[j * 64] = 0; }
-    const bool first_is_head = __shfl((uint32_t)g.seg_first, 0) != 0;
-    const uint32_t last_lane = hw.n_lanes - 1;
-    bool dead = false;
-    uint32_t flag = 0;
-
-    WaveState S;
-    {
-        uint32_t p = 0, c = 0, z = 0, ndu = 0, j = 1;
-        if (g.valid) {
-            uint32_t oa, orem;
-            sync_span<false>(P, g.words, g.col, p, c, z, g.end_bit, ndu, K, j, 0xffffffffu, oa, orem);
-            chk_finish(K, j, ndu);
-        }
-        S.p_img = p + g.base_bit; S.cz = (c << 8) | z; S.cnt = ndu;
-    }
-    if (l == last_lane) op_store(genA + w, pjd_pack_state(S.p_img, S.cz >> 8, S.cz & 255) | OP_FLAG);
-    const uint64_t ts1 = B.dbg ? __builtin_amdgcn_s_memrealtime() : 0;
-
-    uint64_t entry_used = 0;
-    uint32_t err_acc = 0;
-    bool ok = true;
-    WalkBuf wb;
-    wb.ecs = (pjd_gptr)readfirstlane_u64((uint64_t)(B.ecs + im.ecs_off));
-    wb.clamp = rfl(im.ecs_len) + 40u;
-    wb.cb = 0; wb.cw = 0; wb.cn = 0; wb.have = 0;
-    if (!first_is_head) entry_used = op_wait_flag(genA + w - 1, dead);
-    BCache Bc;
-    Bc.st = 0xffffffffu; Bc.rem = 0; Bc.p = 0; Bc.cz = 0;
-    ok = wave_rounds(P, g, K, wb, S, Bc, g.valid ? 1u : 0u, (uint32_t)entry_used,
-                     (((uint32_t)(entry_used >> 32) & 255) << 8) | ((uint32_t)(entry_used >> 40) & 255), !first_is_head && !dead,
-                     err_acc, B.stats, 0, B.dbg ? B.dbg + (size_t)w * 32 + 8 : nullptr);
-    if (l == last_lane) op_store(genB + w, pjd_pack_state(S.p_img, S.cz >> 8, S.cz & 255) | OP_FLAG);
-    const uint64_t ts2 = B.dbg ? __builtin_amdgcn_s_memrealtime() : 0;
-
-    for (uint32_t gen = 1; gen + 1 < PJD_GENS; gen++) {
-        if (!first_is_head && !dead) {
-            const uint64_t truth = op_wait_flag(B.wave_gen + (size_t)gen * B.n_hwave + w - 1, dead);
-            if (!dead && truth != entry_used) {
-                entry_used = truth;
-                ok = wave_rounds(P, g, K, wb, S, Bc, 0u, (uint32_t)truth,
-                                 (((uint32_t)(truth >> 32) & 255) << 8) | ((uint32_t)(truth >> 40) & 255), true,
-                                 err_acc, B.stats, 2, nullptr) && ok;
-            }
-        }
-        if (l == last_lane) op_store(B.wave_gen + (size_t)(gen + 1) * B.n_hwave + w, pjd_pack_state(S.p_img, S.cz >> 8, S.cz & 255) | OP_FLAG);
-    }
-    if (!ok) flag |= 1u << PJD_FLAG_NOSYNC;
-    const uint64_t ts3 = B.dbg ? __builtin_amdgcn_s_memrealtime() : 0;
-
-    const uint32_t du_cap = rfl(im.n_du) + 1;
-    uint32_t cnt = 0, v = 0, f = 0;
-    if (g.valid) {
-        cnt = S.cnt;
-        v = cnt < du_cap ? cnt : du_cap;
-        if (g.seg_first) { f = 1; v = seg_first_du + v < du_cap ? seg_first_du + v : du_cap; }
-    }
-    wave_seg_scan(v, f, du_cap);
-    const uint32_t agg_v = __shfl(v, 63), agg_f = __shfl(f, 63);
-    uint32_t du_in = 0;
-    if (w == im.hwave_base) {
-        if (l == 0) op_store(B.wave_desc + w, op_desc(OP_ST_PFX, agg_v, agg_f, dead));
-    } else {
-        if (l == 0) op_store(B.wave_desc + w, op_desc(OP_ST_AGG, agg_v, agg_f, dead));
-        uint32_t rv = 0, rf = 0;
-        bool poison = false;
-        int hi = (int)w - 1;
-        for (;;) {
-            const int j = hi - (int)l;
-            const bool inside = j >= (int)im.hwave_base;
-            uint64_t d = OP_ST_PFX;
-            if (inside) {
-                uint32_t it = 0;
-                do { d = op_load(B.wave_desc + j); if (d & OP_ST_MASK) break; __builtin_amdgcn_s_sleep(8); } while (++it < OP_SPIN_LIMIT);
-            }
-            const bool ready = (d & OP_ST_MASK) != 0;
-            if (__any(!ready)) { dead = true; break; }
-            const uint64_t pfx_mask = __ballot((d & OP_ST_MASK) == OP_ST_PFX);
-            const int k = pfx_mask ? __builtin_ctzll(pfx_mask) : 64;
-            const bool use = (int)l <= k;
-            uint32_t xv = use ? (uint32_t)d & 0x0fffffffu : 0u, xf = use ? (uint32_t)((d >> 60) & 1u) : 0u;
-            poison = poison || __any(use && (d & OP_POISON));
-            for (int off = 1; off < 64; off <<= 1) {
-                const uint32_t ov = __shfl_down(xv, off), of = __shfl_down(xf, off);
-                if ((int)l + off < 64) seg_combine(ov, of, xv, xf, du_cap);
-            }
-            const uint32_t wvv = __shfl(xv, 0), wf = __shfl(xf, 0);
-            { uint32_t nv = rv, nf = rf; seg_combine(wvv, wf, nv, nf, du_cap); rv = nv; rf = nf; }
-            if (k < 64) break;
-            hi -= 64;
-        }
-        if (poison) dead = true;
-        du_in = rv;
-        uint32_t iv = agg_v, ifl = agg_f;
-        seg_combine(rv, rf, iv, ifl, du_cap);
-        if (l == 0) op_store(B.wave_desc + w, op_desc(OP_ST_PFX, iv, ifl, dead));
-    }
-    const uint64_t ts4 = B.dbg ? __builtin_amdgcn_s_memrealtime() : 0;
-
-    const uint32_t prev_p = __shfl_up(S.p_img, 1), prev_cz = __shfl_up(S.cz, 1);
-    const uint32_t prev_v = __shfl_up(v, 1), prev_f = __shfl_up(f, 1);
-    uint32_t npair = 0;
-    PjdDevLaneInfo li;
-    li.n_ent = 0; li.first_du = g.seg_first ? PJD_LANE_SEG_FIRST : 0u; li.dc_sum[0] = li.dc_sum[1] = li.dc_sum[2] = 0; li.pad_ = 0;
-    if (g.valid && !dead) {
-        uint32_t D;
-        if (g.seg_first) D = seg_first_du;
-        else if (l == 0) D = du_in;
-        else if (prev_f) D = prev_v;
-        else D = du_in + prev_v < du_cap ? du_in + prev_v : du_cap;
-        const uint32_t D_in = D, D_end = seg_first_du + seg_n_du;
-        uint32_t p, c, z;
-        if (g.seg_first) { p = 0; c = 0; z = 0; }
-        else {
-            if (l == 0) { p = (uint32_t)entry_used - g.base_bit; c = (uint32_t)(entry_used >> 32) & 255; z = (uint32_t)(entry_used >> 40) & 255; }
-            else { p = prev_p - g.base_bit; c = prev_cz >> 8; z = prev_cz & 255; }
-            if (D_in < D_end && (D_in % dus) != c) flag |= 1u << PJD_FLAG_SEGMENT;
-        }
-        if (D_in < D_end && !flag) {
-            OutCtx O;
-            O.region = B.ent + im.ent_base + (size_t)(g.q - im.lane_base) * im.lane_cap;
-            O.stage = area + l;
-            O.cap = im.lane_cap;
-            O.n = 0; O.npair = 0; O.dcA = 0; O.dcB = 0; O.overflow = 0;
-            O.ru = im.idct_mcus * dus;
-            O.marks = B.marks + im.iwg_base;
-            O.lane_q = g.q;
-            O.D_in = D_in;
-            li.first_du |= D_in;
-            {
-                const uint32_t first_du = im.first_mcu * dus;
-                const uint32_t d_next = (z == 0) ? D_in : D_in + 1;
-                const uint32_t k = (d_next - first_du + O.ru - 1) / O.ru;
-                O.mark_next = k;
-                O.mark_D = first_du + k * O.ru;
-            }
-            uint32_t err = 0;
-            const uint32_t p0 = p, c0 = c, z0 = z, mark_next0 = O.mark_next, mark_D0 = O.mark_D;
-            write_span(P, g.words, g.col, p, c, z, g.end_bit, err, D, D_end, O);
-            li.n_ent = O.n;
-            npair = O.npair;
-            li.dc_sum[0] = (uint16_t)O.dcA; li.dc_sum[1] = (uint16_t)(O.dcA >> 16); li.dc_sum[2] = (uint16_t)O.dcB;
-            const bool has_next = g.seg + 1 < im.seg_base + im.n_seg;
-            const bool last_seg = !has_next && (im.flags & PJD_IF_ENDS_STREAM) != 0;
-            const bool eof_lane = g.seg_last && last_seg;
-            const bool eof_crossed = last_seg && !g.seg_last && p > g.seg_end_bit;
-            bool settled = false;
-            if (err || (eof_lane && (D < D_end || p > g.seg_end_bit)) || eof_crossed) {
-                Careful R;
-                R.marks = O.marks; R.mark_next = mark_next0; R.mark_D = mark_D0; R.ru = O.ru; R.lane_q = g.q;
-                careful_span(P, g.words, g.col, p0, c0, z0, g.end_bit, (eof_lane || eof_crossed) ? g.seg_end_bit : 0xffffffffu, eof_lane,
-                             D_in, D_end, O.region, O.cap, R);
-                li.n_ent = R.n;
-                npair = 0;
-                li.dc_sum[0] = (uint16_t)R.dcA; li.dc_sum[1] = (uint16_t)(R.dcA >> 16); li.dc_sum[2] = (uint16_t)R.dcB;
-                if (R.ovf) flag |= 1u << PJD_FLAG_OVERFLOW;
-                else if (R.cls) {
-                    const unsigned long long key = ((unsigned long long)(g.base_bit + R.p_err) << 32) | ((unsigned long long)R.D_err << 4) | (R.cls << 1) | R.in_dc;
-                    atomicMin(&B.imstate[hw.image].err_key, key);
-                    settled = true;
-                }
-            }
-            if (!settled) {
-                if (err) flag |= 1u << PJD_FLAG_SYMBOL;
-                if (O.overflow) flag |= 1u << PJD_FLAG_OVERFLOW;
-                if (D == D_end) {
-                    if (p > g.seg_end_bit) flag |= 1u << PJD_FLAG_SEGMENT;
-                    if (has_next && ((p + 7) & ~7u) != g.seg_end_bit) flag |= 1u << PJD_FLAG_SEGMENT;
-                    if (last_seg && !flag) atomicMin(&B.imstate[hw.image].end_pos, g.base_bit + p);
-                } else {
-                    if (S.p_img - g.base_bit != p || (S.cz >> 8) != c || (S.cz & 255) != z) flag |= 1u << PJD_FLAG_VERIFY;
-                    if (D - D_in != S.cnt) flag |= 1u << PJD_FLAG_VERIFY;
-                    if (g.seg_last) flag |= 1u << PJD_FLAG_SEGMENT;
-                }
-            }
-        }
-    }
-    if (g.valid) B.lane_info[g.q] = li;
-    if (!first_is_head && !dead) {
-        const uint64_t fin = op_wait_flag(B.wave_gen + (size_t)(PJD_GENS - 1) * B.n_hwave + w - 1, dead);
-        if (fin != entry_used) flag |= 1u << PJD_FLAG_STITCH;
-    }
-    if (B.dbg && l == 0) {
-        const uint64_t ts5 = __builtin_amdgcn_s_memrealtime();
-        uint32_t *d = B.dbg + (size_t)w * 32;
-        d[0] = (uint32_t)ts0; d[1] = (uint32_t)(ts1 - ts0); d[2] = (uint32_t)(ts2 - ts1); d[3] = (uint32_t)(ts3 - ts2);
-        d[4] = (uint32_t)(ts4 - ts3); d[5] = (uint32_t)(ts5 - ts4); d[6] = hw.image; d[7] = hw.n_lanes;
-        d[7] |= ((uint32_t)(((__builtin_amdgcn_s_memtime() - tc0) * 16) / ((ts5 - ts0) ? (ts5 - ts0) : 1)) & 0xffffffu) << 8;
-    }
-    if (dead) flag |= 1u << PJD_FLAG_TIMEOUT;
-    uint32_t wflag = flag, went = npair, wsteps = g.valid ? li.n_ent / 2 - (li.n_ent + PJD_GROUP - 1) / PJD_GROUP : 0, wpos = (flag && g.valid) ? g.base_bit : 0xffffffffu;
-    uint32_t wfill = g.valid ? (uint32_t)(((uint64_t)li.n_ent << 10) / im.lane_cap) : 0u;
-    for (int off = 1; off < 64; off <<= 1) {
-        wflag |= __shfl_xor(wflag, off); went += __shfl_xor(went, off); wsteps += __shfl_xor(wsteps, off);
-        { const uint32_t o = __shfl_xor(wfill, off); wfill = o > wfill ? o : wfill; }
-        const uint32_t o = __shfl_xor(wpos, off);
-        wpos = o < wpos ? o : wpos;
-    }
-    if (l == 0) { atomicAdd(B.stats + PJD_STAT_ENTRIES, (unsigned long long)(went + wsteps)); atomicAdd(B.stats + PJD_STAT_STEPS, (unsigned long long)wsteps); atomicMax(B.stats + PJD_STAT_FILL, (unsigned long long)wfill); }
-    if (wflag && l == 0) {
-        atomicMin(&B.imstate[hw.image].flag_pos, wpos);
-        for (int r = 0; r < PJD_FLAG_REASONS; r++)
-            if (wflag & (1u << r)) atomicAdd(B.stats + PJD_STAT_FLAG0 + r, 1ull);
-    }
+#define PJD_HB_SYNC 1
+#define PJD_HB_WRITE 1
+#include "pjd_k_huff_body.h"
+#undef PJD_HB_SYNC
+#undef PJD_HB_WRITE
 }
 
 struct SeqWin {
@@ -1190,6 +914,24 @@
     hipLaunchKernelGGL(pjd_k_huff_exact_lut, dim3(n), dim3(64), (size_t)b.max_lut_bytes + 64, s, b, image_list, dense_base);
 }
 
+__global__ __launch_bounds__(PJD_HUFF_THREADS) __attribute__((amdgpu_waves_per_eu(6, 6))) void pjd_k_huff_sync(PjdDevBatch B, uint32_t hwg_base, uint32_t *__restrict__ ticket, PjdDevLaneRec *__restrict__ lane_rec)
+{
+#define PJD_HB_SYNC 1
+#define PJD_HB_WRITE 0
+#include "pjd_k_huff_body.h"
+#undef PJD_HB_SYNC
+#undef PJD_HB_WRITE
+}
+
+__global__ __launch_bounds__(PJD_HUFF_THREADS) void pjd_k_huff_write(PjdDevBatch B, uint32_t hwg_base, const PjdDevLaneRec *__restrict__ lane_rec)
+{
+#define PJD_HB_SYNC 0
+#define PJD_HB_WRITE 1
+#include "pjd_k_huff_body.h"
+#undef PJD_HB_SYNC
+#undef PJD_HB_WRITE
+}
+
 static size_t huff_lds_bytes(const PjdDevBatch &b)
 {
     return (size_t)b.max_lut_bytes + PJD_HUFF_WAVES * (PJD_WAVE_LDS + PJD_PHASE_LDS) + 16;
@@ -1204,16 +946,26 @@
 {
     if (b.n_hwave) hipLaunchKernelGGL(pjd_k_lane_words, dim3(b.n_hwave), dim3(256), 0, s, b);
 }
-void pjd_launch_huff_lanes(hipStream_t s, const PjdDevBatch &b)
-{
-    if (b.n_hwg) hipLaunchKernelGGL(pjd_k_huff_lanes, dim3(b.n_hwg), dim3(PJD_HUFF_THREADS), huff_lds_bytes(b), s, b, 0u, b.ticket);
-}
-hipError_t pjd_huff_lanes_occupancy(const PjdDevBatch &b, int *workgroups_per_cu, size_t *lds_bytes)
+static void launch_huff(hipStream_t s, const PjdDevBatch &b, uint32_t hwg_first, uint32_t hwg_count, uint32_t *ticket, PjdDevLaneRec *rec)
+{
+    if (!hwg_count) return;
+    if (!rec) { hipLaunchKernelGGL(pjd_k_huff_lanes, dim3(hwg_count), dim3(PJD_HUFF_THREADS), huff_lds_bytes(b), s, b, hwg_first, ticket); return; }
+    hipLaunchKernelGGL(pjd_k_huff_sync, dim3(hwg_count), dim3(PJD_HUFF_THREADS), huff_lds_bytes(b), s, b, hwg_first, ticket, rec);
+    hipLaunchKernelGGL(pjd_k_huff_write, dim3(hwg_count), dim3(PJD_HUFF_THREADS), huff_lds_bytes(b), s, b, hwg_first, (const PjdDevLaneRec *)rec);
+}
+void pjd_launch_huff_lanes(hipStream_t s, const PjdDevBatch &b, PjdDevLaneRec *rec)
+{
+    launch_huff(s, b, 0u, b.n_hwg, b.ticket, rec);
+}
+hipError_t pjd_huff_lanes_occupancy(const PjdDevBatch &b, int *workgroups_per_cu, size_t *lds_bytes, int *sync_workgroups_per_cu, int *write_workgroups_per_cu)
 {
     *lds_bytes = huff_lds_bytes(b);
-    return hipOccupancyMaxActiveBlocksPerMultiprocessor(workgroups_per_cu, pjd_k_huff_lanes, PJD_HUFF_THREADS, *lds_bytes);
-}
-void pjd_launch_huff_lanes_group(hipStream_t s, const PjdDevBatch &b, const PjdDevGroup &g, uint32_t group_index)
-{
-    if (g.hwg_count) hipLaunchKernelGGL(pjd_k_huff_lanes, dim3(g.hwg_count), dim3(PJD_HUFF_THREADS), huff_lds_bytes(b), s, b, g.hwg_first, b.ticket + 2 + 2 * group_index);
-}
+    hipError_t e = hipOccupancyMaxActiveBlocksPerMultiprocessor(workgroups_per_cu, pjd_k_huff_lanes, PJD_HUFF_THREADS, *lds_bytes);
+    if (e == hipSuccess && sync_workgroups_per_cu) e = hipOccupancyMaxActiveBlocksPerMultiprocessor(sync_workgroups_per_cu, pjd_k_huff_sync, PJD_HUFF_THREADS, *lds_bytes);
+    if (e == hipSuccess && write_workgroups_per_cu) e = hipOccupancyMaxActiveBlocksPerMultiprocessor(write_workgroups_per_cu, pjd_k_huff_write, PJD_HUFF_THREADS, *lds_bytes);
+    return e;
+}
+void pjd_launch_huff_lanes_group(hipStream_t s, const PjdDevBatch &b, const PjdDevGroup &g, uint32_t group_index, PjdDevLaneRec *rec)
+{
+    launch_huff(s, b, g.hwg_first, g.hwg_count, b.ticket + 2 + 2 * group_index, rec);
+}
diff --git a/pim-jpeg-decoder_amd/csrc/pjd_kernels.h b/pim-jpeg-decoder_amd/csrc/pjd_kernels.h
--- a/pim-jpeg-decoder_amd/csrc/pjd_kernels.h
+++ b/pim-jpeg-decoder_amd/csrc/pjd_kernels.h
@@ -124,6 +124,6 @@
 void pjd_launch_progressive(hipStream_t s, const PjdDevBatch &b, const uint32_t *image_list, const uint64_t *dense_base, uint32_t n);
 void pjd_launch_build_tables(hipStream_t s, const PjdDevBatch &b);
 void pjd_launch_lane_words(hipStream_t s, const PjdDevBatch &b);
-void pjd_launch_huff_lanes(hipStream_t s, const PjdDevBatch &b);
-hipError_t pjd_huff_lanes_occupancy(const PjdDevBatch &b, int *workgroups_per_cu, size_t *lds_bytes);
-void pjd_launch_huff_lanes_group(hipStream_t s, const PjdDevBatch &b, const PjdDevGroup &g, uint32_t group_index);
+void pjd_launch_huff_lanes(hipStream_t s, const PjdDevBatch &b, PjdDevLaneRec *rec);
+hipError_t pjd_huff_lanes_occupancy(const PjdDevBatch &b, int *workgroups_per_cu, size_t *lds_bytes, int *sync_workgroups_per_cu = nullptr, int *write_workgroups_per_cu = nullptr);
+void pjd_launch_huff_lanes_group(hipStream_t s, const PjdDevBatch &b, const PjdDevGroup &g, uint32_t group_index, PjdDevLaneRec *rec);
diff --git a/pim-jpeg-decoder_amd/csrc/pjd_plan.cpp b/pim-jpeg-decoder_amd/csrc/pjd_plan.cpp
--- a/pim-jpeg-decoder_amd/csrc/pjd_plan.cpp
+++ b/pim-jpeg-decoder_amd/csrc/pjd_plan.cpp
@@ -666,6 +666,10 @@
             if (!std::strcmp(e, "picture")) P.dc_per_picture = true;
             else if (!std::strcmp(e, "scan")) P.dc_per_picture = false;
         }
+        if (const char *e = std::getenv("PJD_HUFF_FORM")) {
+            if (!std::strcmp(e, "fused")) P.huff_split_chain = P.huff_split_groups = false;
+            else if (!std::strcmp(e, "split")) P.huff_split_chain = P.huff_split_groups = true;
+        }
     }
     P.lut_buf_bytes = align_up(lut_off + 16, 256);
     if (P.ecs_buf_bytes >= (1ull << 40)) { err = "batch bitstream too large"; return PJD_E_ARG; }
diff --git a/pim-jpeg-decoder_amd/csrc/pjd_plan.h b/pim-jpeg-decoder_amd/csrc/pjd_plan.h
--- a/pim-jpeg-decoder_amd/csrc/pjd_plan.h
+++ b/pim-jpeg-decoder_amd/csrc/pjd_plan.h
@@ -62,6 +62,7 @@
     std::vector<PjdDevIdctWg> iwgs_dense_red, cwgs_red;
     uint64_t plane_bytes = 0;
     bool dc_per_picture = false;
+    bool huff_split_chain = true, huff_split_groups = false;
     int plan_mode = 0;
     std::vector<uint32_t> tset_step_bits;
     std::vector<uint32_t> tset_nominal_bytes;
diff --git a/pim-jpeg-decoder_amd/python/pjd_amd/__init__.py b/pim-jpeg-decoder_amd/python/pjd_amd/__init__.py
--- a/pim-jpeg-decoder_amd/python/pjd_amd/__init__.py
+++ b/pim-jpeg-decoder_amd/python/pjd_amd/__init__.py
@@ -462,6 +462,21 @@
         self.ctx._check(self.L.pjd_batch_huff_occupancy(self._h, C.byref(n), C.byref(lds)), "pjd_batch_huff_occupancy")
         return int(n.value), int(lds.value)
 
+    def huff_split_occupancy(self):
+        self.L.pjd_batch_huff_split_occupancy.restype = C.c_int32
+        self.L.pjd_batch_huff_split_occupancy.argtypes = [C.c_void_p, C.POINTER(C.c_int32), C.POINTER(C.c_int32)]
+        ns, nw = C.c_int32(), C.c_int32()
+        self.ctx._check(self.L.pjd_batch_huff_split_occupancy(self._h, C.byref(ns), C.byref(nw)), "pjd_batch_huff_split_occupancy")
+        return int(ns.value), int(nw.value)
+
+    def huff_form(self):
+        self.L.pjd_batch_huff_form.restype = C.c_int32
+        self.L.pjd_batch_huff_form.argtypes = [C.c_void_p]
+        n = int(self.L.pjd_batch_huff_form(self._h))
+        if n < 0:
+            self.ctx._check(n, "pjd_batch_huff_form")
+        return n
+
     def output_size(self, i):
         return int(self.L.pjd_batch_output_size(self._h, i))
 
```

After: 136,300. 6.4% lower.
